# nanoporetech/dorado

Hardware: NVIDIA H100
Metric: basecalled samples/s (higher is better)
Workload: dtype f16 (fp32 accumulate; fp32 decode)

## Files before the change

### dorado_b200/csrc/capi.cu

```cuda
#include "b200call.h"

#include "common.cuh"
#include "decode.h"
#include "engine.h"

#include <cmath>
#include <cstddef>
#include <cstring>
#include <limits>
#include <string>

#undef b200_engine_create
#undef b200_pool_create

namespace {

thread_local std::string g_last_error;

constexpr size_t kDescSizeBeforeLstmPrecision = offsetof(b200_model_desc, lstm_precision);

b200_model_desc read_desc(const b200_model_desc* desc, size_t desc_size) {
    if (desc_size < kDescSizeBeforeLstmPrecision) throw std::invalid_argument("b200_model_desc: desc_size is smaller than any published descriptor");
    const unsigned char* bytes = reinterpret_cast<const unsigned char*>(desc);
    for (size_t i = sizeof(b200_model_desc); i < desc_size; ++i) {
// ... 90 lines not shown
        buf[buf_len - 1] = '\0';
    });
}

int b200_engine_terminate(b200_engine* e) {
    return guarded([&] {
        if (!e) throw std::invalid_argument("b200_engine_terminate: null argument");
        reinterpret_cast<b200::Engine*>(e)->terminate();
    });
}

int b200_engine_restart(b200_engine* e) {
    return guarded([&] {
        if (!e) throw std::invalid_argument("b200_engine_restart: null argument");
        reinterpret_cast<b200::Engine*>(e)->restart();
    });
}

int b200_engine_set_low_latency(b200_engine* e, int32_t on) {
    return guarded([&] {
        if (!e) throw std::invalid_argument("b200_engine_set_low_latency: null argument");
        reinterpret_cast<b200::Engine*>(e)->set_low_latency(on != 0);
    });
}

int b200_engine_set_num_runners(b200_engine* e, int32_t num_runners) {
    return guarded([&] {
        if (!e || num_runners < 1) throw std::invalid_argument("b200_engine_set_num_runners: null engine or num_runners < 1");
        reinterpret_cast<b200::Engine*>(e)->set_num_runners(num_runners);
    });
}

int32_t b200_engine_num_runners(const b200_engine* e) { return e ? reinterpret_cast<const b200::Engine*>(e)->num_runners() : 0; }

int32_t b200_engine_is_low_latency(const b200_engine* e) { return e && reinterpret_cast<const b200::Engine*>(e)->low_latency(); }

int b200_engine_batch_timeouts_ms(const b200_engine* e, int32_t* first_chunk_ms, int32_t* last_chunk_ms) {
    return guarded([&] {
        if (!e) throw std::invalid_argument("b200_engine_batch_timeouts_ms: null argument");
        int a = 0, b = 0;
        reinterpret_cast<const b200::Engine*>(e)->batch_timeouts_ms(&a, &b);
        if (first_chunk_ms) *first_chunk_ms = a;
        if (last_chunk_ms) *last_chunk_ms = b;
    });
}

int b200_pool_create_sized(const b200_model_desc* desc, size_t desc_size, const b200_tensor* tensors, int32_t num_tensors,
                           const int32_t* devices, int32_t num_devices, int32_t runners_per_device, int32_t batch_size,
                           int32_t chunk_size, b200_pool** out) {
    return guarded([&] {
        if (!desc || !tensors || !devices || !out) throw std::invalid_argument("b200_pool_create: null argument");
        *out = reinterpret_cast<b200_pool*>(new b200::Pool(read_desc(desc, desc_size), tensors, num_tensors, devices, num_devices,
                                                           runners_per_device, batch_size, chunk_size));
    });
}

int b200_pool_create(const b200_model_desc* desc, const b200_tensor* tensors, int32_t num_tensors, const int32_t* devices,
                     int32_t num_devices, int32_t runners_per_device, int32_t batch_size, int32_t chunk_size, b200_pool** out) {
    return b200_pool_create_sized(desc, kDescSizeBeforeLstmPrecision, tensors, num_tensors, devices, num_devices,
                                  runners_per_device, batch_size, chunk_size, out);
}

int b200_pool_destroy(b200_pool* p) {
    return guarded([&] { delete reinterpret_cast<b200::Pool*>(p); });
}

int32_t b200_pool_num_runners(const b200_pool* p) { return p ? reinterpret_cast<const b200::Pool*>(p)->num_runners() : 0; }
int32_t b200_pool_out_len(const b200_pool* p) { return p ? reinterpret_cast<const b200::Pool*>(p)->out_len() : 0; }

b200_runner* b200_pool_runner(b200_pool* p, int32_t index) {
    return p ? reinterpret_cast<b200_runner*>(reinterpret_cast<b200::Pool*>(p)->runner(index)) : nullptr;
}

int b200_pool_runner_info(const b200_pool* p, int32_t index, int32_t* numa_node, int64_t* batches) {
    return guarded([&] {
        if (!p) throw std::invalid_argument("b200_pool_runner_info: null argument");
        const auto* pool = reinterpret_cast<const b200::Pool*>(p);
        if (index < 0 || index >= pool->num_runners()) throw std::invalid_argument("b200_pool_runner_info: index out of range");
        if (numa_node) *numa_node = pool->runner_numa_node(index);
        if (batches) *batches = pool->runner_batches(index);
    });
}

int b200_pool_call_chunks(b200_pool* p, const uint16_t* chunks, int64_t num_chunks, uint8_t* moves, char* sequence,
                          char* qstring, int32_t* n_bases, double* seconds) {
    return guarded([&] {
        if (!p) throw std::invalid_argument("b200_pool_call_chunks: null argument");
        const double s = reinterpret_cast<b200::Pool*>(p)->call_chunks(chunks, num_chunks, moves, sequence, qstring, n_bases);
        if (seconds) *seconds = s;
    });
}

int b200_runner_create(b200_engine* e, int32_t batch_size, int32_t chunk_size, b200_runner** out) {
    return guarded([&] {
        if (!e || !out) throw std::invalid_argument("b200_runner_create: null argument");
        *out = reinterpret_cast<b200_runner*>(new b200::Runner(*reinterpret_cast<b200::Engine*>(e), batch_size, chunk_size));
    });
}

int b200_runner_destroy(b200_runner* r) {
    return guarded([&] { delete reinterpret_cast<b200::Runner*>(r); });
}

int b200_runner_set_decoder_options(b200_runner* r, const b200_decoder_options* o) {
    return guarded([&] {
        if (!r || !o) throw std::invalid_argument("b200_runner_set_decoder_options: null argument");
        reinterpret_cast<b200::Runner*>(r)->set_decoder_options(*o);
    });
}

int32_t b200_runner_batch_size(const b200_runner* r) { return r ? reinterpret_cast<const b200::Runner*>(r)->batch_size() : 0; }
int32_t b200_runner_chunk_size(const b200_runner* r) { return r ? reinterpret_cast<const b200::Runner*>(r)->chunk_size() : 0; }
int32_t b200_runner_out_len(const b200_runner* r) { return r ? reinterpret_cast<const b200::Runner*>(r)->out_len() : 0; }

int b200_runner_accept_chunk_f16(b200_runner* r, int32_t idx, const uint16_t* samples, int64_t len) {
    return guarded([&] {
        if (!r || !samples) throw std::invalid_argument("b200_runner_accept_chunk_f16: null argument");
        reinterpret_cast<b200::Runner*>(r)->accept_chunk_f16(idx, samples, len);
    });
}

int b200_runner_accept_chunk_f32(b200_runner* r, int32_t idx, const float* samples, int64_t len) {
    return guarded([&] {
        if (!r || !samples) throw std::invalid_argument("b200_runner_accept_chunk_f32: null argument");
        reinterpret_cast<b200::Runner*>(r)->accept_chunk_f32(idx, samples, len);
    });
}

int32_t b200_runner_variable_chunk_sizes(const b200_runner* r) {
    return r && reinterpret_cast<const b200::Runner*>(r)->variable_chunk_sizes();
}

int b200_runner_accept_chunk_var_f16(b200_runner* r, int32_t idx, const uint16_t* samples, int64_t len) {
    return guarded([&] {
        if (!r || !samples) throw std::invalid_argument("b200_runner_accept_chunk_var_f16: null argument");
        reinterpret_cast<b200::Runner*>(r)->accept_chunk_var_f16(idx, samples, len);
    });
}

uint16_t* b200_runner_input(b200_runner* r) { return r ? reinterpret_cast<b200::Runner*>(r)->input() : nullptr; }

int b200_runner_call_chunks(b200_runner* r, int32_t num_chunks, b200_result* out) {
    return guarded([&] {
        if (!r || !out) throw std::invalid_argument("b200_runner_call_chunks: null argument");
        *out = reinterpret_cast<b200::Runner*>(r)->call_chunks(num_chunks);
    });
}

int b200_generate_chunks(uint64_t num_samples, uint64_t chunk_size, uint64_t stride, uint64_t overlap, uint64_t* offsets,
                         uint64_t capacity, uint64_t* count) {
    return guarded([&] {
        if (!count || (!offsets && capacity)) throw std::invalid_argument("b200_generate_chunks: null argument");
        *count = b200::generate_chunks(num_samples, chunk_size, stride, overlap, offsets, capacity);
    });
}

int b200_generate_variable_chunks(uint64_t num_samples, uint64_t chunk_size, uint64_t stride, uint64_t overlap,
                                  uint64_t* intervals, uint64_t capacity, uint64_t* count) {
    return guarded([&] {
        if (!count || (!intervals && capacity)) throw std::invalid_argument("b200_generate_variable_chunks: null argument");
        *count = b200::generate_variable_chunks(num_samples, chunk_size, stride, overlap, intervals, capacity);
    });
}

int b200_stitch_chunks(const b200_called_chunk* chunks, uint64_t n_chunks, uint64_t raw_samples, int32_t stride,
                       uint8_t* moves_out, char* sequence_out, char* qstring_out, uint64_t* n_moves_out,
                       uint64_t* n_bases_out) {
    return guarded([&] {
        if (!moves_out || !sequence_out || !qstring_out || !n_moves_out || !n_bases_out) {
            throw std::invalid_argument("b200_stitch_chunks: null argument");
        }
        b200::stitch_chunks(chunks, n_chunks, raw_samples, stride, moves_out, sequence_out, qstring_out, n_moves_out,
                            n_bases_out);
    });
}

int b200_runner_accept_raw_chunk(b200_runner* r, int32_t chunk_idx, const b200_raw_chunk* chunk) {
    return guarded([&] {
        if (!r || !chunk) throw std::invalid_argument("b200_runner_accept_raw_chunk: null argument");
        reinterpret_cast<b200::Runner*>(r)->accept_raw_chunk(chunk_idx, *chunk);
    });
}

int b200_runner_debug_read_input(b200_runner* r, int32_t num_chunks, uint16_t* input_out) {
    return guarded([&] {
        if (!r) throw std::invalid_argument("b200_runner_debug_read_input: null argument");
        reinterpret_cast<b200::Runner*>(r)->debug_read_input(num_chunks, input_out);
    });
}

int b200_engine_runner_bytes(b200_engine* e, int32_t batch_size, int32_t chunk_size, uint64_t* bytes) {
    return guarded([&] {
        if (!e || !bytes) throw std::invalid_argument("b200_engine_runner_bytes: null argument");
        *bytes = b200::runner_device_bytes(*reinterpret_cast<b200::Engine*>(e), batch_size, chunk_size);
    });
}

int b200_engine_benchmark_batch_sizes(b200_engine* e, int32_t chunk_size, int32_t granularity, int32_t max_batch_size,
                                      int32_t* batch_sizes, float* ms_per_chunk, int32_t capacity, int32_t* count) {
    return guarded([&] {
        if (!e || !count || capacity < 0) throw std::invalid_argument("b200_engine_benchmark_batch_sizes: bad argument");
        *count = b200::benchmark_batch_sizes(*reinterpret_cast<b200::Engine*>(e), chunk_size, granularity, max_batch_size,
                                             batch_sizes, ms_per_chunk, capacity);
    });
}

int b200_select_batch_size(const int32_t* batch_sizes, const float* ms_per_chunk, int32_t count, int32_t max_batch_size,
                           int32_t granularity, float time_penalty, int32_t* selected) {
    return guarded([&] {
        if (!selected) throw std::invalid_argument("b200_select_batch_size: null argument");
        *selected = b200::select_batch_size(batch_sizes, ms_per_chunk, count, max_batch_size, granularity, time_penalty);
    });
}

int b200_runner_upload(b200_runner* r) {
    return guarded([&] {
        if (!r) throw std::invalid_argument("b200_runner_upload: null argument");
        reinterpret_cast<b200::Runner*>(r)->upload();
    });
}

int b200_runners_step_device(b200_runner** runners, int32_t n_runners, int32_t num_chunks, int32_t iters, float* total_ms) {
    return guarded([&] {
        if (!runners || !total_ms) throw std::invalid_argument("b200_runners_step_device: null argument");
        b200::pipelined_steps(reinterpret_cast<b200::Runner**>(runners), n_runners, num_chunks, iters, total_ms);
    });
}

int b200_runner_step_device(b200_runner* r, int32_t num_chunks, int32_t iters, float* total_ms, float* forward_ms,
                            float* decode_ms) {
    return guarded([&] {
        if (!r || !total_ms) throw std::invalid_argument("b200_runner_step_device: null argument");
        reinterpret_cast<b200::Runner*>(r)->step_device(num_chunks, iters, total_ms, forward_ms, decode_ms);
    });
}

int b200_runner_forward_scores(b200_runner* r, int32_t num_chunks, uint16_t* scores_out) {
    return guarded([&] {
        if (!r || !scores_out) throw std::invalid_argument("b200_runner_forward_scores: null argument");
        reinterpret_cast<b200::Runner*>(r)->forward_scores_to_host(num_chunks, scores_out);
    });
}

int b200_runner_profile(b200_runner* r, int32_t num_chunks, char* buf, uint64_t buf_len) {
    return guarded([&] {
        if (!r || !buf || buf_len == 0) throw std::invalid_argument("b200_runner_profile: null argument");
        const std::string s = reinterpret_cast<b200::Runner*>(r)->profile(num_chunks);
        std::strncpy(buf, s.c_str(), buf_len - 1);
        buf[buf_len - 1] = 0;
    });
}

int b200_runner_plan_info(const b200_runner* r, char* buf, uint64_t buf_len) {
    return guarded([&] {
        if (!r || !buf || buf_len == 0) throw std::invalid_argument("b200_runner_plan_info: null argument");
        const std::string s = reinterpret_cast<const b200::Runner*>(r)->plan_info();
        std::strncpy(buf, s.c_str(), buf_len - 1);
        buf[buf_len - 1] = 0;
    });
}

int b200_runner_debug_read_workspace(b200_runner* r, uint64_t offset, uint64_t bytes, void* dst) {
    return guarded([&] {
        if (!r || !dst) throw std::invalid_argument("debug_read_workspace: null argument");
        reinterpret_cast<b200::Runner*>(r)->debug_read_workspace(offset, bytes, dst);
    });
}

int b200_decode_scores(int32_t device, const uint16_t* scores, int32_t N, int32_t T, int32_t C, float clamp_val,
                       const b200_decoder_options* opts, uint8_t* moves, char* sequence, char* qstring,
                       int32_t* n_bases) {
    return guarded([&] {
        if (!scores || !opts || !moves || !sequence || !qstring || !n_bases) {
            throw std::invalid_argument("b200_decode_scores: null argument");
        }
        b200::decode_host_scores(device, scores, N, T, C, clamp_val, *opts, moves, sequence, qstring, n_bases);
    });
}

int b200_test_gemm(int32_t device, const uint16_t* a, const uint16_t* b, const float* bias, int32_t M, int32_t N,
                   int32_t K, int32_t activation, uint16_t* c) {
    return guarded([&] {
        if (!a || !b || !c) throw std::invalid_argument("b200_test_gemm: null argument");
        b200::test_gemm_host(device, a, b, bias, M, N, K, activation, c);
    });
}

int b200_test_gemm_fp8(int32_t device, const uint8_t* a, const uint8_t* b, int32_t M, int32_t N, int32_t K, int32_t activation,
                       const uint16_t* residual, float alpha, void* c) {
    return guarded([&] {
        if (!a || !b || !c) throw std::invalid_argument("b200_test_gemm_fp8: null argument");
        b200::test_gemm_fp8_host(device, a, b, M, N, K, activation, residual, alpha, c);
    });
}

int b200_test_gemm_s8(int32_t device, const int8_t* a, const int8_t* b, const float* col_scale, const float* bias, int32_t M,
                      int32_t N, int32_t K, int32_t activation, uint16_t* c) {
    return guarded([&] {
        if (!a || !b || !col_scale || !c) throw std::invalid_argument("b200_test_gemm_s8: null argument");
        b200::test_gemm_s8_host(device, a, b, col_scale, bias, M, N, K, activation, c);
    });
}

int b200_test_quantize_rows(const uint16_t* f16, int32_t rows, int32_t cols, int8_t* q, uint16_t* scale) {
    return guarded([&] {
        if (rows < 1 || cols < 1 || !f16 || !q || !scale) throw std::invalid_argument("b200_test_quantize_rows: bad argument");
        b200::quantize_rows_f16(f16, rows, cols, q, scale);
    });
}

int b200_test_to_e4m3(const uint16_t* f16, int64_t n, uint8_t* out) {
    return guarded([&] {
        if (n < 0 || (n && (!f16 || !out))) throw std::invalid_argument("b200_test_to_e4m3: bad argument");
        for (int64_t i = 0; i < n; ++i) out[i] = b200::e4m3_from_f16_bits(f16[i]);
    });
}

int b200_test_remove_bits(const uint16_t* f16, int64_t n, int32_t bits, uint16_t* out) {
    return guarded([&] {
        if (n < 0 || (n && (!f16 || !out)) || bits < 0 || bits > 10) throw std::invalid_argument("b200_test_remove_bits: bad argument");
        for (int64_t i = 0; i < n; ++i) out[i] = b200::remove_bits_f16(f16[i], bits);
    });
}

int b200_test_attention(int32_t device, const uint16_t* qkv, int32_t N, int32_t T, int32_t H, int32_t win_upper,
                        int32_t win_lower, uint16_t* out) {
    return guarded([&] {
        if (!qkv || !out) throw std::invalid_argument("b200_test_attention: null argument");
        b200::test_attention_host(device, qkv, N, T, H, win_upper, win_lower, out);
    });
}

}

extern "C" {

int b200_modbase_engine_create(const b200_modbase_desc* desc, const b200_tensor* tensors, int32_t num_tensors, int32_t device,
                               b200_modbase_engine** out) {
    return guarded([&] {
        if (!desc || !tensors || !out) throw std::invalid_argument("b200_modbase_engine_create: null argument");
        *out = reinterpret_cast<b200_modbase_engine*>(new b200::ModBaseEngine(*desc, tensors, num_tensors, device));
    });
}

int b200_modbase_engine_destroy(b200_modbase_engine* e) {
    return guarded([&] { delete reinterpret_cast<b200::ModBaseEngine*>(e); });
}

int b200_modbase_runner_create(b200_modbase_engine* e, int32_t batch_size, b200_modbase_runner** out) {
    return guarded([&] {
        if (!e || !out) throw std::invalid_argument("b200_modbase_runner_create: null argument");
        *out = reinterpret_cast<b200_modbase_runner*>(new b200::ModBaseRunner(*reinterpret_cast<b200::ModBaseEngine*>(e), batch_size));
    });
}

int b200_modbase_runner_destroy(b200_modbase_runner* r) {
    return guarded([&] { delete reinterpret_cast<b200::ModBaseRunner*>(r); });
}

static const b200::ModBaseRunner* mb_runner(const b200_modbase_runner* r) { return reinterpret_cast<const b200::ModBaseRunner*>(r); }
int32_t b200_modbase_runner_batch_size(const b200_modbase_runner* r) { return r ? mb_runner(r)->batch_size() : 0; }
int32_t b200_modbase_runner_sig_len(const b200_modbase_runner* r) { return r ? mb_runner(r)->engine().sig_len : 0; }
int32_t b200_modbase_runner_seq_len(const b200_modbase_runner* r) { return r ? mb_runner(r)->engine().seq_len : 0; }
int32_t b200_modbase_runner_out_len(const b200_modbase_runner* r) { return r ? mb_runner(r)->engine().out_len : 0; }
int32_t b200_modbase_runner_num_out(const b200_modbase_runner* r) { return r ? mb_runner(r)->engine().desc().num_out : 0; }

int b200_modbase_runner_accept_chunk(b200_modbase_runner* r, int32_t idx, const uint16_t* signal, int64_t sig_len,
                                     const int8_t* kmers, int64_t kmer_elems) {
    return guarded([&] {
        if (!r) throw std::invalid_argument("b200_modbase_runner_accept_chunk: null runner");
        reinterpret_cast<b200::ModBaseRunner*>(r)->accept_chunk(idx, signal, sig_len, kmers, kmer_elems);
    });
}

int b200_modbase_runner_call_chunks(b200_modbase_runner* r, int32_t num_chunks, const uint16_t** probs) {
    return guarded([&] {
        if (!r || !probs) throw std::invalid_argument("b200_modbase_runner_call_chunks: null argument");
        *probs = reinterpret_cast<b200::ModBaseRunner*>(r)->call_chunks(num_chunks);
    });
}

int b200_modbase_runner_profile(b200_modbase_runner* r, char* buf, uint64_t buf_len) {
    return guarded([&] {
        if (!r || !buf || buf_len == 0) throw std::invalid_argument("b200_modbase_runner_profile: null argument");
        const std::string s = reinterpret_cast<b200::ModBaseRunner*>(r)->profile();
        std::strncpy(buf, s.c_str(), buf_len - 1);
        buf[buf_len - 1] = '\0';
    });
}

int b200_modbase_runner_debug_read_workspace(b200_modbase_runner* r, uint64_t offset, uint64_t bytes, void* dst) {
    return guarded([&] {
        if (!r || !dst) throw std::invalid_argument("b200_modbase_runner_debug_read_workspace: null argument");
        reinterpret_cast<b200::ModBaseRunner*>(r)->debug_read_workspace(offset, bytes, dst);
    });
}

}
```

### dorado_b200/csrc/engine.h

```cpp
#pragma once

#include "b200call.h"
#include "b200_crf_math.h"
#include "frontend.h"
#include "common.cuh"
#include "lstm_kernels.h"

#include <atomic>
#include <condition_variable>
#include <memory>
#include <mutex>
#include <stdexcept>
#include <string>
#include <vector>

namespace b200 {

struct Unsupported : std::runtime_error {
    using std::runtime_error::runtime_error;
};

class Bump {
public:
    Bump() = default;
// ... 3 lines not shown
        const size_t off = m_used;
        m_used += (bytes + 255) & ~size_t(255);
        if (!m_base) return nullptr;
        if (m_used > m_cap) throw std::logic_error("device memory layout overflows its allocation");
        return static_cast<T*>(static_cast<void*>(m_base + off));
    }
    size_t used() const { return m_used; }

private:
    unsigned char* m_base = nullptr;
    size_t m_cap = 0, m_used = 0;
};

class Arena {
public:
    Arena() = default;
    ~Arena() {
        if (m_base) cudaFree(m_base);
    }
    Arena(const Arena&) = delete;
    Arena& operator=(const Arena&) = delete;
    template <typename F>
    void allocate(F&& layout) {
        if (m_base) throw std::logic_error("Arena::allocate called twice");
        Bump sizing;
        layout(sizing);
        B200_CUDA(cudaMalloc(&m_base, sizing.used()));
        m_cap = sizing.used();
        Bump carve(m_base, m_cap);
        layout(carve);
    }
    size_t capacity() const { return m_cap; }

private:
    unsigned char* m_base = nullptr;
    size_t m_cap = 0;
};

struct ProfileSink {
    std::vector<cudaEvent_t> events;
    std::vector<std::string> names;
    void begin(cudaStream_t s);
    void mark(const char* name, cudaStream_t s);
    std::vector<std::pair<std::string, float>> report();
    ~ProfileSink();
};

class ForwardPlan {
public:
    virtual ~ForwardPlan() = default;
    virtual void run(cudaStream_t stream, ProfileSink* prof = nullptr) = 0;
    virtual int launches() const = 0;
    virtual void set_chunk_lengths(const int32_t* ) {}
    virtual std::string info() const { return std::string(); }
    virtual void check_errors() {}
};

class Model {
public:
    virtual ~Model() = default;
    virtual size_t workspace_bytes(int N, int T_in) const = 0;
    virtual bool variable_chunk_sizes() const { return false; }
    int num_runners_hint = 2;
    virtual std::unique_ptr<ForwardPlan> make_plan(int N, int T_in, const __half* signal, __half* scores,
                                                   void* workspace, size_t workspace_bytes) = 0;
};

std::unique_ptr<Model> make_lstm_model(const b200_model_desc& desc, const b200_tensor* tensors, int n);
std::unique_ptr<Model> make_tx_model(const b200_model_desc& desc, const b200_tensor* tensors, int n);

const b200_tensor& find_tensor(const b200_tensor* tensors, int n, const std::string& name);
__half* upload_f16(const std::vector<float>& v);
float* upload_f32(const std::vector<float>& v);

class Engine {
public:
    Engine(const b200_model_desc& desc, const b200_tensor* tensors, int num_tensors, int device);
    ~Engine();
    const b200_model_desc& desc() const { return m_desc; }
    int device() const { return m_device; }
    cudaStream_t stream() const { return m_stream; }
    Model& model() { return *m_model; }
    std::mutex& stats_mutex() { return m_stats_mutex; }
    b200_stats stats() const;

    void terminate();
    void restart();
    bool terminated() const { return m_terminated.load(); }
    void set_low_latency(bool on) { m_low_latency.store(on); }
    void set_num_runners(int n) { m_model->num_runners_hint = n < 1 ? 1 : (n > 16 ? 16 : n); }
    int num_runners() const { return m_model->num_runners_hint; }
    bool low_latency() const { return m_low_latency.load(); }
    void batch_timeouts_ms(int* first_chunk_ms, int* last_chunk_ms) const;
    struct CallGuard {
        explicit CallGuard(Engine& e);
        ~CallGuard();
        Engine& eng;
    };

    std::atomic<int64_t> batches_called{0};
    std::atomic<int64_t> gpu_launches{0};
    std::atomic<int64_t> arena_bytes{0};
    double model_decode_ms = 0, h2d_ms = 0, d2h_ms = 0;

private:
    b200_model_desc m_desc;
    int m_device;
    cudaStream_t m_stream = nullptr;
    std::unique_ptr<Model> m_model;
    mutable std::mutex m_stats_mutex;
    std::atomic<bool> m_terminated{false};
    std::atomic<bool> m_low_latency{false};
    std::mutex m_life_mutex;
    std::condition_variable m_life_cv;
    int m_in_flight = 0;
};

class Runner;
void pipelined_steps(Runner** runners, int n_runners, int num_chunks, int iters, float* total_ms);

struct RunnerBuffers {
    b200_qtable* qtable = nullptr;
    int32_t* lens = nullptr;
    __half* input = nullptr;
    __half* scores = nullptr;
    void* ws = nullptr;
    size_t ws_bytes = 0;
    float* bwd = nullptr;
    uint2* beam = nullptr;
    unsigned char* out = nullptr;
    size_t out_bytes = 0;
};

class Runner {
public:
    friend void pipelined_steps(Runner** runners, int n_runners, int num_chunks, int iters, float* total_ms);
    Runner(Engine& engine, int batch_size, int chunk_size);
    ~Runner();
    int batch_size() const { return m_N; }
    int chunk_size() const { return m_T_in; }
    int out_len() const { return m_T_out; }
    uint16_t* input();
    void set_decoder_options(const b200_decoder_options& o);
    void accept_chunk_f16(int idx, const uint16_t* samples, int64_t len);
    void accept_chunk_f32(int idx, const float* samples, int64_t len);
    bool variable_chunk_sizes() const;
    void accept_chunk_var_f16(int idx, const uint16_t* samples, int64_t len);
    void accept_raw_chunk(int idx, const b200_raw_chunk& chunk);
    void debug_read_input(int num_chunks, uint16_t* input_out);
    b200_result call_chunks(int num_chunks);
    void upload();
    void fill_synthetic_input();
    void step_device(int num_chunks, int iters, float* total_ms, float* forward_ms, float* decode_ms);
    void forward_scores_to_host(int num_chunks, uint16_t* scores_out);
    void debug_read_workspace(uint64_t offset, uint64_t bytes, void* dst);
    std::string profile(int num_chunks);
    std::string plan_info() const { return m_plan ? m_plan->info() : std::string(); }

private:
    void init();
    void release();
    bool m_counted = false;
    void stage_input(int n);
    void clear_raw_slot(int idx);
    void run_forward(int n);
    void run_decode(int n, ProfileSink* prof = nullptr);

    Engine& m_engine;
    cudaStream_t m_stream = nullptr;
    std::mutex m_mutex;
    int m_N, m_T_in, m_T_out, m_C;
    b200_decoder_options m_opts;
    uint16_t* m_h_input = nullptr;
    unsigned char* m_h_out = nullptr;
    int16_t* m_h_raw = nullptr;
    RawSlot* m_h_slots = nullptr;
    int16_t* m_d_raw = nullptr;
    RawSlot* m_d_slots = nullptr;
    int m_num_raw = 0;
    Arena m_arena;
    RunnerBuffers m_dev;
    std::unique_ptr<ForwardPlan> m_plan;
    void upload_qtable();
    int32_t* m_h_lens = nullptr;
    int32_t* m_h_nmoves = nullptr;
    cudaEvent_t m_ev[4] = {nullptr, nullptr, nullptr, nullptr};
};

class ModBaseEngine {
public:
    ModBaseEngine(const b200_modbase_desc& desc, const b200_tensor* tensors, int num_tensors, int device);
    ~ModBaseEngine();
    ModBaseEngine(const ModBaseEngine&) = delete;
    ModBaseEngine& operator=(const ModBaseEngine&) = delete;
    const b200_modbase_desc& desc() const { return m_desc; }
    int device() const { return m_device; }

    int sig_len = 0;
    int seq_len = 0;
    int t_enc = 0;
    int T = 0;
    int out_len = 0;
    float* sig12_w = nullptr;
    __half* sig3_w = nullptr;
    float* sig3_b = nullptr;
    float* seq1_w = nullptr;
    __half* seq2_w = nullptr;
    float* seq2_b = nullptr;
    __half* merge_w = nullptr;
    float* merge_b = nullptr;
    LstmLayerWeights lstm[2];
    float* fc_w = nullptr;
    float* fc_b = nullptr;
    float* up_w = nullptr;
    float* up_b = nullptr;

private:
    b200_modbase_desc m_desc;
    int m_device;
};

struct ModBasePlan;
class ModBaseRunner {
public:
    ModBaseRunner(ModBaseEngine& engine, int batch_size);
    ~ModBaseRunner();
    int batch_size() const { return m_N; }
    const ModBaseEngine& engine() const { return m_engine; }
    void accept_chunk(int idx, const uint16_t* signal, int64_t sig_len, const int8_t* kmers, int64_t kmer_elems);
    const uint16_t* call_chunks(int num_chunks);
    std::string profile();
    void debug_read_workspace(uint64_t offset, uint64_t bytes, void* dst);

private:
    void init();
    void release();
    void run(ProfileSink* prof);

    ModBaseEngine& m_engine;
    int m_N;
    int64_t m_kmer_elems = 0, m_out_elems = 0;
    cudaStream_t m_stream = nullptr;
    std::mutex m_mutex;
    uint16_t* m_h_sig = nullptr;
    int8_t* m_h_kmers = nullptr;
    __half* m_h_out = nullptr;
    Arena m_arena;
    void* m_d_ws = nullptr;
    size_t m_ws_bytes = 0;
    __half* m_d_sig = nullptr;
    int8_t* m_d_kmers = nullptr;
    __half* m_d_out = nullptr;
    std::unique_ptr<ModBasePlan> m_plan;
};

class Pool {
public:
    Pool(const b200_model_desc& desc, const b200_tensor* tensors, int num_tensors, const int* devices, int num_devices,
         int runners_per_device, int batch_size, int chunk_size);
    ~Pool();
    int num_runners() const;
    Runner* runner(int i);
    int runner_numa_node(int i) const;
    int64_t runner_batches(int i) const;
    int out_len() const { return m_t_out; }
    double call_chunks(const uint16_t* chunks, int64_t num_chunks, uint8_t* moves, char* sequence, char* qstring,
                       int32_t* n_bases);

private:
    struct Worker;
    struct Job {
        const uint16_t* chunks = nullptr;
        int64_t num_chunks = 0;
        uint8_t* moves = nullptr;
        char* sequence = nullptr;
        char* qstring = nullptr;
        int32_t* n_bases = nullptr;
    };
    void worker_main(Worker& w);
    void shutdown();
    int m_batch, m_chunk, m_t_out = 0;
    std::vector<std::unique_ptr<Engine>> m_engines;
    std::vector<std::unique_ptr<Worker>> m_workers;
    std::mutex m_mutex, m_job_mutex;
    std::condition_variable m_cv_job, m_cv_done;
    long long m_job_id = 0;
    int m_ready = 0, m_done = 0;
    bool m_stop = false;
    Job m_job;
    std::atomic<int64_t> m_cursor{0};
};

void decode_host_scores(int device, const uint16_t* scores, int N, int T, int C, float clamp_val,
                        const b200_decoder_options& opts, uint8_t* moves, char* sequence, char* qstring,
                        int32_t* n_bases);
void test_gemm_host(int device, const uint16_t* a, const uint16_t* b, const float* bias, int M, int N, int K,
                    int activation, uint16_t* c);
void test_attention_host(int device, const uint16_t* qkv, int N, int T, int H, int win_upper, int win_lower, uint16_t* out);
void test_gemm_fp8_host(int device, const uint8_t* a, const uint8_t* b, int M, int N, int K, int activation,
                        const uint16_t* residual, float alpha, void* c);

void test_gemm_s8_host(int device, const int8_t* a, const int8_t* b, const float* col_scale, const float* bias, int M, int N,
                       int K, int activation, uint16_t* c);
void quantize_rows_f16(const uint16_t* w16, int rows, int cols, int8_t* q, uint16_t* scale16);
float int8_row_inv(uint16_t scale16);

uint16_t f16_bits(float v);
uint16_t remove_bits_f16(uint16_t b, int bits);
std::vector<float> fp16_remove_bits(const float* v, size_t n, int bits);
uint8_t e4m3_from_f16_bits(uint16_t b);

size_t runner_device_bytes(Engine& engine, int batch_size, int chunk_size);
int benchmark_batch_sizes(Engine& engine, int chunk_size, int granularity, int max_batch_size, int32_t* batch_sizes,
                          float* ms_per_chunk, int capacity);
int select_batch_size(const int32_t* batch_sizes, const float* ms_per_chunk, int count, int max_batch_size, int granularity,
                      float time_penalty);

int lookup_chunk_benchmarks(const char* gpu_name, const char* model_name, int32_t* batch_sizes, float* ms_per_chunk, int capacity);
std::string device_name(int device);

void ensure_dynamic_smem(const void* kernel, int bytes);
template <typename K>
inline void ensure_dynamic_smem(K* kernel, int bytes) {
    ensure_dynamic_smem(reinterpret_cast<const void*>(kernel), bytes);
}

float log_beam_cut_of(float beam_cut);
void require_sm90(int device);

}
```

### dorado_b200/csrc/gemm.cu

```cuda
#include "gemm.h"

#include "common.cuh"
#include "engine.h"

#include <cstdlib>
#include <cstring>
#include <type_traits>
#include <vector>

namespace b200 {

namespace {

constexpr int BM = 128;
constexpr int BK = 64;
constexpr int BK8 = 128;
constexpr int BN_MAX = 128;
constexpr int STAGES = 5;
constexpr int GEMM_PARTS = 4;
constexpr int GEMM_THREADS = 384;

struct GemmKernelParams {
    int rows_per_batch, tiles_per_batch, N, num_k_blocks, bn;
    int num_tiles, n_tiles, m_tiles;
    int mfast;
    const float* bias;
    __half* out;
    uint32_t out_m1;
    long long out_s0, out_s1;
    uint32_t out_col_m1;
    long long out_col_s0;
    int bias_per_row;
    const float* rope;
    int rope_T, rope_cols, rope_stride;
    const __half* residual;
    float alpha;
    float* out_ss;
    const float* a_ss;
    const float* res_ss;
    const float* res_gain;
    int a_ss_parts, res_ss_parts;
    float norm_inv_dim, norm_eps;
    const float* col_scale;
};

__device__ __forceinline__ bool gemm_tile_at(const GemmKernelParams& p, int i, int* mt, int* nt) {
    const int tile = (int)blockIdx.x + i * (int)gridDim.x;
    if (p.mfast) {
        *mt = tile % p.m_tiles;
        *nt = tile / p.m_tiles;
    } else {
        *mt = tile / p.n_tiles;
        *nt = tile % p.n_tiles;
    }
    return tile < p.num_tiles;
}

template <int ACT>
__device__ __forceinline__ float act_apply(float v) {
    if constexpr (ACT == GEMM_ACT_SWISH) return swish_fast(v);
    else if constexpr (ACT == GEMM_ACT_SWISH_CLAMP) return fminf(swish_fast(v), 3.5f);
    else if constexpr (ACT == GEMM_ACT_TANH) return tanh_fast(v);
    else if constexpr (ACT == GEMM_ACT_TANH_X5) return 5.0f * tanh_fast(v);
    else return v;
}

template <int NCH, bool FP8, typename Acc>
__device__ __forceinline__ void wgmma_k_block(Acc (&acc)[BN_MAX / 32][16], uint64_t adesc, uint64_t bdesc, bool accumulate) {
#pragma unroll
    for (int k = 0; k < 4; ++k) {
#pragma unroll
        for (int c = 0; c < NCH; ++c) {
            if constexpr (std::is_same_v<Acc, int32_t>) {
                tc::wgmma_m64n32k32_s8(acc[c], adesc + (uint64_t)(2 * k), bdesc + (uint64_t)(c * 256 + 2 * k), accumulate || k != 0);
            } else if constexpr (FP8) {
                tc::wgmma_m64n32k32_e4m3(acc[c], adesc + (uint64_t)(2 * k), bdesc + (uint64_t)(c * 256 + 2 * k), accumulate || k != 0);
            } else {
                tc::wgmma_m64n32k16(acc[c], adesc + (uint64_t)(2 * k), bdesc + (uint64_t)(c * 256 + 2 * k), accumulate || k != 0);
            }
        }
    }
}

template <int ACT, bool FP8, int Q8 = GEMM_Q8_NONE>
__global__ void __launch_bounds__(GEMM_THREADS, 1) gemm_wgmma_kernel(const __grid_constant__ CUtensorMap tma_a,
                                                                     const __grid_constant__ CUtensorMap tma_w,
                                                                     const GemmKernelParams p) {
    constexpr bool S8 = Q8 == GEMM_Q8_OPERANDS;
    constexpr int KB = FP8 || S8 ? BK8 : BK;
    using Acc = std::conditional_t<S8, int32_t, float>;
    extern __shared__ __align__(1024) uint8_t smem_raw[];
    uint8_t* smem = smem_raw + ((1024u - (tc::smem_u32(smem_raw) & 1023u)) & 1023u);
    const uint32_t a_bytes = BM * 128;
    const uint32_t w_bytes = (uint32_t)p.bn * 128;
    const uint32_t stage_bytes = a_bytes + w_bytes;
    uint64_t* full = reinterpret_cast<uint64_t*>(smem + STAGES * stage_bytes);
    uint64_t* empty = full + STAGES;
    const int nch = p.bn / 32;

    if (threadIdx.x == 0) {
        for (int s = 0; s < STAGES; ++s) {
            tc::mbar_init(&full[s], 1);
            tc::mbar_init(&empty[s], 2);
        }
        tc::fence_barrier_init();
        tc::prefetch_tmap(&tma_a);
        tc::prefetch_tmap(&tma_w);
    }
    __syncthreads();
    const int wg = threadIdx.x >> 7;

    if (wg == 0) {
        if (threadIdx.x == 0) {
            int s = 0;
            uint32_t ph = 0;
            int mt, nt;
            for (int i = 0; gemm_tile_at(p, i, &mt, &nt); ++i) {
                const int batch = mt / p.tiles_per_batch;
                const int r0 = (mt % p.tiles_per_batch) * BM;
                for (int kb = 0; kb < p.num_k_blocks; ++kb) {
                    tc::mbar_wait_silent(&empty[s], ph ^ 1);
                    tc::mbar_arrive_expect_tx(&full[s], stage_bytes);
                    uint8_t* st = smem + s * stage_bytes;
                    tc::tma_load_3d(st, &tma_a, &full[s], kb * KB, r0, batch);
                    tc::tma_load_2d(st + a_bytes, &tma_w, &full[s], kb * KB, nt * p.bn);
                    if (++s == STAGES) {
                        s = 0;
                        ph ^= 1;
                    }
                }
            }
        }
        return;
    }

    const int half = wg - 1;
    const int t = threadIdx.x - 128 * wg;
    const int lane = t & 31, quad = lane & 3;
    const int rloc = half * 64 + (t >> 5) * 16 + (lane >> 2);
    const int n_out_total = ACT == GEMM_ACT_SWIGLU ? p.N / 2 : p.N;
    int s = 0;
    uint32_t ph = 0;
    int mt, nt;
    for (int ti = 0; gemm_tile_at(p, ti, &mt, &nt); ++ti) {
        Acc acc[BN_MAX / 32][16];
        int prev = -1;
        for (int kb = 0; kb < p.num_k_blocks; ++kb) {
            tc::mbar_wait_silent(&full[s], ph);
            const uint32_t st = tc::smem_u32(smem + s * stage_bytes);
            const uint64_t adesc = tc::wgmma_desc_sw128(st + (uint32_t)(half * 64 * 128));
            const uint64_t bdesc = tc::wgmma_desc_sw128(st + a_bytes);
            tc::wgmma_fence();
            switch (nch) {
                case 1: wgmma_k_block<1, FP8>(acc, adesc, bdesc, kb != 0); break;
                case 2: wgmma_k_block<2, FP8>(acc, adesc, bdesc, kb != 0); break;
                case 3: wgmma_k_block<3, FP8>(acc, adesc, bdesc, kb != 0); break;
                default: wgmma_k_block<4, FP8>(acc, adesc, bdesc, kb != 0); break;
            }
            tc::wgmma_commit();
            tc::wgmma_wait<1>();
            if (prev >= 0 && t == 0) tc::mbar_arrive(&empty[prev]);
            prev = s;
            if (++s == STAGES) {
                s = 0;
                ph ^= 1;
            }
        }
        tc::wgmma_wait<0>();
        if (t == 0) tc::mbar_arrive(&empty[prev]);

        const int batch = mt / p.tiles_per_batch;
        const int r0 = (mt % p.tiles_per_batch) * BM;
        const int n0 = nt * p.bn;
        bool valid[2];
        long long g[2], off[2];
        float r_a[2], r_res[2], row_bias[2];
#pragma unroll
        for (int h = 0; h < 2; ++h) {
            const int row = r0 + rloc + 8 * h;
            valid[h] = row < p.rows_per_batch;
            const uint32_t g32 = (uint32_t)(batch * p.rows_per_batch + row);
            g[h] = g32;
            off[h] = valid[h] ? (long long)(g32 / p.out_m1) * p.out_s0 + (long long)(g32 % p.out_m1) * p.out_s1 : 0;
            r_a[h] = 1.0f;
            r_res[h] = 1.0f;
            if (p.a_ss && valid[h]) {
                float ss = 0.0f;
                for (int i = 0; i < p.a_ss_parts; ++i) ss += __ldg(p.a_ss + g[h] * p.a_ss_parts + i);
                r_a[h] = rsqrtf(ss * p.norm_inv_dim + p.norm_eps);
            }
            if (p.res_ss && valid[h]) {
                float ss = 0.0f;
                for (int i = 0; i < p.res_ss_parts; ++i) ss += __ldg(p.res_ss + g[h] * p.res_ss_parts + i);
                r_res[h] = rsqrtf(ss * p.norm_inv_dim + p.norm_eps);
            }
            row_bias[h] = (p.bias && p.bias_per_row && valid[h]) ? __ldg(p.bias + g[h]) : 0.0f;
        }
        if constexpr (S8) {
#pragma unroll
            for (int c = 0; c < BN_MAX / 32; ++c) {
                if (c >= nch) continue;
#pragma unroll
                for (int j = 0; j < 4; ++j) {
                    const int nc = n0 + c * 32 + 8 * j + 2 * quad;
                    const float2 sc = __ldg(reinterpret_cast<const float2*>(p.col_scale + nc));
                    float2 b2 = make_float2(0.0f, 0.0f);
                    if (p.bias) b2 = __ldg(reinterpret_cast<const float2*>(p.bias + nc));
#pragma unroll
                    for (int h = 0; h < 2; ++h) {
                        if (!valid[h]) continue;
                        const float v0 = fmaf((float)acc[c][4 * j + 2 * h], sc.x, b2.x);
                        const float v1 = fmaf((float)acc[c][4 * j + 2 * h + 1], sc.y, b2.y);
                        *reinterpret_cast<__half2*>(p.out + off[h] + nc) = __floats2half2_rn(act_apply<ACT>(v0), act_apply<ACT>(v1));
                    }
                }
            }
        } else if constexpr (ACT == GEMM_ACT_ROPE) {
#pragma unroll
            for (int c = 0; c < BN_MAX / 32; c += 2) {
                if (c < nch) {
                    const int nc0 = n0 + c * 32;
                    const bool rot = nc0 < p.rope_cols;
#pragma unroll
                    for (int h = 0; h < 2; ++h) {
                        if (!valid[h]) continue;
                        const float4* tab = reinterpret_cast<const float4*>(p.rope) + (int)((uint32_t)g[h] % (uint32_t)p.rope_T);
#pragma unroll
                        for (int j = 0; j < 4; ++j) {
                            const int col = 8 * j + 2 * quad;
                            float a0 = acc[c][4 * j + 2 * h] * r_a[h], a1 = acc[c][4 * j + 2 * h + 1] * r_a[h];
                            float b0 = acc[c + 1][4 * j + 2 * h] * r_a[h], b1 = acc[c + 1][4 * j + 2 * h + 1] * r_a[h];
                            if (rot) {
                                const float4 cs = __ldg(tab + (size_t)(col / 2) * p.rope_stride);
                                const float x0 = cs.x * a0 - cs.y * b0, y0 = cs.y * a0 + cs.x * b0;
                                const float x1 = cs.z * a1 - cs.w * b1, y1 = cs.w * a1 + cs.z * b1;
                                a0 = x0; b0 = y0; a1 = x1; b1 = y1;
                            }
                            *reinterpret_cast<__half2*>(p.out + off[h] + nc0 + col) = __floats2half2_rn(a0, a1);
                            *reinterpret_cast<__half2*>(p.out + off[h] + nc0 + 32 + col) = __floats2half2_rn(b0, b1);
                        }
                    }
                }
            }
        } else {
            float ss_out[2][BN_MAX / 32];
#pragma unroll
            for (int c = 0; c < BN_MAX / 32; ++c) {
                ss_out[0][c] = ss_out[1][c] = 0.0f;
                if (c >= nch) continue;
#pragma unroll
                for (int j = 0; j < 4; ++j) {
                    const int nc = n0 + c * 32 + 8 * j + 2 * quad;
                    float2 b2 = make_float2(0.0f, 0.0f);
                    if (p.bias && !p.bias_per_row) b2 = __ldg(reinterpret_cast<const float2*>(p.bias + nc));
                    float2 gain = make_float2(1.0f, 1.0f);
                    if (p.residual && p.res_gain) gain = __ldg(reinterpret_cast<const float2*>(p.res_gain + nc));
                    const long long coff = p.out_col_m1 > 0
                            ? (long long)((uint32_t)nc / p.out_col_m1) * p.out_col_s0 + (long long)((uint32_t)nc % p.out_col_m1)
                            : nc;
#pragma unroll
                    for (int h = 0; h < 2; ++h) {
                        if (!valid[h]) continue;
                        float v0 = acc[c][4 * j + 2 * h] * r_a[h] + b2.x + row_bias[h];
                        float v1 = acc[c][4 * j + 2 * h + 1] * r_a[h] + b2.y + row_bias[h];
                        if constexpr (ACT == GEMM_ACT_SWIGLU) {
                            if constexpr (FP8) {
                                reinterpret_cast<uint8_t*>(p.out)[off[h] + nc / 2] = (uint8_t)tc::cvt_e4m3x2(v0 * swish_fast(v1), 0.0f);
                            } else {
                                p.out[off[h] + nc / 2] = __float2half_rn(v0 * swish_fast(v1));
                            }
                        } else {
                            if (p.residual) {
                                const float2 f = __half22float2(
                                        *reinterpret_cast<const __half2*>(p.residual + g[h] * (long long)n_out_total + nc));
                                const float ar = p.alpha * r_res[h];
                                v0 += (ar * gain.x) * f.x;
                                v1 += (ar * gain.y) * f.y;
                            }
                            const __half2 o = __floats2half2_rn(act_apply<ACT>(v0), act_apply<ACT>(v1));
                            if (p.out_ss) {
                                const float2 f = __half22float2(o);
                                ss_out[h][c] = fmaf(f.x, f.x, ss_out[h][c]);
                                ss_out[h][c] = fmaf(f.y, f.y, ss_out[h][c]);
                            }
                            if constexpr (Q8 == GEMM_Q8_STORE) {
                                const int32_t q0 = tc::cvt_rni_sat_s8(kInt8ActScale * act_apply<ACT>(v0));
                                const int32_t q1 = tc::cvt_rni_sat_s8(kInt8ActScale * act_apply<ACT>(v1));
                                *reinterpret_cast<uint16_t*>(reinterpret_cast<int8_t*>(p.out) + off[h] + coff) =
                                        (uint16_t)((q0 & 0xff) | ((q1 & 0xff) << 8));
                            } else {
                                *reinterpret_cast<__half2*>(p.out + off[h] + coff) = o;
                            }
                        }
                    }
                }
            }
            if (p.out_ss) {
#pragma unroll
                for (int h = 0; h < 2; ++h) {
#pragma unroll
                    for (int c = 0; c < GEMM_PARTS; ++c) {
                        float v = ss_out[h][c];
                        v += __shfl_xor_sync(0xffffffffu, v, 1);
                        v += __shfl_xor_sync(0xffffffffu, v, 2);
                        if (quad == 0 && valid[h]) p.out_ss[g[h] * (long long)(p.n_tiles * GEMM_PARTS) + nt * GEMM_PARTS + c] = v;
                    }
                }
            }
        }
    }
}

using EncodeFn = CUresult (*)(CUtensorMap*, CUtensorMapDataType, cuuint32_t, void*, const cuuint64_t*, const cuuint64_t*,
                              const cuuint32_t*, const cuuint32_t*, CUtensorMapInterleave, CUtensorMapSwizzle,
                              CUtensorMapL2promotion, CUtensorMapFloatOOBfill);

EncodeFn get_encode_fn() {
    static const EncodeFn fn = [] {
        void* p = nullptr;
        cudaDriverEntryPointQueryResult q;
        B200_CUDA(cudaGetDriverEntryPoint("cuTensorMapEncodeTiled", &p, cudaEnableDefault, &q));
        if (q != cudaDriverEntryPointSuccess || !p) throw CudaError("cuTensorMapEncodeTiled entry point not available");
        return reinterpret_cast<EncodeFn>(p);
    }();
    return fn;
}

CUtensorMap encode(const void* base, int rank, const cuuint64_t* dims, const cuuint64_t* strides_bytes,
                   const cuuint32_t* box, CUtensorMapSwizzle swz, uint32_t elem_bytes) {
    CUtensorMap m;
    cuuint32_t estr[5] = {1, 1, 1, 1, 1};
    const CUtensorMapDataType dt = elem_bytes == 1 ? CU_TENSOR_MAP_DATA_TYPE_UINT8 : CU_TENSOR_MAP_DATA_TYPE_FLOAT16;
    const CUresult r = get_encode_fn()(&m, dt, (cuuint32_t)rank, const_cast<void*>(base), dims,
                                       strides_bytes, box, estr, CU_TENSOR_MAP_INTERLEAVE_NONE, swz,
                                       CU_TENSOR_MAP_L2_PROMOTION_L2_256B, CU_TENSOR_MAP_FLOAT_OOB_FILL_NONE);
    if (r != CUDA_SUCCESS) {
        throw CudaError("cuTensorMapEncodeTiled failed with CUresult " + std::to_string((int)r));
    }
    return m;
}

}

CUtensorMap make_tmap_2d(const void* base, uint64_t inner, uint64_t outer, uint64_t outer_stride_bytes, uint32_t box_inner,
                         uint32_t box_outer, uint32_t elem_bytes) {
    const cuuint64_t dims[2] = {inner, outer};
    const cuuint64_t strides[1] = {outer_stride_bytes};
    const cuuint32_t box[2] = {box_inner, box_outer};
    const CUtensorMapSwizzle swz = box_inner * elem_bytes == 128 ? CU_TENSOR_MAP_SWIZZLE_128B
                                   : box_inner * elem_bytes == 64 ? CU_TENSOR_MAP_SWIZZLE_64B
                                                                  : CU_TENSOR_MAP_SWIZZLE_NONE;
    return encode(base, 2, dims, strides, box, swz, elem_bytes);
}

CUtensorMap make_tmap_3d(const void* base, uint64_t d0, uint64_t d1, uint64_t d2, uint64_t s1_bytes, uint64_t s2_bytes,
                         uint32_t b0, uint32_t b1, uint32_t b2, uint32_t elem_bytes) {
    const cuuint64_t dims[3] = {d0, d1, d2};
    const cuuint64_t strides[2] = {s1_bytes, s2_bytes};
    const cuuint32_t box[3] = {b0, b1, b2};
    const CUtensorMapSwizzle swz = b0 * elem_bytes == 128 ? CU_TENSOR_MAP_SWIZZLE_128B
                                   : b0 * elem_bytes == 64 ? CU_TENSOR_MAP_SWIZZLE_64B
                                                           : CU_TENSOR_MAP_SWIZZLE_NONE;
    return encode(base, 3, dims, strides, box, swz, elem_bytes);
}

static int pick_bn(int N) {
    for (int bn = BN_MAX; bn >= 32; bn -= 32) {
        if (N % bn == 0) return bn;
    }
    return 0;
}

int gemm_out_ss_parts(int N) {
    const int bn = pick_bn(N);
    if (bn <= 0) throw std::invalid_argument("gemm: N must be a multiple of 32");
    return (N / bn) * GEMM_PARTS;
}

GemmPlan make_gemm_plan(const GemmDesc& d) {
    const bool s8 = d.q8 == GEMM_Q8_OPERANDS;
    const int kb = d.fp8 || s8 ? BK8 : BK;
    const int eb = d.fp8 || s8 ? 1 : 2;
    if (d.K % kb != 0 || d.K <= 0) {
        throw std::invalid_argument(eb == 1 ? "gemm: E4M3 / int8 K must be a positive multiple of 128" : "gemm: K must be a positive multiple of 64");
    }
    if (d.q8 != GEMM_Q8_NONE) {
        const bool plain = !d.fp8 && !d.residual && !d.out_ss && !d.a_ss && !d.res_ss && !d.bias_per_row && d.out_col_m1 == 0;
        if (s8 && !(plain && d.col_scale && (d.act == GEMM_ACT_NONE || d.act == GEMM_ACT_TANH_X5))) {
            throw std::invalid_argument("gemm: int8 operands take col_scale, a column bias and the plain or TANH_X5 epilogue only");
        }
        if (d.q8 == GEMM_Q8_STORE && !(plain && d.act == GEMM_ACT_TANH)) {
            throw std::invalid_argument("gemm: the int8 store goes with fp16 operands and the TANH epilogue only");
        }
        if (!s8 && d.q8 != GEMM_Q8_STORE) throw std::invalid_argument("gemm: unknown q8 form");
    }
    if (d.fp8 && (d.act != GEMM_ACT_NONE && d.act != GEMM_ACT_SWIGLU)) {
        throw std::invalid_argument("gemm: E4M3 operands take the plain and SwiGLU epilogues only");
    }
    if (d.N % 32 != 0) throw std::invalid_argument("gemm: N must be a multiple of 32");
    if (d.batches < 1 || d.rows_per_batch < 1) throw std::invalid_argument("gemm: empty A");
    if ((d.a_row_stride * eb) % 16 != 0 || (d.a_batch_stride * eb) % 16 != 0) {
        throw std::invalid_argument("gemm: A strides must be multiples of 16 bytes");
    }
    GemmPlan p{};
    p.d = d;
    p.bn = pick_bn(d.N);
    if (d.N / p.bn < 2 && d.N >= 128 && (long long)d.batches * ((d.rows_per_batch + BM - 1) / BM) < kNumSMs / 2) {
        p.bn = pick_bn(d.N / 2);
    }
    if (p.bn == 0) throw std::invalid_argument("gemm: no valid tile width");
    if (d.out_ss) {
        if (p.bn != pick_bn(d.N) || p.bn / 32 != GEMM_PARTS || d.act == GEMM_ACT_SWIGLU || d.act == GEMM_ACT_ROPE) {
            throw std::invalid_argument("gemm: out_ss needs a plain epilogue and tiles of 128 columns");
        }
    }
    if ((d.a_ss && (d.a_ss_parts < 1 || d.norm_dim < 1)) || (d.res_ss && (d.res_ss_parts < 1 || d.norm_dim < 1 || !d.residual))) {
        throw std::invalid_argument("gemm: folded RMSNorm needs the partial count, the norm dimension and a residual");
    }
    if (d.act == GEMM_ACT_SWIGLU && (p.bn % 64) != 0) throw std::invalid_argument("gemm: swiglu needs BN % 64 == 0");
    if (d.act == GEMM_ACT_ROPE && ((p.bn % 64) != 0 || !d.rope || d.rope_T <= 0)) {
        throw std::invalid_argument("gemm: rope epilogue needs BN % 64 == 0 and a table");
    }
    p.tiles_per_batch = (d.rows_per_batch + BM - 1) / BM;
    if ((long long)p.tiles_per_batch * BM * d.batches >= (1LL << 31) || d.out_m1 < 1 || d.out_m1 >= (1LL << 32) ||
        d.out_col_m1 < 0 || d.out_col_m1 >= (1LL << 32)) {
        throw std::invalid_argument("gemm: rows and output blocking must fit 32-bit index arithmetic");
    }
    p.grid = dim3((unsigned)(p.tiles_per_batch * d.batches), (unsigned)(d.N / p.bn), 1);
    p.smem = (size_t)STAGES * ((size_t)BM * 128 + (size_t)p.bn * 128) + 256 + 1024;
    if (p.smem > 227 * 1024) throw std::logic_error("gemm: shared-memory plan does not fit");
    const uint64_t batch_stride = d.batches > 1 ? (uint64_t)d.a_batch_stride * eb : (uint64_t)d.a_row_stride * eb * d.rows_per_batch;
    p.tma_a = make_tmap_3d(d.a, (uint64_t)(d.a_inner > 0 ? d.a_inner : d.K), (uint64_t)d.rows_per_batch, (uint64_t)d.batches, (uint64_t)d.a_row_stride * eb,
                           batch_stride, kb, BM, 1, eb);
    p.tma_w = make_tmap_2d(d.w, (uint64_t)d.K, (uint64_t)d.N, (uint64_t)d.K * eb, kb, (uint32_t)p.bn, eb);
    return p;
}

template <int ACT, bool FP8 = false, int Q8 = GEMM_Q8_NONE>
static void launch_gemm(int grid, size_t smem, cudaStream_t stream, const CUtensorMap& a, const CUtensorMap& w,
                        const GemmKernelParams& k) {
    ensure_dynamic_smem(gemm_wgmma_kernel<ACT, FP8, Q8>, 227 * 1024);
    gemm_wgmma_kernel<ACT, FP8, Q8><<<grid, GEMM_THREADS, smem, stream>>>(a, w, k);
}

void run_gemm(const GemmPlan& p, cudaStream_t stream) {
    GemmKernelParams k{};
    k.rows_per_batch = p.d.rows_per_batch;
    k.tiles_per_batch = p.tiles_per_batch;
    k.N = p.d.N;
    k.num_k_blocks = p.d.K / (p.d.fp8 || p.d.q8 == GEMM_Q8_OPERANDS ? BK8 : BK);
    k.bn = p.bn;
    k.bias = p.d.bias;
    k.out = static_cast<__half*>(p.d.out);
    k.out_m1 = (uint32_t)p.d.out_m1;
    k.out_s0 = p.d.out_s0;
    k.out_s1 = p.d.out_s1;
    k.out_col_m1 = (uint32_t)p.d.out_col_m1;
    k.out_col_s0 = p.d.out_col_s0;
    k.bias_per_row = p.d.bias_per_row;
    k.rope = p.d.rope;
    k.rope_T = p.d.rope_T;
    k.rope_cols = p.d.rope_cols;
    k.rope_stride = p.d.rope_stride;
    k.residual = p.d.residual;
    k.alpha = p.d.alpha;
    k.n_tiles = p.d.N / p.bn;
    k.m_tiles = p.tiles_per_batch * p.d.batches;
    k.num_tiles = k.m_tiles * k.n_tiles;
    k.mfast = k.m_tiles < k.n_tiles ? 1 : 0;
    k.out_ss = p.d.out_ss;
    k.a_ss = p.d.a_ss;
    k.res_ss = p.d.res_ss;
    k.res_gain = p.d.res_gain;
    k.a_ss_parts = p.d.a_ss_parts;
    k.res_ss_parts = p.d.res_ss_parts;
    k.norm_inv_dim = p.d.norm_dim > 0 ? 1.0f / (float)p.d.norm_dim : 0.0f;
    k.norm_eps = p.d.norm_eps;
    k.col_scale = p.d.col_scale;
    const int max_ctas = p.d.max_ctas > 0 && p.d.max_ctas < kNumSMs ? p.d.max_ctas : kNumSMs;
    const int grid = k.num_tiles < max_ctas ? k.num_tiles : max_ctas;
    if (p.d.fp8) {
        if (p.d.act == GEMM_ACT_SWIGLU) launch_gemm<GEMM_ACT_SWIGLU, true>(grid, p.smem, stream, p.tma_a, p.tma_w, k);
        else launch_gemm<GEMM_ACT_NONE, true>(grid, p.smem, stream, p.tma_a, p.tma_w, k);
        B200_CUDA(cudaGetLastError());
        return;
    }
    if (p.d.q8 != GEMM_Q8_NONE) {
        if (p.d.q8 == GEMM_Q8_STORE) launch_gemm<GEMM_ACT_TANH, false, GEMM_Q8_STORE>(grid, p.smem, stream, p.tma_a, p.tma_w, k);
        else if (p.d.act == GEMM_ACT_TANH_X5) launch_gemm<GEMM_ACT_TANH_X5, false, GEMM_Q8_OPERANDS>(grid, p.smem, stream, p.tma_a, p.tma_w, k);
        else launch_gemm<GEMM_ACT_NONE, false, GEMM_Q8_OPERANDS>(grid, p.smem, stream, p.tma_a, p.tma_w, k);
        B200_CUDA(cudaGetLastError());
        return;
    }
    switch (p.d.act) {
        case GEMM_ACT_NONE: launch_gemm<GEMM_ACT_NONE>(grid, p.smem, stream, p.tma_a, p.tma_w, k); break;
        case GEMM_ACT_SWISH: launch_gemm<GEMM_ACT_SWISH>(grid, p.smem, stream, p.tma_a, p.tma_w, k); break;
        case GEMM_ACT_SWISH_CLAMP: launch_gemm<GEMM_ACT_SWISH_CLAMP>(grid, p.smem, stream, p.tma_a, p.tma_w, k); break;
        case GEMM_ACT_TANH: launch_gemm<GEMM_ACT_TANH>(grid, p.smem, stream, p.tma_a, p.tma_w, k); break;
        case GEMM_ACT_TANH_X5: launch_gemm<GEMM_ACT_TANH_X5>(grid, p.smem, stream, p.tma_a, p.tma_w, k); break;
        case GEMM_ACT_SWIGLU: launch_gemm<GEMM_ACT_SWIGLU>(grid, p.smem, stream, p.tma_a, p.tma_w, k); break;
        case GEMM_ACT_ROPE: launch_gemm<GEMM_ACT_ROPE>(grid, p.smem, stream, p.tma_a, p.tma_w, k); break;
        default: throw std::invalid_argument("gemm: unknown activation");
    }
    B200_CUDA(cudaGetLastError());
}

void test_gemm_host(int device, const uint16_t* a, const uint16_t* b, const float* bias, int M, int N, int K, int activation,
                    uint16_t* c) {
    require_sm90(device);
    const int Kp = (K + BK - 1) / BK * BK;
    const int n_out = activation == GEMM_ACT_SWIGLU ? N / 2 : N;
    __half *d_a = nullptr, *d_w = nullptr, *d_c = nullptr;
    float* d_bias = nullptr;
    Arena arena;
    arena.allocate([&](Bump& b) {
        d_a = b.take<__half>((size_t)M * Kp * 2);
        d_w = b.take<__half>((size_t)N * Kp * 2);
        d_bias = b.take<float>((size_t)N * 4);
        d_c = b.take<__half>((size_t)M * n_out * 2);
    });
    B200_CUDA(cudaMemset(d_a, 0, (size_t)M * Kp * 2));
    B200_CUDA(cudaMemset(d_w, 0, (size_t)N * Kp * 2));
    B200_CUDA(cudaMemcpy2D(d_a, (size_t)Kp * 2, a, (size_t)K * 2, (size_t)K * 2, M, cudaMemcpyHostToDevice));
    B200_CUDA(cudaMemcpy2D(d_w, (size_t)Kp * 2, b, (size_t)K * 2, (size_t)K * 2, N, cudaMemcpyHostToDevice));
    if (bias) B200_CUDA(cudaMemcpy(d_bias, bias, (size_t)N * 4, cudaMemcpyHostToDevice));
    GemmDesc d{};
    d.a = d_a;
    d.batches = 1;
    d.rows_per_batch = M;
    d.a_row_stride = Kp;
    d.a_batch_stride = (int64_t)M * Kp;
    d.w = d_w;
    d.N = N;
    d.K = Kp;
    d.bias = bias ? d_bias : nullptr;
    d.act = activation;
    d.out = d_c;
    d.out_m1 = 1;
    d.out_s0 = n_out;
    d.out_s1 = 0;
    const GemmPlan plan = make_gemm_plan(d);
    run_gemm(plan, nullptr);
    B200_CUDA(cudaDeviceSynchronize());
    B200_CUDA(cudaMemcpy(c, d_c, (size_t)M * n_out * 2, cudaMemcpyDeviceToHost));
}

void test_gemm_fp8_host(int device, const uint8_t* a, const uint8_t* b, int M, int N, int K, int activation,
                        const uint16_t* residual, float alpha, void* c) {
    if (M < 1 || N < 1 || K < 1) throw std::invalid_argument("test_gemm_fp8: empty operand");
    if (activation != GEMM_ACT_NONE && activation != GEMM_ACT_SWIGLU) throw std::invalid_argument("test_gemm_fp8: plain or SwiGLU only");
    if (residual && activation != GEMM_ACT_NONE) throw std::invalid_argument("test_gemm_fp8: the residual goes with the plain epilogue");
    require_sm90(device);
    const int Kp = (K + BK8 - 1) / BK8 * BK8;
    const bool swiglu = activation == GEMM_ACT_SWIGLU;
    const int n_out = swiglu ? N / 2 : N;
    const size_t out_bytes = (size_t)M * n_out * (swiglu ? 1 : 2);
    uint8_t *d_a = nullptr, *d_w = nullptr;
    __half* d_res = nullptr;
    void* d_c = nullptr;
    Arena arena;
    arena.allocate([&](Bump& b) {
        d_a = b.take<uint8_t>((size_t)M * Kp);
        d_w = b.take<uint8_t>((size_t)N * Kp);
        d_res = b.take<__half>((size_t)M * N * 2);
        d_c = b.take(out_bytes);
    });
    B200_CUDA(cudaMemset(d_a, 0, (size_t)M * Kp));
    B200_CUDA(cudaMemset(d_w, 0, (size_t)N * Kp));
    B200_CUDA(cudaMemcpy2D(d_a, (size_t)Kp, a, (size_t)K, (size_t)K, M, cudaMemcpyHostToDevice));
    B200_CUDA(cudaMemcpy2D(d_w, (size_t)Kp, b, (size_t)K, (size_t)K, N, cudaMemcpyHostToDevice));
    if (residual) B200_CUDA(cudaMemcpy(d_res, residual, (size_t)M * N * 2, cudaMemcpyHostToDevice));
    GemmDesc d{};
    d.fp8 = 1;
    d.a = d_a;
    d.batches = 1;
    d.rows_per_batch = M;
    d.a_row_stride = Kp;
    d.a_batch_stride = (int64_t)M * Kp;
    d.w = d_w;
    d.N = N;
    d.K = Kp;
    d.act = activation;
    d.out = d_c;
    d.out_m1 = 1;
    d.out_s0 = n_out;
    d.out_s1 = 0;
    d.residual = residual ? d_res : nullptr;
    d.alpha = alpha;
    const GemmPlan plan = make_gemm_plan(d);
    run_gemm(plan, nullptr);
    B200_CUDA(cudaDeviceSynchronize());
    B200_CUDA(cudaMemcpy(c, d_c, out_bytes, cudaMemcpyDeviceToHost));
}

void test_gemm_s8_host(int device, const int8_t* a, const int8_t* b, const float* col_scale, const float* bias, int M, int N,
                       int K, int activation, uint16_t* c) {
    if (M < 1 || N < 1 || K < 1) throw std::invalid_argument("test_gemm_s8: empty operand");
    require_sm90(device);
    const int Kp = (K + BK8 - 1) / BK8 * BK8;
    int8_t *d_a = nullptr, *d_w = nullptr;
    float *d_scale = nullptr, *d_bias = nullptr;
    __half* d_c = nullptr;
    Arena arena;
    arena.allocate([&](Bump& bump) {
        d_a = bump.take<int8_t>((size_t)M * Kp);
        d_w = bump.take<int8_t>((size_t)N * Kp);
        d_scale = bump.take<float>((size_t)N * 4);
        d_bias = bump.take<float>((size_t)N * 4);
        d_c = bump.take<__half>((size_t)M * N * 2);
    });
    B200_CUDA(cudaMemset(d_a, 0, (size_t)M * Kp));
    B200_CUDA(cudaMemset(d_w, 0, (size_t)N * Kp));
    B200_CUDA(cudaMemcpy2D(d_a, (size_t)Kp, a, (size_t)K, (size_t)K, M, cudaMemcpyHostToDevice));
    B200_CUDA(cudaMemcpy2D(d_w, (size_t)Kp, b, (size_t)K, (size_t)K, N, cudaMemcpyHostToDevice));
    B200_CUDA(cudaMemcpy(d_scale, col_scale, (size_t)N * 4, cudaMemcpyHostToDevice));
    if (bias) B200_CUDA(cudaMemcpy(d_bias, bias, (size_t)N * 4, cudaMemcpyHostToDevice));
    GemmDesc d{};
    d.q8 = GEMM_Q8_OPERANDS;
    d.col_scale = d_scale;
    d.a = d_a;
    d.batches = 1;
    d.rows_per_batch = M;
    d.a_row_stride = Kp;
    d.a_batch_stride = (int64_t)M * Kp;
    d.w = d_w;
    d.N = N;
    d.K = Kp;
    d.bias = bias ? d_bias : nullptr;
    d.act = activation;
    d.out = d_c;
    d.out_m1 = 1;
    d.out_s0 = N;
    d.out_s1 = 0;
    const GemmPlan plan = make_gemm_plan(d);
    run_gemm(plan, nullptr);
    B200_CUDA(cudaDeviceSynchronize());
    B200_CUDA(cudaMemcpy(c, d_c, (size_t)M * N * 2, cudaMemcpyDeviceToHost));
}

}
```

### dorado_b200/csrc/gemm.h

```cpp
#pragma once

#include "tc.cuh"

namespace b200 {

enum GemmAct : int {
    GEMM_ACT_NONE = -1,
    GEMM_ACT_SWISH = 0,
    GEMM_ACT_SWISH_CLAMP = 1,
    GEMM_ACT_TANH = 2,
    GEMM_ACT_TANH_X5 = 3,
    GEMM_ACT_SWIGLU = 4,
    GEMM_ACT_ROPE = 5,
};

enum GemmQ8 : int {
    GEMM_Q8_NONE = 0,
    GEMM_Q8_OPERANDS = 1,
    GEMM_Q8_STORE = 2,
};
constexpr float kInt8ActScale = 127.0f;

struct GemmDesc {
    int fp8 = 0;
    int q8 = GEMM_Q8_NONE;
    const float* col_scale = nullptr;
    const void* a = nullptr;
    int batches = 1;
    int rows_per_batch = 0;
    int64_t a_row_stride = 0;
    int64_t a_batch_stride = 0;
    const void* w = nullptr;
    int N = 0;
    int K = 0;
    int a_inner = 0;
    const float* bias = nullptr;
    int act = GEMM_ACT_NONE;
    void* out = nullptr;
    int64_t out_m1 = 1;
    int64_t out_s0 = 0;
    int64_t out_s1 = 0;
    int64_t out_col_m1 = 0;
    int64_t out_col_s0 = 0;
    int bias_per_row = 0;
    const float* rope = nullptr;
    int rope_T = 0;
    int rope_cols = 0;
    int max_ctas = 0;
    int rope_stride = 0;
    const __half* residual = nullptr;
    float alpha = 0.0f;
    float* out_ss = nullptr;
    const float* a_ss = nullptr;
    int a_ss_parts = 0;
    const float* res_ss = nullptr;
    int res_ss_parts = 0;
    const float* res_gain = nullptr;
    int norm_dim = 0;
    float norm_eps = 1e-5f;
};

struct GemmPlan {
    CUtensorMap tma_a, tma_w;
    GemmDesc d;
    int bn = 128;
    int tiles_per_batch = 0;
    dim3 grid;
    size_t smem = 0;
};

GemmPlan make_gemm_plan(const GemmDesc& d);
int gemm_out_ss_parts(int N);
void run_gemm(const GemmPlan& p, cudaStream_t stream);

}
```

### dorado_b200/csrc/lstm_model.cu

```cuda
#include "engine.h"
#include "gemm.h"
#include "lstm_kernels.h"
#include "nvtx.h"
#include "tc.cuh"

#include <algorithm>
#include <cmath>
#include <cstdio>
#include <cstdlib>
#include <cstring>
#include <vector>

#include <cooperative_groups.h>

namespace cg = cooperative_groups;

namespace b200 {

namespace {

constexpr int CONV_TT = 256;
constexpr int MAXW = kConv12MaxWin;

constexpr int CONV_W_FLOATS = 16 * MAXW + 16 + MAXW * 16 * 16 + 16;
// ... 1119 lines not shown
}

bool LstmStack::run(cudaStream_t stream, ProfileSink* prof) {
    NvtxRange stack_range("lstm_stack");
    auto mark = [&](const char* name) {
        if (prof) prof->mark(name, stream);
    };
    const int C = m_d.C, Np = m_d.Np;
    if (m_ws.counters) B200_CUDA(cudaMemsetAsync(m_ws.counters, 0, m_ws.counter_bytes, stream));
    const int nl = m_debug_layers >= 0 && m_debug_layers < m_d.num_layers ? m_debug_layers : m_d.num_layers;
    for (int l = 0; l < nl; ++l) {
        NvtxRange r("lstm_layer");
        const LstmLayerWeights& w = m_d.layers[l];
        const int reverse = (l % 2 == 0) == m_d.reverse_first ? 1 : 0;
        if (m_kind == Kind::Layer) {
            lstm_layer_kernel<<<m_groups, FL_THREADS, 0, stream>>>(
                    LstmLayerParams{static_cast<__half*>(m_d.seq), w.w_ih, w.w_hh, w.bias, m_d.T, Np, reverse});
            mark("lstm_layer");
            continue;
        }
        run_gemm(m_gx_gemm[l], stream);
        if (m_d.int8) {
            mark("lstm_gx_gemm_i8");
            launch_lstm_rec_i8(C, m_nb, m_groups * m_group_ctas,
                               LstmRecI8Params{static_cast<int8_t*>(m_d.seq), m_ws.gx, w.w_hh8, w.inv, m_d.T, Np, reverse, m_lens,
                                               m_d.stride},
                               stream);
            mark("lstm_rec_i8");
            continue;
        }
        mark("lstm_gx_gemm");
        for (int i = 0; i < m_launches; ++i) {
            const int ctas = std::min(m_groups, Np / m_nb - i * m_groups) * m_group_ctas;
            unsigned int* counters = m_ws.counters ? m_ws.counters + (size_t)l * (Np / 32) + (size_t)i * m_groups : nullptr;
            const LstmRecParams p{static_cast<__half*>(m_d.seq), m_ws.gx, w.w_hh, m_d.T, Np, reverse, m_lens, m_d.stride, i * m_groups * m_nb,
                                  counters, m_ws.error};
            if (m_kind == Kind::Rec) {
                launch_lstm_rec(C, m_nb, ctas, p, stream);
                mark("lstm_rec");
            } else {
                launch_lstm_grid(C, m_nb, ctas, p, stream);
                mark("lstm_grid_rec");
            }
        }
    }
    if (m_error_host) B200_CUDA(cudaMemcpyAsync(m_error_host, m_ws.error, sizeof(int), cudaMemcpyDeviceToHost, stream));
    return nl == m_d.num_layers;
}

void LstmStack::check_errors() {
    if (!m_error_host || *m_error_host == 0) return;
    *m_error_host = 0;
    B200_CUDA(cudaMemset(m_ws.error, 0, sizeof(int)));
    throw std::runtime_error("lstm_grid_rec_kernel: a group of CTAs did not reach its step barrier within the time "
                             "budget; the outputs of this batch are invalid");
}

std::string LstmStack::info() const {
    const std::string ctas = std::to_string(m_groups * m_group_ctas);
    switch (m_kind) {
        case Kind::Layer: return "lstm_layer.ctas=" + ctas;
        case Kind::Rec:
            return "lstm_rec.ctas=" + ctas + ";lstm_rec.chunks_per_cluster=" + std::to_string(m_nb) + (m_d.int8 ? ";lstm.int8=1" : "");
        default:
            return "lstm_grid.ctas=" + ctas + ";lstm_grid.groups=" + std::to_string(m_groups) + ";lstm_grid.chunks_per_group=" +
                   std::to_string(m_nb) + ";lstm_grid.launches_per_layer=" + std::to_string(m_launches);
    }
}

int LstmStack::launches() const { return m_d.num_layers * (m_kind == Kind::Layer ? 1 : 1 + m_launches); }

namespace {

class LstmPlan final : public ForwardPlan {
public:
    void run(cudaStream_t stream, ProfileSink* prof) override;
    int launches() const override { return 1 + 1 + lstm->launches() + num_linear; }
    std::string info() const override { return lstm->info(); }
    void set_chunk_lengths(const int32_t* d_lens) override {
        if (!variable) return;
        conv12.lens = d_lens;
        lstm->set_chunk_lengths(d_lens);
    }
    void check_errors() override { lstm->check_errors(); }

    Conv12Params conv12{};
    dim3 conv12_grid;
    bool conv12_tc = false;
    int conv12_tiles_per_chunk = 0, conv12_tc_grid = 0;
    GemmPlan conv3;
    bool variable = false;
    std::unique_ptr<LstmStack> lstm;
    GemmPlan linear1, linear2;
    int num_linear = 1;
};

class LstmModel final : public Model {
public:
    LstmModel(const b200_model_desc& d, const b200_tensor* tensors, int n);
    ~LstmModel() override;
    size_t workspace_bytes(int N, int T_in) const override;
    std::unique_ptr<ForwardPlan> make_plan(int N, int T_in, const __half* signal, __half* scores, void* ws,
                                           size_t ws_bytes) override;
    bool variable_chunk_sizes() const override {
        return large() && desc.lstm_inner_dim == 0;
    }

    b200_model_desc desc;
    float* conv_w = nullptr;
    __half* w3 = nullptr;
    float* b3 = nullptr;
    int K3 = 0, K3p = 0;
    std::vector<LstmLayerWeights> layers;
    __half* wl1 = nullptr;
    float* bl1 = nullptr;
    __half* wl2 = nullptr;
    int Cp = 0, out1 = 0, out1p = 0;
    bool int8 = false;
    int8_t* wl1_8 = nullptr;
    float* wl1_inv = nullptr;

private:
    struct Buffers {
        __half* x2;
        void* seq;
        __half* mid;
        int* tile_counter;
        LstmStackBuffers lstm;
    };
    Buffers carve(Bump& b, int N, int T_in) const;
    int pad3() const { return desc.convs[2].winlen / 2; }
    int t_pad(int T_in) const { return T_in + 2 * pad3() + 8; }
    bool large() const { return desc.lstm_size > 96; }
    int n_pad(int N) const { return large() ? (N + 31) / 32 * 32 : (N + 15) / 16 * 16; }
};

LstmModel::LstmModel(const b200_model_desc& d, const b200_tensor* tensors, int n) : desc(d) {
    if (d.num_convs != 3) throw std::invalid_argument("Expected 3 convolution layers but found: " + std::to_string(d.num_convs));
    const auto &c1 = d.convs[0], &c2 = d.convs[1], &c3 = d.convs[2];
    if (c1.insize != 1 || c1.stride != 1 || c2.stride != 1 || c2.size != 16 || c1.size > 16 || c1.winlen > MAXW ||
        c2.winlen > MAXW || c2.insize != c1.size || c3.insize != 16) {
        throw Unsupported("conv stack shape outside what conv12_kernel implements");
    }
    const int C = d.lstm_size;
    if (C != c3.size) throw std::invalid_argument("last convolution size != lstm_size");
    if (C != 96 && C != 128 && C != 192 && C != 256 && C != 384 && C != 768 && C != 1024) {
        throw Unsupported("lstm_size " + std::to_string(C) + " is not supported (96, 128, 192, 256, 384, 768 and 1024 are)");
    }

    if (d.lstm_layers < 1 || d.lstm_layers > 8) throw std::invalid_argument("bad lstm_layers");
    int8 = d.lstm_precision == B200_LSTM_INT8;
    if (int8) {
        if (C != 256 && C != 384) {
            throw Unsupported("int8_lstm precision: lstm_size " + std::to_string(C) + " is not supported (256 and 384 are)");
        }
        if (c3.activation != B200_ACT_TANH) {
            throw Unsupported("int8_lstm precision needs a tanh last convolution: the int8 activations assume values in [-1, 1]");
        }
        if (d.lstm_inner_dim > 0) throw Unsupported("int8_lstm precision: FLSTM models (lstm_inner_dim > 0) are not supported");
    }

    conv_w = upload_conv12_weights(find_tensor(tensors, n, "0.conv.weight.tensor"), find_tensor(tensors, n, "0.conv.bias.tensor"),
                                   find_tensor(tensors, n, "1.conv.weight.tensor"), find_tensor(tensors, n, "1.conv.bias.tensor"),
                                   c1, c2);
    {
        const auto& tw = find_tensor(tensors, n, "2.conv.weight.tensor");
        const auto& tb = find_tensor(tensors, n, "2.conv.bias.tensor");
        K3 = c3.winlen * 16;
        K3p = (K3 + 63) / 64 * 64;
        std::vector<float> w((size_t)C * K3p, 0.0f);
        for (int co = 0; co < C; ++co)
            for (int ci = 0; ci < 16; ++ci)
                for (int k = 0; k < c3.winlen; ++k)
                    w[(size_t)co * K3p + k * 16 + ci] = tw.data[((size_t)co * 16 + ci) * c3.winlen + k];
        w3 = upload_f16(w);
        b3 = upload_f32(std::vector<float>(tb.data, tb.data + C));
    }
    for (int l = 0; l < d.lstm_layers; ++l) {
        const std::string pfx = std::to_string(d.num_convs + l + 1) + ".rnn.";
        std::vector<float> folded_ih, folded_hh;
        const float *wih, *whh, *bih, *bhh;
        if (d.lstm_inner_dim > 0) {
            const int K = d.lstm_inner_dim;
            auto fold = [&](const char* up_name, const char* dn_name, std::vector<float>& out) {
                const auto& up = find_tensor(tensors, n, pfx + up_name);
                const auto& dn = find_tensor(tensors, n, pfx + dn_name);
                if (up.ndim != 2 || dn.ndim != 2 || up.dims[0] != 4 * C || up.dims[1] != K || dn.dims[0] != K || dn.dims[1] != C) {
                    throw std::invalid_argument("FLSTM tensor " + pfx + up_name + " / " + dn_name + " has the wrong shape");
                }
                out.assign((size_t)4 * C * C, 0.0f);
                std::vector<double> acc((size_t)C);
                for (int r = 0; r < 4 * C; ++r) {
                    std::fill(acc.begin(), acc.end(), 0.0);
                    for (int k = 0; k < K; ++k) {
                        const double u = up.data[(size_t)r * K + k];
                        const float* drow = dn.data + (size_t)k * C;
                        for (int c2 = 0; c2 < C; ++c2) acc[c2] += u * (double)drow[c2];
                    }
                    for (int c2 = 0; c2 < C; ++c2) out[(size_t)r * C + c2] = (float)acc[c2];
                }
            };
            fold("up_weight_ih.tensor", "dn_weight_ih.tensor", folded_ih);
            fold("up_weight_hh.tensor", "dn_weight_hh.tensor", folded_hh);
            wih = folded_ih.data();
            whh = folded_hh.data();
            bih = find_tensor(tensors, n, pfx + "up_bias_ih.tensor").data;
            bhh = find_tensor(tensors, n, pfx + "up_bias_hh.tensor").data;
        } else {
            wih = find_tensor(tensors, n, pfx + "weight_ih_l0.tensor").data;
            whh = find_tensor(tensors, n, pfx + "weight_hh_l0.tensor").data;
            bih = find_tensor(tensors, n, pfx + "bias_ih_l0.tensor").data;
            bhh = find_tensor(tensors, n, pfx + "bias_hh_l0.tensor").data;
        }
        layers.push_back(int8 ? upload_lstm_layer_int8(C, wih, whh, bih, bhh) : upload_lstm_layer(C, wih, whh, bih, bhh));
    }
    {
        const int layer = d.num_convs + d.lstm_layers + 1;
        const auto& tw = find_tensor(tensors, n, std::to_string(layer) + ".linear.weight.tensor");
        out1 = d.out_features > 0 ? d.out_features : d.outsize;
        Cp = (C + 63) / 64 * 64;
        std::vector<float> w((size_t)out1 * Cp, 0.0f);
        for (int o = 0; o < out1; ++o) std::memcpy(&w[(size_t)o * Cp], &tw.data[(size_t)o * C], sizeof(float) * C);
        if (int8) {
            std::vector<uint16_t> w16((size_t)out1 * C), scale(out1);
            for (size_t i = 0; i < w16.size(); ++i) w16[i] = f16_bits(tw.data[i]);
            std::vector<int8_t> q(w16.size());
            quantize_rows_f16(w16.data(), out1, C, q.data(), scale.data());
            std::vector<float> inv(out1);
            for (int o = 0; o < out1; ++o) inv[o] = int8_row_inv(scale[o]);
            wl1_8 = upload_raw(q);
            wl1_inv = upload_f32(inv);
        } else {
            wl1 = upload_f16(w);
        }
        if (d.linear_bias) {
            const auto& tb = find_tensor(tensors, n, std::to_string(layer) + ".linear.bias.tensor");
            bl1 = upload_f32(std::vector<float>(tb.data, tb.data + out1));
        }
        if (d.out_features > 0) {
            if (out1 % 64 != 0) throw Unsupported("out_features must be a multiple of 64");
            const auto& tw2 = find_tensor(tensors, n, std::to_string(layer + 1) + ".linear.weight.tensor");
            wl2 = upload_f16(std::vector<float>(tw2.data, tw2.data + (size_t)d.outsize * out1));
        }
    }
}

LstmModel::~LstmModel() {
    cudaFree(conv_w);
    cudaFree(w3);
    cudaFree(b3);
    for (auto& l : layers) free_lstm_layer(l);
    cudaFree(wl1);
    cudaFree(wl1_8);
    cudaFree(wl1_inv);
    cudaFree(bl1);
    cudaFree(wl2);
}

LstmModel::Buffers LstmModel::carve(Bump& b, int N, int T_in) const {
    const int C = desc.lstm_size;
    const int T_out = T_in / desc.stride;
    const int Np = n_pad(N);
    if (Np != N) {
        throw std::invalid_argument(large() ? "batch_size must be a multiple of 32 for this LSTM size"
                                              : "batch_size must be a multiple of 16 for LSTM models");
    }
    Buffers w;
    w.x2 = b.take<__half>((size_t)N * t_pad(T_in) * 16 * 2);
    w.seq = b.take((size_t)(T_out + 1) * Np * C * (int8 ? 1 : 2));
    w.mid = desc.out_features > 0 ? b.take<__half>((size_t)T_out * Np * desc.out_features * 2) : nullptr;
    w.tile_counter = b.take<int>(sizeof(int));
    w.lstm = carve_lstm_stack(b, C, desc.lstm_layers, T_out, Np);
    return w;
}

size_t LstmModel::workspace_bytes(int N, int T_in) const {
    Bump sizing;
    carve(sizing, N, T_in);
    return sizing.used();
}

std::unique_ptr<ForwardPlan> LstmModel::make_plan(int N, int T_in, const __half* signal, __half* scores, void* ws,
                                                  size_t ws_bytes) {
    const int C = desc.lstm_size;
    const int T_out = T_in / desc.stride;
    const int Np = n_pad(N);
    Bump b(ws, ws_bytes);
    const auto [x2, seq, mid, tile_counter, lstm_ws] = carve(b, N, T_in);
    if (b.used() != ws_bytes) throw std::logic_error("LSTM workspace: the plan's layout differs from workspace_bytes()");
    auto plan = std::make_unique<LstmPlan>();
    const int Tp = t_pad(T_in);

    plan->conv12 = Conv12Params{signal, x2, conv_w, N, T_in, Tp, pad3(), desc.convs[0].size, desc.convs[0].winlen,
                                desc.convs[1].winlen, desc.convs[0].activation, desc.convs[1].activation, nullptr, tile_counter};
    plan->conv12_grid = dim3((T_in + CONV_TT - 1) / CONV_TT, N, 1);
    plan->conv12_tc = desc.convs[0].size == 16 && desc.convs[1].winlen == 5 && !std::getenv("B200_CONV12_FMA");
    plan->conv12_tiles_per_chunk = (T_in + C12_TILE - 1) / C12_TILE;
    {
        const long long tiles = (long long)plan->conv12_tiles_per_chunk * N;
        plan->conv12_tc_grid = (int)std::min<long long>(tiles, 5LL * kNumSMs);
        if (plan->conv12_tc) ensure_dynamic_smem(conv12_tc_kernel, C12_SMEM);
    }

    {
        GemmDesc g{};
        g.a = x2;
        g.batches = N;
        g.rows_per_batch = T_out;
        g.a_row_stride = (int64_t)desc.convs[2].stride * 16;
        g.a_batch_stride = (int64_t)Tp * 16;
        g.w = w3;
        g.N = C;
        g.K = K3p;
        g.bias = b3;
        g.act = desc.convs[2].activation;
        g.q8 = int8 ? GEMM_Q8_STORE : GEMM_Q8_NONE;
        g.out = seq;
        g.out_m1 = T_out;
        g.out_s0 = C;
        g.out_s1 = (int64_t)Np * C;
        plan->conv3 = make_gemm_plan(g);
    }
    plan->variable = variable_chunk_sizes();
    LstmStackDesc lstm{};
    lstm.C = C;
    lstm.T = T_out;
    lstm.Np = Np;
    lstm.stride = desc.stride;
    lstm.runners = num_runners_hint;
    lstm.reverse_first = true;
    lstm.int8 = int8;
    lstm.seq = seq;
    lstm.layers = layers.data();
    lstm.num_layers = desc.lstm_layers;
    plan->lstm = std::make_unique<LstmStack>(lstm, lstm_ws);
    {
        GemmDesc g{};
        g.a = seq;
        g.batches = 1;
        g.rows_per_batch = T_out * Np;
        g.a_row_stride = C;
        g.a_batch_stride = (int64_t)T_out * Np * C;
        g.w = wl1;
        g.N = out1;
        g.K = Cp;
        g.a_inner = C;
        g.bias = bl1;
        if (int8) {
            g.q8 = GEMM_Q8_OPERANDS;
            g.w = wl1_8;
            g.col_scale = wl1_inv;
            g.K = C;
        }
        if (desc.out_features > 0) {
            g.act = GEMM_ACT_NONE;
            g.out = mid;
            g.out_m1 = 1;
            g.out_s0 = out1;
            g.out_s1 = 0;
            plan->linear1 = make_gemm_plan(g);
            GemmDesc g2{};
            g2.a = mid;
            g2.batches = 1;
            g2.rows_per_batch = T_out * Np;
            g2.a_row_stride = out1;
            g2.a_batch_stride = (int64_t)T_out * Np * out1;
            g2.w = wl2;
            g2.N = desc.outsize;
            g2.K = out1;
            g2.act = desc.crf_scale == 5.0f ? GEMM_ACT_TANH_X5 : GEMM_ACT_NONE;
            g2.out = scores;
            g2.out_m1 = Np;
            g2.out_s0 = desc.outsize;
            g2.out_s1 = (int64_t)T_out * desc.outsize;
            plan->linear2 = make_gemm_plan(g2);
            plan->num_linear = 2;
        } else {
            g.act = desc.crf_scale == 5.0f ? GEMM_ACT_TANH_X5 : GEMM_ACT_NONE;
            g.out = scores;
            g.out_m1 = Np;
            g.out_s0 = desc.outsize;
            g.out_s1 = (int64_t)T_out * desc.outsize;
            plan->linear1 = make_gemm_plan(g);
            plan->num_linear = 1;
        }
    }
    return plan;
}

void LstmPlan::run(cudaStream_t stream, ProfileSink* prof) {
    {
        NvtxRange r("conv");
        if (conv12_tc) {
            B200_CUDA(cudaMemsetAsync(conv12.tile_counter, 0, sizeof(int), stream));
            conv12_tc_kernel<<<conv12_tc_grid, C12_THREADS, C12_SMEM, stream>>>(conv12, conv12_tiles_per_chunk,
                                                                                 conv12_tiles_per_chunk * conv12.N);
        } else {
            conv12_kernel<<<conv12_grid, CONV_TT, 0, stream>>>(conv12);
        }
        if (prof) prof->mark("conv12", stream);
        run_gemm(conv3, stream);
        if (prof) prof->mark("conv3_gemm", stream);
    }
    if (!lstm->run(stream, prof)) {
        B200_CUDA(cudaGetLastError());
        return;
    }
    NvtxRange r("linear");
    run_gemm(linear1, stream);
    if (prof) prof->mark("linear_gemm", stream);
    if (num_linear == 2) {
        run_gemm(linear2, stream);
        if (prof) prof->mark("linear2_gemm", stream);
    }
    B200_CUDA(cudaGetLastError());
}

}

std::unique_ptr<Model> make_lstm_model(const b200_model_desc& desc, const b200_tensor* tensors, int n) {
    return std::make_unique<LstmModel>(desc, tensors, n);
}

}
```

### dorado_b200/csrc/tc.cuh

```cuda
#pragma once

#include <cuda.h>
#include <cuda_fp16.h>
#include <cuda_runtime.h>
#include <stdint.h>
#include <stdio.h>

namespace b200 {
namespace tc {

__device__ __forceinline__ uint32_t smem_u32(const void* p) { return (uint32_t)__cvta_generic_to_shared(p); }

__device__ __forceinline__ void mbar_init(uint64_t* bar, uint32_t count) {
    asm volatile("mbarrier.init.shared::cta.b64 [%0], %1;" ::"r"(smem_u32(bar)), "r"(count));
}
__device__ __forceinline__ void fence_barrier_init() {
    asm volatile("fence.mbarrier_init.release.cluster;" ::: "memory");
}
__device__ __forceinline__ void mbar_arrive_expect_tx(uint64_t* bar, uint32_t bytes) {
    asm volatile("mbarrier.arrive.expect_tx.shared::cta.b64 _, [%0], %1;" ::"r"(smem_u32(bar)), "r"(bytes) : "memory");
}
__device__ __forceinline__ void mbar_arrive(uint64_t* bar) {
    asm volatile("mbarrier.arrive.shared::cta.b64 _, [%0];" ::"r"(smem_u32(bar)) : "memory");
}
__device__ __forceinline__ bool mbar_try_wait(uint64_t* bar, uint32_t parity) {
    uint32_t ok;
    asm volatile(
            "{\n\t.reg .pred p;\n\t"
            "mbarrier.try_wait.parity.shared::cta.b64 p, [%1], %2;\n\t"
            "selp.u32 %0, 1, 0, p;\n\t}"
            : "=r"(ok)
            : "r"(smem_u32(bar)), "r"(parity)
            : "memory");
    return ok != 0;
}
__device__ __forceinline__ void mbar_wait(uint64_t* bar, uint32_t parity) {
    uint32_t spins = 0;
    while (!mbar_try_wait(bar, parity)) {
        if (++spins > (1u << 26)) {
            printf("b200: mbarrier wait timeout (block %d thread %d)\n", (int)blockIdx.x, (int)threadIdx.x);
            __trap();
        }
    }
}

__device__ __forceinline__ void mbar_wait_silent(uint64_t* bar, uint32_t parity) {
    uint32_t spins = 0;
    while (!mbar_try_wait(bar, parity)) {
        if (++spins > (1u << 26)) __trap();
    }
}

__device__ __forceinline__ void prefetch_tmap(const CUtensorMap* m) {
    asm volatile("prefetch.tensormap [%0];" ::"l"(m) : "memory");
}
__device__ __forceinline__ void tma_load_2d(void* smem_dst, const CUtensorMap* m, uint64_t* bar, int c0, int c1) {
    asm volatile(
            "cp.async.bulk.tensor.2d.shared::cluster.global.mbarrier::complete_tx::bytes [%0], [%1, {%3, %4}], [%2];"
            ::"r"(smem_u32(smem_dst)), "l"(m), "r"(smem_u32(bar)), "r"(c0), "r"(c1)
            : "memory");
}
__device__ __forceinline__ void tma_load_3d(void* smem_dst, const CUtensorMap* m, uint64_t* bar, int c0, int c1, int c2) {
    asm volatile(
            "cp.async.bulk.tensor.3d.shared::cluster.global.mbarrier::complete_tx::bytes [%0], [%1, {%3, %4, %5}], [%2];"
            ::"r"(smem_u32(smem_dst)), "l"(m), "r"(smem_u32(bar)), "r"(c0), "r"(c1), "r"(c2)
            : "memory");
}
__device__ __forceinline__ void tma_store_2d(const CUtensorMap* m, const void* smem_src, int c0, int c1) {
    asm volatile("cp.async.bulk.tensor.2d.global.shared::cta.bulk_group [%0, {%2, %3}], [%1];"
                 ::"l"(m), "r"(smem_u32(smem_src)), "r"(c0), "r"(c1)
                 : "memory");
}
__device__ __forceinline__ void tma_store_3d(const CUtensorMap* m, const void* smem_src, int c0, int c1, int c2) {
    asm volatile("cp.async.bulk.tensor.3d.global.shared::cta.bulk_group [%0, {%2, %3, %4}], [%1];"
                 ::"l"(m), "r"(smem_u32(smem_src)), "r"(c0), "r"(c1), "r"(c2)
                 : "memory");
}
__device__ __forceinline__ void bulk_commit_group() { asm volatile("cp.async.bulk.commit_group;" ::: "memory"); }
template <int N>
__device__ __forceinline__ void bulk_wait_group_read() { asm volatile("cp.async.bulk.wait_group.read %0;" ::"n"(N) : "memory"); }
template <int N>
__device__ __forceinline__ void bulk_wait_group() { asm volatile("cp.async.bulk.wait_group %0;" ::"n"(N) : "memory"); }
__device__ __forceinline__ void bulk_copy_smem_to_cluster(uint32_t dst_cluster_addr, uint32_t src_cta_addr, uint32_t bytes,
                                                          uint32_t dst_mbar_cluster_addr) {
    asm volatile("cp.async.bulk.shared::cluster.shared::cta.mbarrier::complete_tx::bytes [%0], [%1], %2, [%3];"
                 ::"r"(dst_cluster_addr), "r"(src_cta_addr), "r"(bytes), "r"(dst_mbar_cluster_addr)
                 : "memory");
}
__device__ __forceinline__ void tma_load_2d_multicast(void* smem_dst, const CUtensorMap* m, uint64_t* bar, int c0, int c1,
                                                      uint16_t cta_mask) {
    asm volatile(
            "cp.async.bulk.tensor.2d.shared::cluster.global.mbarrier::complete_tx::bytes.multicast::cluster [%0], [%1, {%3, %4}], [%2], %5;"
            ::"r"(smem_u32(smem_dst)), "l"(m), "r"(smem_u32(bar)), "r"(c0), "r"(c1), "h"(cta_mask)
            : "memory");
}
__device__ __forceinline__ void cp_async_16(uint32_t smem_dst, const void* gmem_src) {
    asm volatile("cp.async.cg.shared.global [%0], [%1], 16;" ::"r"(smem_dst), "l"(gmem_src) : "memory");
}
__device__ __forceinline__ void cp_async_commit() { asm volatile("cp.async.commit_group;" ::: "memory"); }
template <int N>
__device__ __forceinline__ void cp_async_wait() { asm volatile("cp.async.wait_group %0;" ::"n"(N) : "memory"); }

__device__ __forceinline__ void red_release_gpu_add(unsigned int* p, unsigned int v) {
    asm volatile("red.release.gpu.global.add.u32 [%0], %1;" ::"l"(p), "r"(v) : "memory");
}
__device__ __forceinline__ unsigned int ld_acquire_gpu(const unsigned int* p) {
    unsigned int v;
    asm volatile("ld.acquire.gpu.global.u32 %0, [%1];" : "=r"(v) : "l"(p) : "memory");
    return v;
}
__device__ __forceinline__ int ld_relaxed_gpu(const int* p) {
    int v;
    asm volatile("ld.relaxed.gpu.global.s32 %0, [%1];" : "=r"(v) : "l"(p) : "memory");
    return v;
}

__device__ __forceinline__ void fence_proxy_async_smem() { asm volatile("fence.proxy.async.shared::cta;" ::: "memory"); }

__device__ __forceinline__ uint64_t wgmma_desc_sw128(uint32_t smem_addr) {
    uint64_t d = 0;
    d |= (uint64_t)((smem_addr & 0x3ffffu) >> 4);
    d |= (uint64_t)1 << 16;
    d |= (uint64_t)(1024 >> 4) << 32;
    d |= (uint64_t)1 << 62;
    return d;
}
__device__ __forceinline__ void wgmma_fence() { asm volatile("wgmma.fence.sync.aligned;" ::: "memory"); }
__device__ __forceinline__ void wgmma_commit() { asm volatile("wgmma.commit_group.sync.aligned;" ::: "memory"); }
template <int N>
__device__ __forceinline__ void wgmma_wait() { asm volatile("wgmma.wait_group.sync.aligned %0;" ::"n"(N) : "memory"); }
__device__ __forceinline__ void wgmma_m64n32k16(float* d, uint64_t adesc, uint64_t bdesc, bool accumulate) {
    asm volatile(
            "{\n\t.reg .pred p;\n\t"
            "setp.ne.b32 p, %18, 0;\n\t"
            "wgmma.mma_async.sync.aligned.m64n32k16.f32.f16.f16 "
            "{%0,%1,%2,%3,%4,%5,%6,%7,%8,%9,%10,%11,%12,%13,%14,%15}, %16, %17, p, 1, 1, 0, 0;\n\t}"
            : "+f"(d[0]), "+f"(d[1]), "+f"(d[2]), "+f"(d[3]), "+f"(d[4]), "+f"(d[5]), "+f"(d[6]), "+f"(d[7]), "+f"(d[8]),
              "+f"(d[9]), "+f"(d[10]), "+f"(d[11]), "+f"(d[12]), "+f"(d[13]), "+f"(d[14]), "+f"(d[15])
            : "l"(adesc), "l"(bdesc), "r"((uint32_t)accumulate)
            : "memory");
}
__device__ __forceinline__ void wgmma_m64n32k32_e4m3(float* d, uint64_t adesc, uint64_t bdesc, bool accumulate) {
    asm volatile(
            "{\n\t.reg .pred p;\n\t"
            "setp.ne.b32 p, %18, 0;\n\t"
            "wgmma.mma_async.sync.aligned.m64n32k32.f32.e4m3.e4m3 "
            "{%0,%1,%2,%3,%4,%5,%6,%7,%8,%9,%10,%11,%12,%13,%14,%15}, %16, %17, p, 1, 1;\n\t}"
            : "+f"(d[0]), "+f"(d[1]), "+f"(d[2]), "+f"(d[3]), "+f"(d[4]), "+f"(d[5]), "+f"(d[6]), "+f"(d[7]), "+f"(d[8]),
              "+f"(d[9]), "+f"(d[10]), "+f"(d[11]), "+f"(d[12]), "+f"(d[13]), "+f"(d[14]), "+f"(d[15])
            : "l"(adesc), "l"(bdesc), "r"((uint32_t)accumulate)
            : "memory");
}
__device__ __forceinline__ void wgmma_m64n32k32_s8(int32_t* d, uint64_t adesc, uint64_t bdesc, bool accumulate) {
    asm volatile(
            "{\n\t.reg .pred p;\n\t"
            "setp.ne.b32 p, %18, 0;\n\t"
            "wgmma.mma_async.sync.aligned.m64n32k32.s32.s8.s8 "
            "{%0,%1,%2,%3,%4,%5,%6,%7,%8,%9,%10,%11,%12,%13,%14,%15}, %16, %17, p;\n\t}"
            : "+r"(d[0]), "+r"(d[1]), "+r"(d[2]), "+r"(d[3]), "+r"(d[4]), "+r"(d[5]), "+r"(d[6]), "+r"(d[7]), "+r"(d[8]),
              "+r"(d[9]), "+r"(d[10]), "+r"(d[11]), "+r"(d[12]), "+r"(d[13]), "+r"(d[14]), "+r"(d[15])
            : "l"(adesc), "l"(bdesc), "r"((uint32_t)accumulate)
            : "memory");
}
__device__ __forceinline__ uint16_t cvt_e4m3x2(float lo, float hi) {
    uint16_t r;
    asm("cvt.rn.satfinite.e4m3x2.f32 %0, %1, %2;" : "=h"(r) : "f"(hi), "f"(lo));
    return r;
}

__device__ __forceinline__ void mma_f16_16816(float* c, const uint32_t* a, uint32_t b0, uint32_t b1) {
    asm volatile("mma.sync.aligned.m16n8k16.row.col.f32.f16.f16.f32 {%0,%1,%2,%3}, {%4,%5,%6,%7}, {%8,%9}, {%0,%1,%2,%3};"
                 : "+f"(c[0]), "+f"(c[1]), "+f"(c[2]), "+f"(c[3])
                 : "r"(a[0]), "r"(a[1]), "r"(a[2]), "r"(a[3]), "r"(b0), "r"(b1));
}
__device__ __forceinline__ void mma_s8_16832(int32_t* c, const uint32_t* a, uint32_t b0, uint32_t b1) {
    asm volatile("mma.sync.aligned.m16n8k32.row.col.s32.s8.s8.s32 {%0,%1,%2,%3}, {%4,%5,%6,%7}, {%8,%9}, {%0,%1,%2,%3};"
                 : "+r"(c[0]), "+r"(c[1]), "+r"(c[2]), "+r"(c[3])
                 : "r"(a[0]), "r"(a[1]), "r"(a[2]), "r"(a[3]), "r"(b0), "r"(b1));
}
__device__ __forceinline__ int32_t cvt_rni_sat_s8(float v) {
    int32_t r;
    asm("cvt.rni.sat.s8.f32 %0, %1;" : "=r"(r) : "f"(v));
    return r;
}
__device__ __forceinline__ void ldmatrix_x4(uint32_t* r, uint32_t smem_addr) {
    asm volatile("ldmatrix.sync.aligned.m8n8.x4.shared.b16 {%0,%1,%2,%3}, [%4];"
                 : "=r"(r[0]), "=r"(r[1]), "=r"(r[2]), "=r"(r[3])
                 : "r"(smem_addr));
}
__device__ __forceinline__ void ldmatrix_x4_trans(uint32_t* r, uint32_t smem_addr) {
    asm volatile("ldmatrix.sync.aligned.m8n8.x4.trans.shared.b16 {%0,%1,%2,%3}, [%4];"
                 : "=r"(r[0]), "=r"(r[1]), "=r"(r[2]), "=r"(r[3])
                 : "r"(smem_addr));
}
__device__ __forceinline__ uint32_t pack_half2(float lo, float hi) {
    const __half2 h = __floats2half2_rn(lo, hi);
    return *reinterpret_cast<const uint32_t*>(&h);
}

__device__ __forceinline__ bool elect_one() {
    uint32_t pred;
    asm volatile(
            "{\n\t.reg .pred p;\n\t"
            "elect.sync _|p, 0xffffffff;\n\t"
            "selp.u32 %0, 1, 0, p;\n\t}"
            : "=r"(pred));
    return pred != 0;
}

__device__ __forceinline__ uint32_t sw128_offset(int row, int chunk16) {
    return (uint32_t)(row * 128 + ((chunk16 ^ (row & 7)) << 4));
}

}

CUtensorMap make_tmap_2d(const void* base, uint64_t inner, uint64_t outer, uint64_t outer_stride_bytes, uint32_t box_inner,
                         uint32_t box_outer, uint32_t elem_bytes = 2);
CUtensorMap make_tmap_3d(const void* base, uint64_t d0, uint64_t d1, uint64_t d2, uint64_t s1_bytes, uint64_t s2_bytes,
                         uint32_t b0, uint32_t b1, uint32_t b2, uint32_t elem_bytes = 2);

}
```

### dorado_b200/lib.py

```python
from __future__ import annotations

import ctypes as C
import pathlib
import subprocess

import numpy as np

from .config import BasecallModelConfig

HERE = pathlib.Path(__file__).resolve().parent
import os as _os
LIB_PATH = pathlib.Path(_os.environ["B200CALL_LIB"]) if _os.environ.get("B200CALL_LIB") else HERE / "libb200call.so"

B200_OK, B200_ERR_INVALID, B200_ERR_CUDA, B200_ERR_UNSUPPORTED, B200_ERR_INTERNAL = 0, -1, -2, -3, -4


class B200Error(RuntimeError):
    def __init__(self, status, msg):
        super().__init__(f"b200call error {status}: {msg}")
        self.status = status


class ConvDesc(C.Structure):
    _fields_ = [(n, C.c_int32) for n in ("insize", "size", "winlen", "stride", "activation")]


class ModelDesc(C.Structure):
    _fields_ = [
        ("model_type", C.c_int32), ("num_convs", C.c_int32), ("convs", ConvDesc * 8),
        ("state_len", C.c_int32), ("outsize", C.c_int32), ("stride", C.c_int32), ("clamp", C.c_int32),
        ("qscale", C.c_float), ("qbias", C.c_float),
        ("lstm_size", C.c_int32), ("lstm_layers", C.c_int32), ("linear_bias", C.c_int32),
        ("out_features", C.c_int32), ("crf_scale", C.c_float),
        ("d_model", C.c_int32), ("nhead", C.c_int32), ("dim_feedforward", C.c_int32), ("depth", C.c_int32),
        ("attn_window_upper", C.c_int32), ("attn_window_lower", C.c_int32),
        ("upsample_scale", C.c_int32), ("max_seq_len", C.c_int32),
        ("deepnorm_alpha", C.c_float), ("theta", C.c_float), ("tx_crf_scale", C.c_float),
        ("lstm_inner_dim", C.c_int32), ("tx_precision", C.c_int32), ("lstm_precision", C.c_int32),
    ]


PRECISIONS = {"fp16": (0, 0), "fp8_ffn": (1, 0), "int8_lstm": (0, 1)}


class Tensor(C.Structure):
    _fields_ = [("name", C.c_char_p), ("data", C.POINTER(C.c_float)), ("ndim", C.c_int32), ("dims", C.c_int64 * 4)]


class DecoderOptions(C.Structure):
    _fields_ = [("beam_width", C.c_int32), ("beam_cut", C.c_float), ("blank_score", C.c_float),
                ("q_shift", C.c_float), ("q_scale", C.c_float), ("temperature", C.c_float), ("move_pad", C.c_int32)]


class Result(C.Structure):
    _fields_ = [("moves", C.POINTER(C.c_uint8)), ("sequence", C.POINTER(C.c_char)), ("qstring", C.POINTER(C.c_char)),
                ("n_bases", C.POINTER(C.c_int32)), ("t_out", C.c_int32), ("num_chunks", C.c_int32),
                ("n_moves", C.POINTER(C.c_int32))]


class RawChunk(C.Structure):
    _fields_ = [("raw", C.c_void_p), ("num_samples", C.c_uint64), ("input_offset", C.c_uint64), ("shift", C.c_float),
                ("scale", C.c_float)]


class CalledChunk(C.Structure):
    _fields_ = [("input_offset", C.c_uint64), ("raw_chunk_size", C.c_uint64), ("moves", C.c_void_p),
                ("n_moves", C.c_uint64), ("sequence", C.c_void_p), ("qstring", C.c_void_p), ("n_bases", C.c_uint64)]


class ModBaseDesc(C.Structure):
    _fields_ = [("sig_convs", ConvDesc * 3), ("seq_convs", ConvDesc * 2), ("merge_conv", ConvDesc),
                ("lstm_size", C.c_int32), ("num_out", C.c_int32), ("upsample_scale", C.c_int32),
                ("kmer_len", C.c_int32), ("chunk_size", C.c_int32)]


class Stats(C.Structure):
    _fields_ = [("batches_called", C.c_int64), ("model_decode_ms", C.c_double), ("h2d_ms", C.c_double),
                ("d2h_ms", C.c_double), ("gpu_launches", C.c_int64), ("arena_bytes", C.c_int64)]


EXPORTS = [
    "b200_last_error", "b200_version", "b200_device_count", "b200_default_decoder_options", "b200_engine_create", "b200_engine_create_sized",
    "b200_engine_destroy", "b200_engine_get_stats", "b200_runner_create", "b200_runner_destroy",
    "b200_runner_set_decoder_options", "b200_runner_batch_size", "b200_runner_chunk_size", "b200_runner_out_len",
    "b200_runner_accept_chunk_f16", "b200_runner_accept_chunk_f32", "b200_runner_input", "b200_runner_call_chunks",
    "b200_runner_upload", "b200_runner_step_device", "b200_runners_step_device", "b200_runner_forward_scores", "b200_runner_profile", "b200_runner_plan_info", "b200_runner_debug_read_workspace", "b200_decode_scores",
    "b200_test_gemm", "b200_test_gemm_fp8", "b200_test_gemm_s8", "b200_test_quantize_rows", "b200_test_to_e4m3", "b200_test_remove_bits", "b200_test_attention", "b200_generate_chunks", "b200_stitch_chunks", "b200_runner_accept_raw_chunk",
    "b200_runner_debug_read_input", "b200_engine_runner_bytes", "b200_engine_benchmark_batch_sizes",
    "b200_select_batch_size", "b200_generate_variable_chunks", "b200_engine_terminate", "b200_engine_restart",
    "b200_engine_set_low_latency", "b200_engine_is_low_latency", "b200_engine_batch_timeouts_ms",
    "b200_engine_set_num_runners", "b200_engine_num_runners",
    "b200_pool_create", "b200_pool_create_sized", "b200_pool_destroy", "b200_pool_num_runners", "b200_pool_runner", "b200_pool_out_len",
    "b200_pool_runner_info", "b200_pool_call_chunks", "b200_runner_variable_chunk_sizes",
    "b200_runner_accept_chunk_var_f16", "b200_chunk_benchmarks_lookup", "b200_engine_gpu_name",
    "b200_modbase_engine_create", "b200_modbase_engine_destroy", "b200_modbase_runner_create", "b200_modbase_runner_destroy",
    "b200_modbase_runner_batch_size", "b200_modbase_runner_sig_len", "b200_modbase_runner_seq_len",
    "b200_modbase_runner_out_len", "b200_modbase_runner_num_out", "b200_modbase_runner_accept_chunk",
    "b200_modbase_runner_call_chunks", "b200_modbase_runner_profile", "b200_modbase_runner_debug_read_workspace",
]

_lib = None


def build_library(verbose: bool = False) -> None:
    subprocess.run(["make", "-j8", "-C", str(HERE / "csrc")], check=True,
                   stdout=None if verbose else subprocess.DEVNULL)


def load_library() -> C.CDLL:
    global _lib
    if _lib is not None:
        return _lib
    if not LIB_PATH.exists():
        raise FileNotFoundError(f"{LIB_PATH} is missing: run `python -c 'import __graft_entry__ as g; g.build()'`; "
                                "there is no CPU fallback")
    lib = C.CDLL(str(LIB_PATH))
    vp, i32, f32 = C.c_void_p, C.c_int32, C.c_float
    lib.b200_last_error.restype = C.c_char_p
    lib.b200_version.restype = C.c_char_p
    lib.b200_default_decoder_options.argtypes = [C.POINTER(DecoderOptions)]
    lib.b200_pool_create.argtypes = [C.POINTER(ModelDesc), C.POINTER(Tensor), i32, C.POINTER(i32), i32, i32, i32, i32,
                                     C.POINTER(vp)]
    lib.b200_pool_create_sized.argtypes = [C.POINTER(ModelDesc), C.c_size_t, C.POINTER(Tensor), i32, C.POINTER(i32), i32, i32, i32,
                                           i32, C.POINTER(vp)]
    lib.b200_pool_destroy.argtypes = [vp]
    lib.b200_pool_num_runners.argtypes = [vp]
    lib.b200_pool_out_len.argtypes = [vp]
    lib.b200_pool_runner.argtypes = [vp, i32]
    lib.b200_pool_runner.restype = vp
    lib.b200_pool_runner_info.argtypes = [vp, i32, C.POINTER(i32), C.POINTER(C.c_int64)]
    lib.b200_pool_call_chunks.argtypes = [vp, vp, C.c_int64, vp, vp, vp, vp, C.POINTER(C.c_double)]
    lib.b200_chunk_benchmarks_lookup.argtypes = [C.c_char_p, C.c_char_p, C.POINTER(i32), C.POINTER(f32), i32, C.POINTER(i32)]
    lib.b200_engine_gpu_name.argtypes = [vp, C.c_char_p, C.c_uint64]
    lib.b200_runner_variable_chunk_sizes.argtypes = [vp]
    lib.b200_runner_variable_chunk_sizes.restype = i32
    lib.b200_runner_accept_chunk_var_f16.argtypes = [vp, i32, vp, C.c_int64]
    lib.b200_engine_terminate.argtypes = [vp]
    lib.b200_engine_restart.argtypes = [vp]
    lib.b200_engine_set_low_latency.argtypes = [vp, i32]
    lib.b200_engine_set_num_runners.argtypes = [vp, i32]
    lib.b200_engine_num_runners.argtypes = [vp]
    lib.b200_engine_num_runners.restype = i32
    lib.b200_engine_is_low_latency.argtypes = [vp]
    lib.b200_engine_is_low_latency.restype = i32
    lib.b200_engine_batch_timeouts_ms.argtypes = [vp, C.POINTER(i32), C.POINTER(i32)]
    lib.b200_engine_create.argtypes = [C.POINTER(ModelDesc), C.POINTER(Tensor), i32, i32, C.POINTER(vp)]
    lib.b200_engine_create_sized.argtypes = [C.POINTER(ModelDesc), C.c_size_t, C.POINTER(Tensor), i32, i32, C.POINTER(vp)]
    lib.b200_engine_destroy.argtypes = [vp]
    lib.b200_engine_get_stats.argtypes = [vp, C.POINTER(Stats)]
    lib.b200_runner_create.argtypes = [vp, i32, i32, C.POINTER(vp)]
    lib.b200_runner_destroy.argtypes = [vp]
    lib.b200_runner_set_decoder_options.argtypes = [vp, C.POINTER(DecoderOptions)]
    for fn in ("b200_runner_batch_size", "b200_runner_chunk_size", "b200_runner_out_len"):
        getattr(lib, fn).argtypes = [vp]
        getattr(lib, fn).restype = i32
    lib.b200_runner_accept_chunk_f16.argtypes = [vp, i32, vp, C.c_int64]
    lib.b200_runner_accept_chunk_f32.argtypes = [vp, i32, vp, C.c_int64]
    lib.b200_runner_input.argtypes = [vp]
    lib.b200_runner_input.restype = C.POINTER(C.c_uint16)
    lib.b200_runner_call_chunks.argtypes = [vp, i32, C.POINTER(Result)]
    lib.b200_runner_upload.argtypes = [vp]
    lib.b200_runner_step_device.argtypes = [vp, i32, i32, C.POINTER(f32), C.POINTER(f32), C.POINTER(f32)]
    lib.b200_runners_step_device.argtypes = [C.POINTER(vp), i32, i32, i32, C.POINTER(f32)]
    lib.b200_runner_forward_scores.argtypes = [vp, i32, vp]
    lib.b200_decode_scores.argtypes = [i32, vp, i32, i32, i32, f32, C.POINTER(DecoderOptions), vp, vp, vp, vp]
    lib.b200_runner_profile.argtypes = [vp, i32, C.c_char_p, C.c_uint64]
    lib.b200_runner_plan_info.argtypes = [vp, C.c_char_p, C.c_uint64]
    lib.b200_runner_debug_read_workspace.argtypes = [vp, C.c_uint64, C.c_uint64, vp]
    lib.b200_test_gemm.argtypes = [i32, vp, vp, vp, i32, i32, i32, i32, vp]
    lib.b200_test_attention.argtypes = [i32, vp, i32, i32, i32, i32, i32, vp]
    lib.b200_test_gemm_fp8.argtypes = [i32, vp, vp, i32, i32, i32, i32, vp, f32, vp]
    lib.b200_test_gemm_s8.argtypes = [i32, vp, vp, vp, vp, i32, i32, i32, i32, vp]
    lib.b200_test_quantize_rows.argtypes = [vp, i32, i32, vp, vp]
    lib.b200_test_to_e4m3.argtypes = [vp, C.c_int64, vp]
    lib.b200_test_remove_bits.argtypes = [vp, C.c_int64, i32, vp]
    u64 = C.c_uint64
    lib.b200_generate_chunks.argtypes = [u64, u64, u64, u64, C.POINTER(u64), u64, C.POINTER(u64)]
    lib.b200_generate_variable_chunks.argtypes = [u64, u64, u64, u64, C.POINTER(u64), u64, C.POINTER(u64)]
    lib.b200_stitch_chunks.argtypes = [C.POINTER(CalledChunk), u64, u64, i32, vp, vp, vp, C.POINTER(u64), C.POINTER(u64)]
    lib.b200_runner_accept_raw_chunk.argtypes = [vp, i32, C.POINTER(RawChunk)]
    lib.b200_runner_debug_read_input.argtypes = [vp, i32, vp]
    lib.b200_engine_runner_bytes.argtypes = [vp, i32, i32, C.POINTER(u64)]
    lib.b200_engine_benchmark_batch_sizes.argtypes = [vp, i32, i32, i32, C.POINTER(i32), C.POINTER(f32), i32, C.POINTER(i32)]
    lib.b200_select_batch_size.argtypes = [C.POINTER(i32), C.POINTER(f32), i32, i32, i32, f32, C.POINTER(i32)]
    lib.b200_modbase_engine_create.argtypes = [C.POINTER(ModBaseDesc), C.POINTER(Tensor), i32, i32, C.POINTER(vp)]
    lib.b200_modbase_engine_destroy.argtypes = [vp]
    lib.b200_modbase_runner_create.argtypes = [vp, i32, C.POINTER(vp)]
    lib.b200_modbase_runner_destroy.argtypes = [vp]
    for fn in ("batch_size", "sig_len", "seq_len", "out_len", "num_out"):
        getattr(lib, "b200_modbase_runner_" + fn).argtypes = [vp]
        getattr(lib, "b200_modbase_runner_" + fn).restype = i32
    lib.b200_modbase_runner_accept_chunk.argtypes = [vp, i32, vp, C.c_int64, vp, C.c_int64]
    lib.b200_modbase_runner_call_chunks.argtypes = [vp, i32, C.POINTER(C.POINTER(C.c_uint16))]
    lib.b200_modbase_runner_profile.argtypes = [vp, C.c_char_p, C.c_uint64]
    lib.b200_modbase_runner_debug_read_workspace.argtypes = [vp, C.c_uint64, C.c_uint64, vp]
    _lib = lib
    return lib


def check(status: int) -> None:
    if status != B200_OK:
        raise B200Error(status, load_library().b200_last_error().decode())


def model_desc_from_config(cfg: BasecallModelConfig, precision: str = "fp16") -> ModelDesc:
    if precision not in PRECISIONS:
        raise ValueError(f"precision must be one of {sorted(PRECISIONS)}, got {precision!r}")
    d = ModelDesc()
    d.tx_precision, d.lstm_precision = PRECISIONS[precision]
    d.model_type = 1 if cfg.is_tx_model else 0
    d.num_convs = len(cfg.convs)
    for i, c in enumerate(cfg.convs):
        d.convs[i] = ConvDesc(c.insize, c.size, c.winlen, c.stride, c.activation)
    d.state_len, d.outsize, d.stride, d.clamp = cfg.state_len, cfg.outsize, cfg.stride, int(cfg.clamp)
    d.qscale, d.qbias = cfg.qscale, cfg.qbias
    d.lstm_size, d.lstm_layers = cfg.lstm_size, cfg.lstm_layers
    d.lstm_inner_dim = cfg.lstm_inner_dim or 0
    d.linear_bias, d.out_features, d.crf_scale = int(cfg.bias), cfg.out_features or 0, cfg.scale
    if cfg.tx:
        t = cfg.tx
        d.d_model, d.nhead, d.dim_feedforward, d.depth = t.d_model, t.nhead, t.dim_feedforward, t.depth
        d.attn_window_upper, d.attn_window_lower = t.attn_window
        d.upsample_scale, d.max_seq_len = t.upsample_scale, t.max_seq_len
        d.deepnorm_alpha, d.theta, d.tx_crf_scale = t.deepnorm_alpha, t.theta, t.crf_scale
    return d


def modbase_desc_from_config(cfg) -> ModBaseDesc:
    if len(cfg.modules.signal_convs) != 3 or len(cfg.modules.sequence_convs) != 2 or len(cfg.modules.lstms) != 2:
        raise ValueError("ModBaseConvLSTMV3Model expects 3 signal convolutions, 2 sequence convolutions and 2 lstms")
    d = ModBaseDesc()
    conv = lambda c: ConvDesc(c.insize, c.size, c.winlen, c.stride, c.activation)
    for i, c in enumerate(cfg.modules.signal_convs):
        d.sig_convs[i] = conv(c)
    for i, c in enumerate(cfg.modules.sequence_convs):
        d.seq_convs[i] = conv(c)
    d.merge_conv = conv(cfg.modules.merge_conv)
    d.lstm_size, d.num_out, d.upsample_scale = cfg.lstm_size, cfg.num_out, cfg.upsample_scale
    d.kmer_len, d.chunk_size = cfg.kmer_len, cfg.chunk_size
    return d


def default_decoder_options() -> DecoderOptions:
    o = DecoderOptions()
    load_library().b200_default_decoder_options(C.byref(o))
    return o


def decode_scores(scores: np.ndarray, clamp_val: float = 0.0, opts: DecoderOptions | None = None, device: int = 0):
    lib = load_library()
    assert scores.dtype == np.float16 and scores.ndim == 3
    s = np.ascontiguousarray(scores)
    N, T, Cc = s.shape
    opts = opts or default_decoder_options()
    moves = np.zeros((N, T), np.uint8)
    seq = np.zeros((N, T), np.uint8)
    qstr = np.zeros((N, T), np.uint8)
    nb = np.zeros(N, np.int32)
    check(lib.b200_decode_scores(device, s.ctypes.data, N, T, Cc, clamp_val, C.byref(opts), moves.ctypes.data,
                                 seq.ctypes.data, qstr.ctypes.data, nb.ctypes.data))
    return moves, seq, qstr, nb


def test_gemm(a: np.ndarray, b: np.ndarray, bias: np.ndarray | None, activation: int = -1, device: int = 0):
    lib = load_library()
    a = np.ascontiguousarray(a, np.float16)
    b = np.ascontiguousarray(b, np.float16)
    M, K = a.shape
    N = b.shape[0]
    c = np.empty((M, N // 2 if activation == 4 else N), np.float16)
    bias_p = None
    if bias is not None:
        bias = np.ascontiguousarray(bias, np.float32)
        bias_p = bias.ctypes.data
    check(lib.b200_test_gemm(device, a.ctypes.data, b.ctypes.data, bias_p, M, N, K, activation, c.ctypes.data))
    return c


def test_gemm_fp8(a: np.ndarray, b: np.ndarray, activation: int = -1, residual: np.ndarray | None = None,
                  alpha: float = 0.0, device: int = 0):
    lib = load_library()
    a = np.ascontiguousarray(a, np.uint8)
    b = np.ascontiguousarray(b, np.uint8)
    M, K = a.shape
    N = b.shape[0]
    c = np.empty((M, N // 2), np.uint8) if activation == 4 else np.empty((M, N), np.float16)
    res_p = None
    if residual is not None:
        residual = np.ascontiguousarray(residual, np.float16)
        assert residual.shape == (M, N)
        res_p = residual.ctypes.data
    check(lib.b200_test_gemm_fp8(device, a.ctypes.data, b.ctypes.data, M, N, K, activation, res_p, alpha, c.ctypes.data))
    return c


def test_gemm_s8(a: np.ndarray, b: np.ndarray, col_scale: np.ndarray, bias: np.ndarray | None = None, activation: int = -1,
                 device: int = 0):
    lib = load_library()
    a = np.ascontiguousarray(a, np.int8)
    b = np.ascontiguousarray(b, np.int8)
    M, K = a.shape
    N = b.shape[0]
    col_scale = np.ascontiguousarray(col_scale, np.float32)
    assert col_scale.shape == (N,)
    bias_p = None
    if bias is not None:
        bias = np.ascontiguousarray(bias, np.float32)
        bias_p = bias.ctypes.data
    c = np.empty((M, N), np.float16)
    check(lib.b200_test_gemm_s8(device, a.ctypes.data, b.ctypes.data, col_scale.ctypes.data, bias_p, M, N, K, activation,
                                c.ctypes.data))
    return c


def quantize_rows(w: np.ndarray):
    h = np.ascontiguousarray(w, np.float16)
    q = np.empty(h.shape, np.int8)
    scale = np.empty(h.shape[0], np.float16)
    check(load_library().b200_test_quantize_rows(h.ctypes.data, h.shape[0], h.shape[1], q.ctypes.data, scale.ctypes.data))
    return q, scale


def to_e4m3(x: np.ndarray) -> np.ndarray:
    h = np.ascontiguousarray(x, np.float16)
    out = np.empty(h.shape, np.uint8)
    check(load_library().b200_test_to_e4m3(h.ctypes.data, h.size, out.ctypes.data))
    return out


def remove_bits(x: np.ndarray, bits: int = 4) -> np.ndarray:
    h = np.ascontiguousarray(x, np.float16)
    out = np.empty(h.shape, np.float16)
    check(load_library().b200_test_remove_bits(h.ctypes.data, h.size, bits, out.ctypes.data))
    return out


def test_attention(qkv: np.ndarray, win_upper: int, win_lower: int, device: int = 0):
    lib = load_library()
    qkv = np.ascontiguousarray(qkv, np.float16)
    N, T, three, H, D = qkv.shape
    assert three == 3 and D == 64
    out = np.empty((N, T, H * 64), np.float16)
    check(lib.b200_test_attention(device, qkv.ctypes.data, N, T, H, win_upper, win_lower, out.ctypes.data))
    return out
```

### include/b200call.h

```cpp
#ifndef B200CALL_H
#define B200CALL_H

#include <stddef.h>
#include <stdint.h>

#ifdef __cplusplus
extern "C" {
#endif

#define B200_API __attribute__((visibility("default")))

typedef enum b200_status {
    B200_OK = 0,
    B200_ERR_INVALID = -1,
    B200_ERR_CUDA = -2,
    B200_ERR_UNSUPPORTED = -3,
    B200_ERR_INTERNAL = -4
} b200_status;

enum { B200_ACT_SWISH = 0, B200_ACT_SWISH_CLAMP = 1, B200_ACT_TANH = 2 };
enum { B200_MODEL_LSTM = 0, B200_MODEL_TX = 1 };
enum { B200_TX_FP16 = 0, B200_TX_FP8_FFN = 1 };
enum { B200_LSTM_FP16 = 0, B200_LSTM_INT8 = 1 };

typedef struct b200_conv_desc {
    int32_t insize, size, winlen, stride, activation;
} b200_conv_desc;

typedef struct b200_model_desc {
    int32_t model_type;
    int32_t num_convs;
    b200_conv_desc convs[8];
    int32_t state_len;
    int32_t outsize;
    int32_t stride;
    int32_t clamp;
    float qscale, qbias;
    int32_t lstm_size, lstm_layers;
    int32_t linear_bias;
    int32_t out_features;
    float crf_scale;
    int32_t d_model, nhead, dim_feedforward, depth;
    int32_t attn_window_upper, attn_window_lower;
    int32_t upsample_scale, max_seq_len;
    float deepnorm_alpha, theta, tx_crf_scale;
    int32_t lstm_inner_dim;
    int32_t tx_precision;
    int32_t lstm_precision;
} b200_model_desc;

typedef struct b200_tensor {
    const char* name;
    const float* data;
    int32_t ndim;
    int64_t dims[4];
} b200_tensor;

typedef struct b200_decoder_options {
    int32_t beam_width;
    float beam_cut;
    float blank_score;
    float q_shift;
    float q_scale;
    float temperature;
    int32_t move_pad;
} b200_decoder_options;

typedef struct b200_result {
    const uint8_t* moves;
    const char* sequence;
    const char* qstring;
    const int32_t* n_bases;
    int32_t t_out;
    int32_t num_chunks;
    const int32_t* n_moves;
} b200_result;

typedef struct b200_stats {
    int64_t batches_called;
    double model_decode_ms;
    double h2d_ms, d2h_ms;
    int64_t gpu_launches;
    int64_t arena_bytes;
} b200_stats;

typedef struct b200_engine b200_engine;
typedef struct b200_runner b200_runner;

B200_API const char* b200_last_error(void);
B200_API const char* b200_version(void);
B200_API int b200_device_count(void);

B200_API void b200_default_decoder_options(b200_decoder_options* opts);

B200_API int b200_engine_create_sized(const b200_model_desc* desc,
                                      size_t desc_size,
                                      const b200_tensor* tensors,
                                      int32_t num_tensors,
                                      int32_t device,
                                      b200_engine** out);
B200_API int b200_engine_create(const b200_model_desc* desc,
                                const b200_tensor* tensors,
                                int32_t num_tensors,
                                int32_t device,
                                b200_engine** out);
#define b200_engine_create(desc, tensors, num_tensors, device, out) \
    b200_engine_create_sized((desc), sizeof(b200_model_desc), (tensors), (num_tensors), (device), (out))
B200_API int b200_engine_destroy(b200_engine* engine);
B200_API int b200_engine_get_stats(const b200_engine* engine, b200_stats* out);

B200_API int b200_engine_terminate(b200_engine* engine);
B200_API int b200_engine_restart(b200_engine* engine);
B200_API int b200_engine_set_low_latency(b200_engine* engine, int32_t on);
B200_API int32_t b200_engine_is_low_latency(const b200_engine* engine);
B200_API int b200_engine_batch_timeouts_ms(const b200_engine* engine, int32_t* first_chunk_ms, int32_t* last_chunk_ms);
B200_API int b200_engine_set_num_runners(b200_engine* engine, int32_t num_runners);
B200_API int32_t b200_engine_num_runners(const b200_engine* engine);

B200_API int b200_runner_create(b200_engine* engine, int32_t batch_size, int32_t chunk_size, b200_runner** out);
B200_API int b200_runner_destroy(b200_runner* runner);
B200_API int b200_runner_set_decoder_options(b200_runner* runner, const b200_decoder_options* opts);
B200_API int32_t b200_runner_batch_size(const b200_runner* runner);
B200_API int32_t b200_runner_chunk_size(const b200_runner* runner);
B200_API int32_t b200_runner_out_len(const b200_runner* runner);

B200_API int b200_runner_accept_chunk_f16(b200_runner* runner, int32_t chunk_idx, const uint16_t* samples, int64_t len);
B200_API int b200_runner_accept_chunk_f32(b200_runner* runner, int32_t chunk_idx, const float* samples, int64_t len);
B200_API int32_t b200_runner_variable_chunk_sizes(const b200_runner* runner);
B200_API int b200_runner_accept_chunk_var_f16(b200_runner* runner, int32_t chunk_idx, const uint16_t* samples, int64_t len);

B200_API uint16_t* b200_runner_input(b200_runner* runner);

B200_API int b200_runner_call_chunks(b200_runner* runner, int32_t num_chunks, b200_result* out);

B200_API int b200_runner_upload(b200_runner* runner);
B200_API int b200_runner_step_device(b200_runner* runner, int32_t num_chunks, int32_t iters, float* total_ms,
                                     float* forward_ms, float* decode_ms);
B200_API int b200_runners_step_device(b200_runner** runners, int32_t n_runners, int32_t num_chunks, int32_t iters,
                                      float* total_ms);

B200_API int b200_generate_chunks(uint64_t num_samples,
                                  uint64_t chunk_size,
                                  uint64_t stride,
                                  uint64_t overlap,
                                  uint64_t* offsets,
                                  uint64_t capacity,
                                  uint64_t* count);

B200_API int b200_generate_variable_chunks(uint64_t num_samples,
                                           uint64_t chunk_size,
                                           uint64_t stride,
                                           uint64_t overlap,
                                           uint64_t* intervals,
                                           uint64_t capacity,
                                           uint64_t* count);

typedef struct b200_raw_chunk {
    const int16_t* raw;
    uint64_t num_samples;
    uint64_t input_offset;
    float shift, scale;
} b200_raw_chunk;
B200_API int b200_runner_accept_raw_chunk(b200_runner* runner, int32_t chunk_idx, const b200_raw_chunk* chunk);
B200_API int b200_runner_debug_read_input(b200_runner* runner, int32_t num_chunks, uint16_t* input_out);

typedef struct b200_called_chunk {
    uint64_t input_offset;
    uint64_t raw_chunk_size;
    const uint8_t* moves;
    uint64_t n_moves;
    const char* sequence;
    const char* qstring;
    uint64_t n_bases;
} b200_called_chunk;
B200_API int b200_stitch_chunks(const b200_called_chunk* chunks,
                                uint64_t n_chunks,
                                uint64_t raw_samples,
                                int32_t stride,
                                uint8_t* moves_out,
                                char* sequence_out,
                                char* qstring_out,
                                uint64_t* n_moves_out,
                                uint64_t* n_bases_out);

B200_API int b200_engine_runner_bytes(b200_engine* engine, int32_t batch_size, int32_t chunk_size, uint64_t* bytes);
B200_API int b200_engine_benchmark_batch_sizes(b200_engine* engine,
                                               int32_t chunk_size,
                                               int32_t granularity,
                                               int32_t max_batch_size,
                                               int32_t* batch_sizes,
                                               float* ms_per_chunk,
                                               int32_t capacity,
                                               int32_t* count);
B200_API int b200_chunk_benchmarks_lookup(const char* gpu_name,
                                          const char* model_name,
                                          int32_t* batch_sizes,
                                          float* ms_per_chunk,
                                          int32_t capacity,
                                          int32_t* count);
B200_API int b200_engine_gpu_name(const b200_engine* engine, char* buf, uint64_t buf_len);

B200_API int b200_select_batch_size(const int32_t* batch_sizes,
                                    const float* ms_per_chunk,
                                    int32_t count,
                                    int32_t max_batch_size,
                                    int32_t granularity,
                                    float time_penalty,
                                    int32_t* selected);

typedef struct b200_pool b200_pool;
B200_API int b200_pool_create_sized(const b200_model_desc* desc,
                                    size_t desc_size,
                                    const b200_tensor* tensors,
                                    int32_t num_tensors,
                                    const int32_t* devices,
                                    int32_t num_devices,
                                    int32_t runners_per_device,
                                    int32_t batch_size,
                                    int32_t chunk_size,
                                    b200_pool** out);
B200_API int b200_pool_create(const b200_model_desc* desc,
                              const b200_tensor* tensors,
                              int32_t num_tensors,
                              const int32_t* devices,
                              int32_t num_devices,
                              int32_t runners_per_device,
                              int32_t batch_size,
                              int32_t chunk_size,
                              b200_pool** out);
#define b200_pool_create(desc, tensors, num_tensors, devices, num_devices, runners_per_device, batch_size, chunk_size, out) \
    b200_pool_create_sized((desc), sizeof(b200_model_desc), (tensors), (num_tensors), (devices), (num_devices),          \
                           (runners_per_device), (batch_size), (chunk_size), (out))
B200_API int b200_pool_destroy(b200_pool* pool);
B200_API int32_t b200_pool_num_runners(const b200_pool* pool);
B200_API b200_runner* b200_pool_runner(b200_pool* pool, int32_t index);
B200_API int32_t b200_pool_out_len(const b200_pool* pool);
B200_API int b200_pool_runner_info(const b200_pool* pool, int32_t index, int32_t* numa_node, int64_t* batches);
B200_API int b200_pool_call_chunks(b200_pool* pool,
                                   const uint16_t* chunks,
                                   int64_t num_chunks,
                                   uint8_t* moves,
                                   char* sequence,
                                   char* qstring,
                                   int32_t* n_bases,
                                   double* seconds);

B200_API int b200_runner_forward_scores(b200_runner* runner, int32_t num_chunks, uint16_t* scores_out );
B200_API int b200_decode_scores(int32_t device,
                                const uint16_t* scores ,
                                int32_t N,
                                int32_t T,
                                int32_t C,
                                float clamp_val,
                                const b200_decoder_options* opts,
                                uint8_t* moves,
                                char* sequence,
                                char* qstring,
                                int32_t* n_bases);

B200_API int b200_runner_profile(b200_runner* runner, int32_t num_chunks, char* buf, uint64_t buf_len);

B200_API int b200_runner_plan_info(const b200_runner* runner, char* buf, uint64_t buf_len);

B200_API int b200_runner_debug_read_workspace(b200_runner* runner, uint64_t offset, uint64_t bytes, void* dst);

typedef struct b200_modbase_desc {
    b200_conv_desc sig_convs[3];
    b200_conv_desc seq_convs[2];
    b200_conv_desc merge_conv;
    int32_t lstm_size;
    int32_t num_out;
    int32_t upsample_scale;
    int32_t kmer_len;
    int32_t chunk_size;
} b200_modbase_desc;

typedef struct b200_modbase_engine b200_modbase_engine;
typedef struct b200_modbase_runner b200_modbase_runner;

B200_API int b200_modbase_engine_create(const b200_modbase_desc* desc,
                                        const b200_tensor* tensors,
                                        int32_t num_tensors,
                                        int32_t device,
                                        b200_modbase_engine** out);
B200_API int b200_modbase_engine_destroy(b200_modbase_engine* engine);

B200_API int b200_modbase_runner_create(b200_modbase_engine* engine, int32_t batch_size, b200_modbase_runner** out);
B200_API int b200_modbase_runner_destroy(b200_modbase_runner* runner);
B200_API int32_t b200_modbase_runner_batch_size(const b200_modbase_runner* runner);
B200_API int32_t b200_modbase_runner_sig_len(const b200_modbase_runner* runner);
B200_API int32_t b200_modbase_runner_seq_len(const b200_modbase_runner* runner);
B200_API int32_t b200_modbase_runner_out_len(const b200_modbase_runner* runner);
B200_API int32_t b200_modbase_runner_num_out(const b200_modbase_runner* runner);

B200_API int b200_modbase_runner_accept_chunk(b200_modbase_runner* runner,
                                              int32_t idx,
                                              const uint16_t* signal,
                                              int64_t sig_len,
                                              const int8_t* kmers,
                                              int64_t kmer_elems);
B200_API int b200_modbase_runner_call_chunks(b200_modbase_runner* runner, int32_t num_chunks, const uint16_t** probs);
B200_API int b200_modbase_runner_profile(b200_modbase_runner* runner, char* buf, uint64_t buf_len);
B200_API int b200_modbase_runner_debug_read_workspace(b200_modbase_runner* runner, uint64_t offset, uint64_t bytes, void* dst);

B200_API int b200_test_gemm_fp8(int32_t device, const uint8_t* a, const uint8_t* b, int32_t M, int32_t N, int32_t K,
                                int32_t activation, const uint16_t* residual, float alpha, void* c);
B200_API int b200_test_gemm_s8(int32_t device, const int8_t* a, const int8_t* b, const float* col_scale, const float* bias,
                               int32_t M, int32_t N, int32_t K, int32_t activation, uint16_t* c);
B200_API int b200_test_quantize_rows(const uint16_t* f16, int32_t rows, int32_t cols, int8_t* q, uint16_t* scale);
B200_API int b200_test_to_e4m3(const uint16_t* f16, int64_t n, uint8_t* out);
B200_API int b200_test_remove_bits(const uint16_t* f16, int64_t n, int32_t bits, uint16_t* out);
B200_API int b200_test_gemm(int32_t device, const uint16_t* a , const uint16_t* b ,
                            const float* bias , int32_t M, int32_t N, int32_t K, int32_t activation,
                            uint16_t* c );
B200_API int b200_test_attention(int32_t device, const uint16_t* qkv , int32_t N, int32_t T,
                                 int32_t H, int32_t win_upper, int32_t win_lower, uint16_t* out );

#ifdef __cplusplus
}
#endif
#endif
```

Baseline: 1.099 billion.

## Stage GEMM epilogue through swizzled shared memory and store tiles via TMA

The GEMM epilogue can now write results into a swizzled shared-memory staging buffer, double-buffered per tile, and issue TMA bulk tensor stores instead of scattered per-thread global writes, whenever the output layout allows it. The wgmma calls are also merged into a single wide m64nN instruction per k-step instead of several n32 instructions. These aim to cut uncoalesced store traffic and instruction overhead. In exchange the kernel uses more shared memory and adds named-barrier synchronisation and bulk-group waits, and test entry points are added.

Result: no change. 1.103 billion (median of 6 runs) (+0.4%).

```diff
diff --git a/dorado_b200/csrc/capi.cu b/dorado_b200/csrc/capi.cu
--- a/dorado_b200/csrc/capi.cu
+++ b/dorado_b200/csrc/capi.cu
@@ -416,6 +416,25 @@
     });
 }
 
+int b200_test_gemm_store_map(int32_t batches, int32_t rows_per_batch, int32_t N, int32_t q8_store, int64_t out_m1,
+                              int64_t out_s0, int64_t out_s1, int64_t* info, uint32_t* slices) {
+    return guarded([&] {
+        if (batches < 1 || rows_per_batch < 1 || N < 32 || !info || !slices) throw std::invalid_argument("b200_test_gemm_store_map: bad argument");
+        b200::test_gemm_store_map_host(batches, rows_per_batch, N, q8_store, out_m1, out_s0, out_s1, info, slices);
+    });
+}
+
+int b200_test_gemm_strided(int32_t device, const uint16_t* a, int64_t a_elems, int32_t batches, int32_t rows_per_batch,
+                           int64_t a_row_stride, int64_t a_batch_stride, const uint16_t* w, const float* bias, int32_t N, int32_t K,
+                           int32_t activation, int32_t q8_store, int64_t out_m1, int64_t out_s0, int64_t out_s1, int64_t out_bytes,
+                           int32_t max_ctas, void* out, int32_t* staged) {
+    return guarded([&] {
+        if (!a || !w || !out || !staged || a_elems < 1 || out_bytes < 1) throw std::invalid_argument("b200_test_gemm_strided: bad argument");
+        b200::test_gemm_strided_host(device, a, a_elems, batches, rows_per_batch, a_row_stride, a_batch_stride, w, bias, N, K,
+                                     activation, q8_store, out_m1, out_s0, out_s1, out_bytes, max_ctas, out, staged);
+    });
+}
+
 int b200_test_quantize_rows(const uint16_t* f16, int32_t rows, int32_t cols, int8_t* q, uint16_t* scale) {
     return guarded([&] {
         if (rows < 1 || cols < 1 || !f16 || !q || !scale) throw std::invalid_argument("b200_test_quantize_rows: bad argument");
diff --git a/dorado_b200/csrc/engine.h b/dorado_b200/csrc/engine.h
--- a/dorado_b200/csrc/engine.h
+++ b/dorado_b200/csrc/engine.h
@@ -329,6 +329,12 @@
 
 void test_gemm_s8_host(int device, const int8_t* a, const int8_t* b, const float* col_scale, const float* bias, int M, int N,
                        int K, int activation, uint16_t* c);
+void test_gemm_store_map_host(int batches, int rows_per_batch, int N, int q8_store, int64_t out_m1, int64_t out_s0, int64_t out_s1,
+                              int64_t* info, uint32_t* slices);
+void test_gemm_strided_host(int device, const uint16_t* a, int64_t a_elems, int batches, int rows_per_batch, int64_t a_row_stride,
+                            int64_t a_batch_stride, const uint16_t* w, const float* bias, int N, int K, int activation, int q8_store,
+                            int64_t out_m1, int64_t out_s0, int64_t out_s1, int64_t out_bytes, int max_ctas, void* out,
+                            int32_t* staged);
 void quantize_rows_f16(const uint16_t* w16, int rows, int cols, int8_t* q, uint16_t* scale16);
 float int8_row_inv(uint16_t scale16);
 
diff --git a/dorado_b200/csrc/gemm.cu b/dorado_b200/csrc/gemm.cu
--- a/dorado_b200/csrc/gemm.cu
+++ b/dorado_b200/csrc/gemm.cu
@@ -42,6 +42,8 @@
     int a_ss_parts, res_ss_parts;
     float norm_inv_dim, norm_eps;
     const float* col_scale;
+    int staged;
+    uint32_t store_m1;
 };
 
 __device__ __forceinline__ bool gemm_tile_at(const GemmKernelParams& p, int i, int* mt, int* nt) {
@@ -65,38 +67,45 @@
     else return v;
 }
 
-template <int NCH, bool FP8, typename Acc>
-__device__ __forceinline__ void wgmma_k_block(Acc (&acc)[BN_MAX / 32][16], uint64_t adesc, uint64_t bdesc, bool accumulate) {
+template <int BN, bool FP8, typename Acc>
+__device__ __forceinline__ void wgmma_k_block(Acc (&acc)[BN_MAX / 2], uint64_t adesc, uint64_t bdesc, bool accumulate) {
 #pragma unroll
     for (int k = 0; k < 4; ++k) {
-#pragma unroll
-        for (int c = 0; c < NCH; ++c) {
-            if constexpr (std::is_same_v<Acc, int32_t>) {
-                tc::wgmma_m64n32k32_s8(acc[c], adesc + (uint64_t)(2 * k), bdesc + (uint64_t)(c * 256 + 2 * k), accumulate || k != 0);
-            } else if constexpr (FP8) {
-                tc::wgmma_m64n32k32_e4m3(acc[c], adesc + (uint64_t)(2 * k), bdesc + (uint64_t)(c * 256 + 2 * k), accumulate || k != 0);
-            } else {
-                tc::wgmma_m64n32k16(acc[c], adesc + (uint64_t)(2 * k), bdesc + (uint64_t)(c * 256 + 2 * k), accumulate || k != 0);
-            }
-        }
-    }
+        if constexpr (std::is_same_v<Acc, int32_t>) {
+            tc::wgmma_m64nNk32_s8<BN>(acc, adesc + (uint64_t)(2 * k), bdesc + (uint64_t)(2 * k), accumulate || k != 0);
+        } else if constexpr (FP8) {
+            tc::wgmma_m64nNk32_e4m3<BN>(acc, adesc + (uint64_t)(2 * k), bdesc + (uint64_t)(2 * k), accumulate || k != 0);
+        } else {
+            tc::wgmma_m64nNk16<BN>(acc, adesc + (uint64_t)(2 * k), bdesc + (uint64_t)(2 * k), accumulate || k != 0);
+        }
+    }
+}
+
+template <int ROW>
+__device__ __forceinline__ uint32_t staging_offset(int row, int b) {
+    const uint32_t o = (uint32_t)(row * ROW + b);
+    return o ^ (((o >> 7) & (ROW / 16 - 1)) << 4);
 }
 
 template <int ACT, bool FP8, int Q8 = GEMM_Q8_NONE>
 __global__ void __launch_bounds__(GEMM_THREADS, 1) gemm_wgmma_kernel(const __grid_constant__ CUtensorMap tma_a,
                                                                      const __grid_constant__ CUtensorMap tma_w,
+                                                                     const __grid_constant__ CUtensorMap tma_out,
                                                                      const GemmKernelParams p) {
     constexpr bool S8 = Q8 == GEMM_Q8_OPERANDS;
     constexpr int KB = FP8 || S8 ? BK8 : BK;
+    constexpr int SROW = Q8 == GEMM_Q8_STORE ? 32 : 64;
     using Acc = std::conditional_t<S8, int32_t, float>;
     extern __shared__ __align__(1024) uint8_t smem_raw[];
     uint8_t* smem = smem_raw + ((1024u - (tc::smem_u32(smem_raw) & 1023u)) & 1023u);
     const uint32_t a_bytes = BM * 128;
     const uint32_t w_bytes = (uint32_t)p.bn * 128;
     const uint32_t stage_bytes = a_bytes + w_bytes;
-    uint64_t* full = reinterpret_cast<uint64_t*>(smem + STAGES * stage_bytes);
+    const int nch = p.bn / 32;
+    const uint32_t box_bytes = 64 * SROW;
+    uint8_t* staging = smem + STAGES * stage_bytes;
+    uint64_t* full = reinterpret_cast<uint64_t*>(staging + (p.staged ? 4 * nch * box_bytes : 0));
     uint64_t* empty = full + STAGES;
-    const int nch = p.bn / 32;
 
     if (threadIdx.x == 0) {
         for (int s = 0; s < STAGES; ++s) {
@@ -106,6 +115,7 @@
         tc::fence_barrier_init();
         tc::prefetch_tmap(&tma_a);
         tc::prefetch_tmap(&tma_w);
+        if (p.staged) tc::prefetch_tmap(&tma_out);
     }
     __syncthreads();
     const int wg = threadIdx.x >> 7;
@@ -143,7 +153,7 @@
     uint32_t ph = 0;
     int mt, nt;
     for (int ti = 0; gemm_tile_at(p, ti, &mt, &nt); ++ti) {
-        Acc acc[BN_MAX / 32][16];
+        Acc acc[BN_MAX / 2];
         int prev = -1;
         for (int kb = 0; kb < p.num_k_blocks; ++kb) {
             tc::mbar_wait_silent(&full[s], ph);
@@ -152,10 +162,10 @@
             const uint64_t bdesc = tc::wgmma_desc_sw128(st + a_bytes);
             tc::wgmma_fence();
             switch (nch) {
-                case 1: wgmma_k_block<1, FP8>(acc, adesc, bdesc, kb != 0); break;
-                case 2: wgmma_k_block<2, FP8>(acc, adesc, bdesc, kb != 0); break;
-                case 3: wgmma_k_block<3, FP8>(acc, adesc, bdesc, kb != 0); break;
-                default: wgmma_k_block<4, FP8>(acc, adesc, bdesc, kb != 0); break;
+                case 1: wgmma_k_block<32, FP8>(acc, adesc, bdesc, kb != 0); break;
+                case 2: wgmma_k_block<64, FP8>(acc, adesc, bdesc, kb != 0); break;
+                case 3: wgmma_k_block<96, FP8>(acc, adesc, bdesc, kb != 0); break;
+                default: wgmma_k_block<128, FP8>(acc, adesc, bdesc, kb != 0); break;
             }
             tc::wgmma_commit();
             tc::wgmma_wait<1>();
@@ -196,6 +206,12 @@
             }
             row_bias[h] = (p.bias && p.bias_per_row && valid[h]) ? __ldg(p.bias + g[h]) : 0.0f;
         }
+        uint8_t* stg = staging + (uint32_t)(2 * half + (ti & 1)) * (uint32_t)nch * box_bytes;
+        const int srow = rloc - 64 * half;
+        if (p.staged) {
+            if (t == 0) tc::bulk_wait_group_read<1>();
+            named_bar_sync(1 + half, 128);
+        }
         if constexpr (S8) {
 #pragma unroll
             for (int c = 0; c < BN_MAX / 32; ++c) {
@@ -209,9 +225,14 @@
 #pragma unroll
                     for (int h = 0; h < 2; ++h) {
                         if (!valid[h]) continue;
-                        const float v0 = fmaf((float)acc[c][4 * j + 2 * h], sc.x, b2.x);
-                        const float v1 = fmaf((float)acc[c][4 * j + 2 * h + 1], sc.y, b2.y);
-                        *reinterpret_cast<__half2*>(p.out + off[h] + nc) = __floats2half2_rn(act_apply<ACT>(v0), act_apply<ACT>(v1));
+                        const float v0 = fmaf((float)acc[16 * c + 4 * j + 2 * h], sc.x, b2.x);
+                        const float v1 = fmaf((float)acc[16 * c + 4 * j + 2 * h + 1], sc.y, b2.y);
+                        const __half2 o = __floats2half2_rn(act_apply<ACT>(v0), act_apply<ACT>(v1));
+                        if (p.staged) {
+                            *reinterpret_cast<__half2*>(stg + c * box_bytes + staging_offset<SROW>(srow + 8 * h, 2 * (8 * j + 2 * quad))) = o;
+                        } else {
+                            *reinterpret_cast<__half2*>(p.out + off[h] + nc) = o;
+                        }
                     }
                 }
             }
@@ -228,8 +249,8 @@
 #pragma unroll
                         for (int j = 0; j < 4; ++j) {
                             const int col = 8 * j + 2 * quad;
-                            float a0 = acc[c][4 * j + 2 * h] * r_a[h], a1 = acc[c][4 * j + 2 * h + 1] * r_a[h];
-                            float b0 = acc[c + 1][4 * j + 2 * h] * r_a[h], b1 = acc[c + 1][4 * j + 2 * h + 1] * r_a[h];
+                            float a0 = acc[16 * c + 4 * j + 2 * h] * r_a[h], a1 = acc[16 * c + 4 * j + 2 * h + 1] * r_a[h];
+                            float b0 = acc[16 * c + 16 + 4 * j + 2 * h] * r_a[h], b1 = acc[16 * c + 16 + 4 * j + 2 * h + 1] * r_a[h];
                             if (rot) {
                                 const float4 cs = __ldg(tab + (size_t)(col / 2) * p.rope_stride);
                                 const float x0 = cs.x * a0 - cs.y * b0, y0 = cs.y * a0 + cs.x * b0;
@@ -261,8 +282,8 @@
 #pragma unroll
                     for (int h = 0; h < 2; ++h) {
                         if (!valid[h]) continue;
-                        float v0 = acc[c][4 * j + 2 * h] * r_a[h] + b2.x + row_bias[h];
-                        float v1 = acc[c][4 * j + 2 * h + 1] * r_a[h] + b2.y + row_bias[h];
+                        float v0 = acc[16 * c + 4 * j + 2 * h] * r_a[h] + b2.x + row_bias[h];
+                        float v1 = acc[16 * c + 4 * j + 2 * h + 1] * r_a[h] + b2.y + row_bias[h];
                         if constexpr (ACT == GEMM_ACT_SWIGLU) {
                             if constexpr (FP8) {
                                 reinterpret_cast<uint8_t*>(p.out)[off[h] + nc / 2] = (uint8_t)tc::cvt_e4m3x2(v0 * swish_fast(v1), 0.0f);
@@ -286,8 +307,14 @@
                             if constexpr (Q8 == GEMM_Q8_STORE) {
                                 const int32_t q0 = tc::cvt_rni_sat_s8(kInt8ActScale * act_apply<ACT>(v0));
                                 const int32_t q1 = tc::cvt_rni_sat_s8(kInt8ActScale * act_apply<ACT>(v1));
-                                *reinterpret_cast<uint16_t*>(reinterpret_cast<int8_t*>(p.out) + off[h] + coff) =
-                                        (uint16_t)((q0 & 0xff) | ((q1 & 0xff) << 8));
+                                const uint16_t q = (uint16_t)((q0 & 0xff) | ((q1 & 0xff) << 8));
+                                if (p.staged) {
+                                    *reinterpret_cast<uint16_t*>(stg + c * box_bytes + staging_offset<SROW>(srow + 8 * h, 8 * j + 2 * quad)) = q;
+                                } else {
+                                    *reinterpret_cast<uint16_t*>(reinterpret_cast<int8_t*>(p.out) + off[h] + coff) = q;
+                                }
+                            } else if (p.staged) {
+                                *reinterpret_cast<__half2*>(stg + c * box_bytes + staging_offset<SROW>(srow + 8 * h, 2 * (8 * j + 2 * quad))) = o;
                             } else {
                                 *reinterpret_cast<__half2*>(p.out + off[h] + coff) = o;
                             }
@@ -308,7 +335,21 @@
                 }
             }
         }
-    }
+        if (p.staged) {
+            tc::fence_proxy_async_smem();
+            named_bar_sync(1 + half, 128);
+            if (t == 0) {
+                const int row0 = r0 + 64 * half;
+                if (row0 < p.rows_per_batch) {
+                    uint32_t brow, bslice;
+                    gemm_store_box((uint32_t)(batch * p.rows_per_batch + row0), p.store_m1, &brow, &bslice);
+                    for (int c = 0; c < nch; ++c) tc::tma_store_3d(&tma_out, stg + c * box_bytes, n0 + 32 * c, (int)brow, (int)bslice);
+                }
+                tc::bulk_commit_group();
+            }
+        }
+    }
+    if (p.staged && t == 0) tc::bulk_wait_group<0>();
 }
 
 using EncodeFn = CUresult (*)(CUtensorMap*, CUtensorMapDataType, cuuint32_t, void*, const cuuint64_t*, const cuuint64_t*,
@@ -371,6 +412,40 @@
     return 0;
 }
 
+GemmStoreMap gemm_store_map(const GemmDesc& d) {
+    GemmStoreMap m;
+    m.elem_bytes = d.q8 == GEMM_Q8_STORE ? 1 : 2;
+    if (d.act == GEMM_ACT_SWIGLU || d.act == GEMM_ACT_ROPE || d.out_col_m1 != 0) return m;
+    const int64_t eb = m.elem_bytes;
+    const int64_t rows = (int64_t)d.batches * d.rows_per_batch;
+    const int64_t m1 = d.out_m1 == 1 ? d.rows_per_batch : d.out_m1;
+    const int64_t s_row = d.out_m1 == 1 ? d.out_s0 : d.out_s1;
+    const int64_t s_slice = d.out_m1 == 1 ? d.rows_per_batch * d.out_s0 : d.out_s0;
+    const auto aligned = [](int64_t bytes) { return bytes > 0 && bytes % 16 == 0 && bytes < (1LL << 40); };
+    if (m1 < 1 || d.rows_per_batch % m1 != 0 || (m1 != d.rows_per_batch && m1 % 64 != 0) || !aligned(s_row * eb) || !aligned(s_slice * eb) ||
+        reinterpret_cast<uintptr_t>(d.out) % 16 != 0) {
+        return m;
+    }
+    m.staged = 1;
+    m.dims[0] = (uint64_t)d.N;
+    m.dims[1] = (uint64_t)m1;
+    m.dims[2] = (uint64_t)(rows / m1);
+    m.strides[0] = (uint64_t)(s_row * eb);
+    m.strides[1] = (uint64_t)(s_slice * eb);
+    m.box[0] = 32;
+    m.box[1] = 64;
+    m.box[2] = 1;
+    return m;
+}
+
+static int plan_bn(const GemmDesc& d) {
+    int bn = pick_bn(d.N);
+    if (bn > 0 && d.N / bn < 2 && d.N >= 128 && (long long)d.batches * ((d.rows_per_batch + BM - 1) / BM) < kNumSMs / 2) {
+        bn = pick_bn(d.N / 2);
+    }
+    return bn;
+}
+
 int gemm_out_ss_parts(int N) {
     const int bn = pick_bn(N);
     if (bn <= 0) throw std::invalid_argument("gemm: N must be a multiple of 32");
@@ -404,10 +479,7 @@
     }
     GemmPlan p{};
     p.d = d;
-    p.bn = pick_bn(d.N);
-    if (d.N / p.bn < 2 && d.N >= 128 && (long long)d.batches * ((d.rows_per_batch + BM - 1) / BM) < kNumSMs / 2) {
-        p.bn = pick_bn(d.N / 2);
-    }
+    p.bn = plan_bn(d);
     if (p.bn == 0) throw std::invalid_argument("gemm: no valid tile width");
     if (d.out_ss) {
         if (p.bn != pick_bn(d.N) || p.bn / 32 != GEMM_PARTS || d.act == GEMM_ACT_SWIGLU || d.act == GEMM_ACT_ROPE) {
@@ -427,20 +499,30 @@
         throw std::invalid_argument("gemm: rows and output blocking must fit 32-bit index arithmetic");
     }
     p.grid = dim3((unsigned)(p.tiles_per_batch * d.batches), (unsigned)(d.N / p.bn), 1);
-    p.smem = (size_t)STAGES * ((size_t)BM * 128 + (size_t)p.bn * 128) + 256 + 1024;
+    p.store = gemm_store_map(d);
+    p.smem = (size_t)STAGES * ((size_t)BM * 128 + (size_t)p.bn * 128) + (p.store.staged ? (size_t)4 * 64 * p.bn * p.store.elem_bytes : 0) +
+             256 + 1024;
     if (p.smem > 227 * 1024) throw std::logic_error("gemm: shared-memory plan does not fit");
     const uint64_t batch_stride = d.batches > 1 ? (uint64_t)d.a_batch_stride * eb : (uint64_t)d.a_row_stride * eb * d.rows_per_batch;
     p.tma_a = make_tmap_3d(d.a, (uint64_t)(d.a_inner > 0 ? d.a_inner : d.K), (uint64_t)d.rows_per_batch, (uint64_t)d.batches, (uint64_t)d.a_row_stride * eb,
                            batch_stride, kb, BM, 1, eb);
     p.tma_w = make_tmap_2d(d.w, (uint64_t)d.K, (uint64_t)d.N, (uint64_t)d.K * eb, kb, (uint32_t)p.bn, eb);
+    if (p.store.staged) {
+        const cuuint64_t sdims[3] = {p.store.dims[0], p.store.dims[1], p.store.dims[2]};
+        const cuuint64_t sstrides[2] = {p.store.strides[0], p.store.strides[1]};
+        const cuuint32_t sbox[3] = {p.store.box[0], p.store.box[1], p.store.box[2]};
+        p.tma_out = encode(d.out, 3, sdims, sstrides, sbox,
+                           p.store.elem_bytes == 2 ? CU_TENSOR_MAP_SWIZZLE_64B : CU_TENSOR_MAP_SWIZZLE_32B, (uint32_t)p.store.elem_bytes);
+    } else {
+        std::memset(&p.tma_out, 0, sizeof(p.tma_out));
+    }
     return p;
 }
 
 template <int ACT, bool FP8 = false, int Q8 = GEMM_Q8_NONE>
-static void launch_gemm(int grid, size_t smem, cudaStream_t stream, const CUtensorMap& a, const CUtensorMap& w,
-                        const GemmKernelParams& k) {
+static void launch_gemm(int grid, size_t smem, cudaStream_t stream, const GemmPlan& p, const GemmKernelParams& k) {
     ensure_dynamic_smem(gemm_wgmma_kernel<ACT, FP8, Q8>, 227 * 1024);
-    gemm_wgmma_kernel<ACT, FP8, Q8><<<grid, GEMM_THREADS, smem, stream>>>(a, w, k);
+    gemm_wgmma_kernel<ACT, FP8, Q8><<<grid, GEMM_THREADS, smem, stream>>>(p.tma_a, p.tma_w, p.tma_out, k);
 }
 
 void run_gemm(const GemmPlan& p, cudaStream_t stream) {
@@ -477,29 +559,31 @@
     k.norm_inv_dim = p.d.norm_dim > 0 ? 1.0f / (float)p.d.norm_dim : 0.0f;
     k.norm_eps = p.d.norm_eps;
     k.col_scale = p.d.col_scale;
+    k.staged = p.store.staged;
+    k.store_m1 = (uint32_t)p.store.dims[1];
     const int max_ctas = p.d.max_ctas > 0 && p.d.max_ctas < kNumSMs ? p.d.max_ctas : kNumSMs;
     const int grid = k.num_tiles < max_ctas ? k.num_tiles : max_ctas;
     if (p.d.fp8) {
-        if (p.d.act == GEMM_ACT_SWIGLU) launch_gemm<GEMM_ACT_SWIGLU, true>(grid, p.smem, stream, p.tma_a, p.tma_w, k);
-        else launch_gemm<GEMM_ACT_NONE, true>(grid, p.smem, stream, p.tma_a, p.tma_w, k);
+        if (p.d.act == GEMM_ACT_SWIGLU) launch_gemm<GEMM_ACT_SWIGLU, true>(grid, p.smem, stream, p, k);
+        else launch_gemm<GEMM_ACT_NONE, true>(grid, p.smem, stream, p, k);
         B200_CUDA(cudaGetLastError());
         return;
     }
     if (p.d.q8 != GEMM_Q8_NONE) {
-        if (p.d.q8 == GEMM_Q8_STORE) launch_gemm<GEMM_ACT_TANH, false, GEMM_Q8_STORE>(grid, p.smem, stream, p.tma_a, p.tma_w, k);
-        else if (p.d.act == GEMM_ACT_TANH_X5) launch_gemm<GEMM_ACT_TANH_X5, false, GEMM_Q8_OPERANDS>(grid, p.smem, stream, p.tma_a, p.tma_w, k);
-        else launch_gemm<GEMM_ACT_NONE, false, GEMM_Q8_OPERANDS>(grid, p.smem, stream, p.tma_a, p.tma_w, k);
+        if (p.d.q8 == GEMM_Q8_STORE) launch_gemm<GEMM_ACT_TANH, false, GEMM_Q8_STORE>(grid, p.smem, stream, p, k);
+        else if (p.d.act == GEMM_ACT_TANH_X5) launch_gemm<GEMM_ACT_TANH_X5, false, GEMM_Q8_OPERANDS>(grid, p.smem, stream, p, k);
+        else launch_gemm<GEMM_ACT_NONE, false, GEMM_Q8_OPERANDS>(grid, p.smem, stream, p, k);
         B200_CUDA(cudaGetLastError());
         return;
     }
     switch (p.d.act) {
-        case GEMM_ACT_NONE: launch_gemm<GEMM_ACT_NONE>(grid, p.smem, stream, p.tma_a, p.tma_w, k); break;
-        case GEMM_ACT_SWISH: launch_gemm<GEMM_ACT_SWISH>(grid, p.smem, stream, p.tma_a, p.tma_w, k); break;
-        case GEMM_ACT_SWISH_CLAMP: launch_gemm<GEMM_ACT_SWISH_CLAMP>(grid, p.smem, stream, p.tma_a, p.tma_w, k); break;
-        case GEMM_ACT_TANH: launch_gemm<GEMM_ACT_TANH>(grid, p.smem, stream, p.tma_a, p.tma_w, k); break;
-        case GEMM_ACT_TANH_X5: launch_gemm<GEMM_ACT_TANH_X5>(grid, p.smem, stream, p.tma_a, p.tma_w, k); break;
-        case GEMM_ACT_SWIGLU: launch_gemm<GEMM_ACT_SWIGLU>(grid, p.smem, stream, p.tma_a, p.tma_w, k); break;
-        case GEMM_ACT_ROPE: launch_gemm<GEMM_ACT_ROPE>(grid, p.smem, stream, p.tma_a, p.tma_w, k); break;
+        case GEMM_ACT_NONE: launch_gemm<GEMM_ACT_NONE>(grid, p.smem, stream, p, k); break;
+        case GEMM_ACT_SWISH: launch_gemm<GEMM_ACT_SWISH>(grid, p.smem, stream, p, k); break;
+        case GEMM_ACT_SWISH_CLAMP: launch_gemm<GEMM_ACT_SWISH_CLAMP>(grid, p.smem, stream, p, k); break;
+        case GEMM_ACT_TANH: launch_gemm<GEMM_ACT_TANH>(grid, p.smem, stream, p, k); break;
+        case GEMM_ACT_TANH_X5: launch_gemm<GEMM_ACT_TANH_X5>(grid, p.smem, stream, p, k); break;
+        case GEMM_ACT_SWIGLU: launch_gemm<GEMM_ACT_SWIGLU>(grid, p.smem, stream, p, k); break;
+        case GEMM_ACT_ROPE: launch_gemm<GEMM_ACT_ROPE>(grid, p.smem, stream, p, k); break;
         default: throw std::invalid_argument("gemm: unknown activation");
     }
     B200_CUDA(cudaGetLastError());
@@ -638,4 +722,80 @@
     B200_CUDA(cudaMemcpy(c, d_c, (size_t)M * N * 2, cudaMemcpyDeviceToHost));
 }
 
-}
+void test_gemm_store_map_host(int batches, int rows_per_batch, int N, int q8_store, int64_t out_m1, int64_t out_s0, int64_t out_s1,
+                              int64_t* info, uint32_t* slices) {
+    GemmDesc d{};
+    d.batches = batches;
+    d.rows_per_batch = rows_per_batch;
+    d.N = N;
+    d.K = BK;
+    d.act = q8_store ? GEMM_ACT_TANH : GEMM_ACT_NONE;
+    d.q8 = q8_store ? GEMM_Q8_STORE : GEMM_Q8_NONE;
+    d.out = reinterpret_cast<void*>(uintptr_t{1} << 20);
+    d.out_m1 = out_m1;
+    d.out_s0 = out_s0;
+    d.out_s1 = out_s1;
+    const GemmStoreMap m = gemm_store_map(d);
+    info[0] = m.staged;
+    info[1] = m.elem_bytes;
+    for (int i = 0; i < 3; ++i) info[2 + i] = (int64_t)m.dims[i];
+    for (int i = 0; i < 2; ++i) info[5 + i] = (int64_t)m.strides[i];
+    for (int i = 0; i < 3; ++i) info[7 + i] = m.box[i];
+    info[10] = plan_bn(d);
+    const int tiles_per_batch = (rows_per_batch + BM - 1) / BM;
+    for (int mt = 0; mt < batches * tiles_per_batch; ++mt) {
+        const int batch = mt / tiles_per_batch, r0 = (mt % tiles_per_batch) * BM;
+        for (int half = 0; half < 2; ++half) {
+            uint32_t* box = slices + (mt * 2 + half) * 2;
+            const int row0 = r0 + 64 * half;
+            box[0] = box[1] = UINT32_MAX;
+            if (!m.staged || row0 >= rows_per_batch) continue;
+            gemm_store_box((uint32_t)(batch * rows_per_batch + row0), (uint32_t)m.dims[1], &box[0], &box[1]);
+        }
+    }
+}
+
+void test_gemm_strided_host(int device, const uint16_t* a, int64_t a_elems, int batches, int rows_per_batch, int64_t a_row_stride,
+                            int64_t a_batch_stride, const uint16_t* w, const float* bias, int N, int K, int activation, int q8_store,
+                            int64_t out_m1, int64_t out_s0, int64_t out_s1, int64_t out_bytes, int max_ctas, void* out,
+                            int32_t* staged) {
+    require_sm90(device);
+    __half *d_a = nullptr, *d_w = nullptr;
+    float* d_bias = nullptr;
+    void* d_out = nullptr;
+    Arena arena;
+    arena.allocate([&](Bump& b) {
+        d_a = b.take<__half>((size_t)a_elems * 2);
+        d_w = b.take<__half>((size_t)N * K * 2);
+        d_bias = b.take<float>((size_t)N * 4);
+        d_out = b.take((size_t)out_bytes);
+    });
+    B200_CUDA(cudaMemcpy(d_a, a, (size_t)a_elems * 2, cudaMemcpyHostToDevice));
+    B200_CUDA(cudaMemcpy(d_w, w, (size_t)N * K * 2, cudaMemcpyHostToDevice));
+    if (bias) B200_CUDA(cudaMemcpy(d_bias, bias, (size_t)N * 4, cudaMemcpyHostToDevice));
+    B200_CUDA(cudaMemcpy(d_out, out, (size_t)out_bytes, cudaMemcpyHostToDevice));
+    GemmDesc d{};
+    d.a = d_a;
+    d.batches = batches;
+    d.rows_per_batch = rows_per_batch;
+    d.a_row_stride = a_row_stride;
+    d.a_batch_stride = a_batch_stride;
+    d.w = d_w;
+    d.N = N;
+    d.K = K;
+    d.bias = bias ? d_bias : nullptr;
+    d.act = activation;
+    d.q8 = q8_store ? GEMM_Q8_STORE : GEMM_Q8_NONE;
+    d.out = d_out;
+    d.out_m1 = out_m1;
+    d.out_s0 = out_s0;
+    d.out_s1 = out_s1;
+    d.max_ctas = max_ctas;
+    const GemmPlan plan = make_gemm_plan(d);
+    run_gemm(plan, nullptr);
+    B200_CUDA(cudaDeviceSynchronize());
+    B200_CUDA(cudaMemcpy(out, d_out, (size_t)out_bytes, cudaMemcpyDeviceToHost));
+    *staged = plan.store.staged;
+}
+
+}
diff --git a/dorado_b200/csrc/gemm.h b/dorado_b200/csrc/gemm.h
--- a/dorado_b200/csrc/gemm.h
+++ b/dorado_b200/csrc/gemm.h
@@ -60,9 +60,24 @@
     float norm_eps = 1e-5f;
 };
 
+struct GemmStoreMap {
+    int staged = 0;
+    int elem_bytes = 2;
+    uint64_t dims[3] = {};
+    uint64_t strides[2] = {};
+    uint32_t box[3] = {};
+};
+GemmStoreMap gemm_store_map(const GemmDesc& d);
+
+__host__ __device__ inline void gemm_store_box(uint32_t g0, uint32_t m1, uint32_t* row, uint32_t* slice) {
+    *row = g0 % m1;
+    *slice = g0 / m1;
+}
+
 struct GemmPlan {
-    CUtensorMap tma_a, tma_w;
+    CUtensorMap tma_a, tma_w, tma_out;
     GemmDesc d;
+    GemmStoreMap store;
     int bn = 128;
     int tiles_per_batch = 0;
     dim3 grid;
diff --git a/dorado_b200/csrc/lstm_model.cu b/dorado_b200/csrc/lstm_model.cu
--- a/dorado_b200/csrc/lstm_model.cu
+++ b/dorado_b200/csrc/lstm_model.cu
@@ -1445,6 +1445,7 @@
         if (plan->conv12_tc) ensure_dynamic_smem(conv12_tc_kernel, C12_SMEM);
     }
 
+    const int share_cap = num_runners_hint >= 3 ? 2 * kNumSMs / num_runners_hint : 0;
     {
         GemmDesc g{};
         g.a = x2;
@@ -1462,6 +1463,7 @@
         g.out_m1 = T_out;
         g.out_s0 = C;
         g.out_s1 = (int64_t)Np * C;
+        g.max_ctas = share_cap;
         plan->conv3 = make_gemm_plan(g);
     }
     plan->variable = variable_chunk_sizes();
@@ -1489,6 +1491,7 @@
         g.K = Cp;
         g.a_inner = C;
         g.bias = bl1;
+        g.max_ctas = share_cap;
         if (int8) {
             g.q8 = GEMM_Q8_OPERANDS;
             g.w = wl1_8;
@@ -1516,6 +1519,7 @@
             g2.out_m1 = Np;
             g2.out_s0 = desc.outsize;
             g2.out_s1 = (int64_t)T_out * desc.outsize;
+            g2.max_ctas = share_cap;
             plan->linear2 = make_gemm_plan(g2);
             plan->num_linear = 2;
         } else {
diff --git a/dorado_b200/csrc/tc.cuh b/dorado_b200/csrc/tc.cuh
--- a/dorado_b200/csrc/tc.cuh
+++ b/dorado_b200/csrc/tc.cuh
@@ -129,36 +129,189 @@
 __device__ __forceinline__ void wgmma_commit() { asm volatile("wgmma.commit_group.sync.aligned;" ::: "memory"); }
 template <int N>
 __device__ __forceinline__ void wgmma_wait() { asm volatile("wgmma.wait_group.sync.aligned %0;" ::"n"(N) : "memory"); }
-__device__ __forceinline__ void wgmma_m64n32k16(float* d, uint64_t adesc, uint64_t bdesc, bool accumulate) {
+template <int N>
+__device__ __forceinline__ void wgmma_m64nNk16(float* d, uint64_t adesc, uint64_t bdesc, bool accumulate);
+template <>
+__device__ __forceinline__ void wgmma_m64nNk16<32>(float* d, uint64_t adesc, uint64_t bdesc, bool accumulate) {
     asm volatile(
             "{\n\t.reg .pred p;\n\t"
             "setp.ne.b32 p, %18, 0;\n\t"
             "wgmma.mma_async.sync.aligned.m64n32k16.f32.f16.f16 "
             "{%0,%1,%2,%3,%4,%5,%6,%7,%8,%9,%10,%11,%12,%13,%14,%15}, %16, %17, p, 1, 1, 0, 0;\n\t}"
-            : "+f"(d[0]), "+f"(d[1]), "+f"(d[2]), "+f"(d[3]), "+f"(d[4]), "+f"(d[5]), "+f"(d[6]), "+f"(d[7]), "+f"(d[8]),
-              "+f"(d[9]), "+f"(d[10]), "+f"(d[11]), "+f"(d[12]), "+f"(d[13]), "+f"(d[14]), "+f"(d[15])
-            : "l"(adesc), "l"(bdesc), "r"((uint32_t)accumulate)
-            : "memory");
-}
-__device__ __forceinline__ void wgmma_m64n32k32_e4m3(float* d, uint64_t adesc, uint64_t bdesc, bool accumulate) {
+            : "+f"(d[0]), "+f"(d[1]), "+f"(d[2]), "+f"(d[3]), "+f"(d[4]), "+f"(d[5]), "+f"(d[6]), "+f"(d[7]),
+              "+f"(d[8]), "+f"(d[9]), "+f"(d[10]), "+f"(d[11]), "+f"(d[12]), "+f"(d[13]), "+f"(d[14]), "+f"(d[15])
+            : "l"(adesc), "l"(bdesc), "r"((uint32_t)accumulate)
+            : "memory");
+}
+template <>
+__device__ __forceinline__ void wgmma_m64nNk16<64>(float* d, uint64_t adesc, uint64_t bdesc, bool accumulate) {
+    asm volatile(
+            "{\n\t.reg .pred p;\n\t"
+            "setp.ne.b32 p, %34, 0;\n\t"
+            "wgmma.mma_async.sync.aligned.m64n64k16.f32.f16.f16 "
+            "{%0,%1,%2,%3,%4,%5,%6,%7,%8,%9,%10,%11,%12,%13,%14,%15,%16,%17,%18,%19,%20,%21,%22,%23,%24,%25,%26,%27,%28,%29,%30,%31}, %32, %33, p, 1, 1, 0, 0;\n\t}"
+            : "+f"(d[0]), "+f"(d[1]), "+f"(d[2]), "+f"(d[3]), "+f"(d[4]), "+f"(d[5]), "+f"(d[6]), "+f"(d[7]),
+              "+f"(d[8]), "+f"(d[9]), "+f"(d[10]), "+f"(d[11]), "+f"(d[12]), "+f"(d[13]), "+f"(d[14]), "+f"(d[15]),
+              "+f"(d[16]), "+f"(d[17]), "+f"(d[18]), "+f"(d[19]), "+f"(d[20]), "+f"(d[21]), "+f"(d[22]), "+f"(d[23]),
+              "+f"(d[24]), "+f"(d[25]), "+f"(d[26]), "+f"(d[27]), "+f"(d[28]), "+f"(d[29]), "+f"(d[30]), "+f"(d[31])
+            : "l"(adesc), "l"(bdesc), "r"((uint32_t)accumulate)
+            : "memory");
+}
+template <>
+__device__ __forceinline__ void wgmma_m64nNk16<96>(float* d, uint64_t adesc, uint64_t bdesc, bool accumulate) {
+    asm volatile(
+            "{\n\t.reg .pred p;\n\t"
+            "setp.ne.b32 p, %50, 0;\n\t"
+            "wgmma.mma_async.sync.aligned.m64n96k16.f32.f16.f16 "
+            "{%0,%1,%2,%3,%4,%5,%6,%7,%8,%9,%10,%11,%12,%13,%14,%15,%16,%17,%18,%19,%20,%21,%22,%23,%24,%25,%26,%27,%28,%29,%30,%31,%32,%33,%34,%35,%36,%37,%38,%39,%40,%41,%42,%43,%44,%45,%46,%47}, %48, %49, p, 1, 1, 0, 0;\n\t}"
+            : "+f"(d[0]), "+f"(d[1]), "+f"(d[2]), "+f"(d[3]), "+f"(d[4]), "+f"(d[5]), "+f"(d[6]), "+f"(d[7]),
+              "+f"(d[8]), "+f"(d[9]), "+f"(d[10]), "+f"(d[11]), "+f"(d[12]), "+f"(d[13]), "+f"(d[14]), "+f"(d[15]),
+              "+f"(d[16]), "+f"(d[17]), "+f"(d[18]), "+f"(d[19]), "+f"(d[20]), "+f"(d[21]), "+f"(d[22]), "+f"(d[23]),
+              "+f"(d[24]), "+f"(d[25]), "+f"(d[26]), "+f"(d[27]), "+f"(d[28]), "+f"(d[29]), "+f"(d[30]), "+f"(d[31]),
+              "+f"(d[32]), "+f"(d[33]), "+f"(d[34]), "+f"(d[35]), "+f"(d[36]), "+f"(d[37]), "+f"(d[38]), "+f"(d[39]),
+              "+f"(d[40]), "+f"(d[41]), "+f"(d[42]), "+f"(d[43]), "+f"(d[44]), "+f"(d[45]), "+f"(d[46]), "+f"(d[47])
+            : "l"(adesc), "l"(bdesc), "r"((uint32_t)accumulate)
+            : "memory");
+}
+template <>
+__device__ __forceinline__ void wgmma_m64nNk16<128>(float* d, uint64_t adesc, uint64_t bdesc, bool accumulate) {
+    asm volatile(
+            "{\n\t.reg .pred p;\n\t"
+            "setp.ne.b32 p, %66, 0;\n\t"
+            "wgmma.mma_async.sync.aligned.m64n128k16.f32.f16.f16 "
+            "{%0,%1,%2,%3,%4,%5,%6,%7,%8,%9,%10,%11,%12,%13,%14,%15,%16,%17,%18,%19,%20,%21,%22,%23,%24,%25,%26,%27,%28,%29,%30,%31,%32,%33,%34,%35,%36,%37,%38,%39,%40,%41,%42,%43,%44,%45,%46,%47,%48,%49,%50,%51,%52,%53,%54,%55,%56,%57,%58,%59,%60,%61,%62,%63}, %64, %65, p, 1, 1, 0, 0;\n\t}"
+            : "+f"(d[0]), "+f"(d[1]), "+f"(d[2]), "+f"(d[3]), "+f"(d[4]), "+f"(d[5]), "+f"(d[6]), "+f"(d[7]),
+              "+f"(d[8]), "+f"(d[9]), "+f"(d[10]), "+f"(d[11]), "+f"(d[12]), "+f"(d[13]), "+f"(d[14]), "+f"(d[15]),
+              "+f"(d[16]), "+f"(d[17]), "+f"(d[18]), "+f"(d[19]), "+f"(d[20]), "+f"(d[21]), "+f"(d[22]), "+f"(d[23]),
+              "+f"(d[24]), "+f"(d[25]), "+f"(d[26]), "+f"(d[27]), "+f"(d[28]), "+f"(d[29]), "+f"(d[30]), "+f"(d[31]),
+              "+f"(d[32]), "+f"(d[33]), "+f"(d[34]), "+f"(d[35]), "+f"(d[36]), "+f"(d[37]), "+f"(d[38]), "+f"(d[39]),
+              "+f"(d[40]), "+f"(d[41]), "+f"(d[42]), "+f"(d[43]), "+f"(d[44]), "+f"(d[45]), "+f"(d[46]), "+f"(d[47]),
+              "+f"(d[48]), "+f"(d[49]), "+f"(d[50]), "+f"(d[51]), "+f"(d[52]), "+f"(d[53]), "+f"(d[54]), "+f"(d[55]),
+              "+f"(d[56]), "+f"(d[57]), "+f"(d[58]), "+f"(d[59]), "+f"(d[60]), "+f"(d[61]), "+f"(d[62]), "+f"(d[63])
+            : "l"(adesc), "l"(bdesc), "r"((uint32_t)accumulate)
+            : "memory");
+}
+template <int N>
+__device__ __forceinline__ void wgmma_m64nNk32_e4m3(float* d, uint64_t adesc, uint64_t bdesc, bool accumulate);
+template <>
+__device__ __forceinline__ void wgmma_m64nNk32_e4m3<32>(float* d, uint64_t adesc, uint64_t bdesc, bool accumulate) {
     asm volatile(
             "{\n\t.reg .pred p;\n\t"
             "setp.ne.b32 p, %18, 0;\n\t"
             "wgmma.mma_async.sync.aligned.m64n32k32.f32.e4m3.e4m3 "
             "{%0,%1,%2,%3,%4,%5,%6,%7,%8,%9,%10,%11,%12,%13,%14,%15}, %16, %17, p, 1, 1;\n\t}"
-            : "+f"(d[0]), "+f"(d[1]), "+f"(d[2]), "+f"(d[3]), "+f"(d[4]), "+f"(d[5]), "+f"(d[6]), "+f"(d[7]), "+f"(d[8]),
-              "+f"(d[9]), "+f"(d[10]), "+f"(d[11]), "+f"(d[12]), "+f"(d[13]), "+f"(d[14]), "+f"(d[15])
-            : "l"(adesc), "l"(bdesc), "r"((uint32_t)accumulate)
-            : "memory");
-}
-__device__ __forceinline__ void wgmma_m64n32k32_s8(int32_t* d, uint64_t adesc, uint64_t bdesc, bool accumulate) {
+            : "+f"(d[0]), "+f"(d[1]), "+f"(d[2]), "+f"(d[3]), "+f"(d[4]), "+f"(d[5]), "+f"(d[6]), "+f"(d[7]),
+              "+f"(d[8]), "+f"(d[9]), "+f"(d[10]), "+f"(d[11]), "+f"(d[12]), "+f"(d[13]), "+f"(d[14]), "+f"(d[15])
+            : "l"(adesc), "l"(bdesc), "r"((uint32_t)accumulate)
+            : "memory");
+}
+template <>
+__device__ __forceinline__ void wgmma_m64nNk32_e4m3<64>(float* d, uint64_t adesc, uint64_t bdesc, bool accumulate) {
+    asm volatile(
+            "{\n\t.reg .pred p;\n\t"
+            "setp.ne.b32 p, %34, 0;\n\t"
+            "wgmma.mma_async.sync.aligned.m64n64k32.f32.e4m3.e4m3 "
+            "{%0,%1,%2,%3,%4,%5,%6,%7,%8,%9,%10,%11,%12,%13,%14,%15,%16,%17,%18,%19,%20,%21,%22,%23,%24,%25,%26,%27,%28,%29,%30,%31}, %32, %33, p, 1, 1;\n\t}"
+            : "+f"(d[0]), "+f"(d[1]), "+f"(d[2]), "+f"(d[3]), "+f"(d[4]), "+f"(d[5]), "+f"(d[6]), "+f"(d[7]),
+              "+f"(d[8]), "+f"(d[9]), "+f"(d[10]), "+f"(d[11]), "+f"(d[12]), "+f"(d[13]), "+f"(d[14]), "+f"(d[15]),
+              "+f"(d[16]), "+f"(d[17]), "+f"(d[18]), "+f"(d[19]), "+f"(d[20]), "+f"(d[21]), "+f"(d[22]), "+f"(d[23]),
+              "+f"(d[24]), "+f"(d[25]), "+f"(d[26]), "+f"(d[27]), "+f"(d[28]), "+f"(d[29]), "+f"(d[30]), "+f"(d[31])
+            : "l"(adesc), "l"(bdesc), "r"((uint32_t)accumulate)
+            : "memory");
+}
+template <>
+__device__ __forceinline__ void wgmma_m64nNk32_e4m3<96>(float* d, uint64_t adesc, uint64_t bdesc, bool accumulate) {
+    asm volatile(
+            "{\n\t.reg .pred p;\n\t"
+            "setp.ne.b32 p, %50, 0;\n\t"
+            "wgmma.mma_async.sync.aligned.m64n96k32.f32.e4m3.e4m3 "
+            "{%0,%1,%2,%3,%4,%5,%6,%7,%8,%9,%10,%11,%12,%13,%14,%15,%16,%17,%18,%19,%20,%21,%22,%23,%24,%25,%26,%27,%28,%29,%30,%31,%32,%33,%34,%35,%36,%37,%38,%39,%40,%41,%42,%43,%44,%45,%46,%47}, %48, %49, p, 1, 1;\n\t}"
+            : "+f"(d[0]), "+f"(d[1]), "+f"(d[2]), "+f"(d[3]), "+f"(d[4]), "+f"(d[5]), "+f"(d[6]), "+f"(d[7]),
+              "+f"(d[8]), "+f"(d[9]), "+f"(d[10]), "+f"(d[11]), "+f"(d[12]), "+f"(d[13]), "+f"(d[14]), "+f"(d[15]),
+              "+f"(d[16]), "+f"(d[17]), "+f"(d[18]), "+f"(d[19]), "+f"(d[20]), "+f"(d[21]), "+f"(d[22]), "+f"(d[23]),
+              "+f"(d[24]), "+f"(d[25]), "+f"(d[26]), "+f"(d[27]), "+f"(d[28]), "+f"(d[29]), "+f"(d[30]), "+f"(d[31]),
+              "+f"(d[32]), "+f"(d[33]), "+f"(d[34]), "+f"(d[35]), "+f"(d[36]), "+f"(d[37]), "+f"(d[38]), "+f"(d[39]),
+              "+f"(d[40]), "+f"(d[41]), "+f"(d[42]), "+f"(d[43]), "+f"(d[44]), "+f"(d[45]), "+f"(d[46]), "+f"(d[47])
+            : "l"(adesc), "l"(bdesc), "r"((uint32_t)accumulate)
+            : "memory");
+}
+template <>
+__device__ __forceinline__ void wgmma_m64nNk32_e4m3<128>(float* d, uint64_t adesc, uint64_t bdesc, bool accumulate) {
+    asm volatile(
+            "{\n\t.reg .pred p;\n\t"
+            "setp.ne.b32 p, %66, 0;\n\t"
+            "wgmma.mma_async.sync.aligned.m64n128k32.f32.e4m3.e4m3 "
+            "{%0,%1,%2,%3,%4,%5,%6,%7,%8,%9,%10,%11,%12,%13,%14,%15,%16,%17,%18,%19,%20,%21,%22,%23,%24,%25,%26,%27,%28,%29,%30,%31,%32,%33,%34,%35,%36,%37,%38,%39,%40,%41,%42,%43,%44,%45,%46,%47,%48,%49,%50,%51,%52,%53,%54,%55,%56,%57,%58,%59,%60,%61,%62,%63}, %64, %65, p, 1, 1;\n\t}"
+            : "+f"(d[0]), "+f"(d[1]), "+f"(d[2]), "+f"(d[3]), "+f"(d[4]), "+f"(d[5]), "+f"(d[6]), "+f"(d[7]),
+              "+f"(d[8]), "+f"(d[9]), "+f"(d[10]), "+f"(d[11]), "+f"(d[12]), "+f"(d[13]), "+f"(d[14]), "+f"(d[15]),
+              "+f"(d[16]), "+f"(d[17]), "+f"(d[18]), "+f"(d[19]), "+f"(d[20]), "+f"(d[21]), "+f"(d[22]), "+f"(d[23]),
+              "+f"(d[24]), "+f"(d[25]), "+f"(d[26]), "+f"(d[27]), "+f"(d[28]), "+f"(d[29]), "+f"(d[30]), "+f"(d[31]),
+              "+f"(d[32]), "+f"(d[33]), "+f"(d[34]), "+f"(d[35]), "+f"(d[36]), "+f"(d[37]), "+f"(d[38]), "+f"(d[39]),
+              "+f"(d[40]), "+f"(d[41]), "+f"(d[42]), "+f"(d[43]), "+f"(d[44]), "+f"(d[45]), "+f"(d[46]), "+f"(d[47]),
+              "+f"(d[48]), "+f"(d[49]), "+f"(d[50]), "+f"(d[51]), "+f"(d[52]), "+f"(d[53]), "+f"(d[54]), "+f"(d[55]),
+              "+f"(d[56]), "+f"(d[57]), "+f"(d[58]), "+f"(d[59]), "+f"(d[60]), "+f"(d[61]), "+f"(d[62]), "+f"(d[63])
+            : "l"(adesc), "l"(bdesc), "r"((uint32_t)accumulate)
+            : "memory");
+}
+template <int N>
+__device__ __forceinline__ void wgmma_m64nNk32_s8(int32_t* d, uint64_t adesc, uint64_t bdesc, bool accumulate);
+template <>
+__device__ __forceinline__ void wgmma_m64nNk32_s8<32>(int32_t* d, uint64_t adesc, uint64_t bdesc, bool accumulate) {
     asm volatile(
             "{\n\t.reg .pred p;\n\t"
             "setp.ne.b32 p, %18, 0;\n\t"
             "wgmma.mma_async.sync.aligned.m64n32k32.s32.s8.s8 "
             "{%0,%1,%2,%3,%4,%5,%6,%7,%8,%9,%10,%11,%12,%13,%14,%15}, %16, %17, p;\n\t}"
-            : "+r"(d[0]), "+r"(d[1]), "+r"(d[2]), "+r"(d[3]), "+r"(d[4]), "+r"(d[5]), "+r"(d[6]), "+r"(d[7]), "+r"(d[8]),
-              "+r"(d[9]), "+r"(d[10]), "+r"(d[11]), "+r"(d[12]), "+r"(d[13]), "+r"(d[14]), "+r"(d[15])
+            : "+r"(d[0]), "+r"(d[1]), "+r"(d[2]), "+r"(d[3]), "+r"(d[4]), "+r"(d[5]), "+r"(d[6]), "+r"(d[7]),
+              "+r"(d[8]), "+r"(d[9]), "+r"(d[10]), "+r"(d[11]), "+r"(d[12]), "+r"(d[13]), "+r"(d[14]), "+r"(d[15])
+            : "l"(adesc), "l"(bdesc), "r"((uint32_t)accumulate)
+            : "memory");
+}
+template <>
+__device__ __forceinline__ void wgmma_m64nNk32_s8<64>(int32_t* d, uint64_t adesc, uint64_t bdesc, bool accumulate) {
+    asm volatile(
+            "{\n\t.reg .pred p;\n\t"
+            "setp.ne.b32 p, %34, 0;\n\t"
+            "wgmma.mma_async.sync.aligned.m64n64k32.s32.s8.s8 "
+            "{%0,%1,%2,%3,%4,%5,%6,%7,%8,%9,%10,%11,%12,%13,%14,%15,%16,%17,%18,%19,%20,%21,%22,%23,%24,%25,%26,%27,%28,%29,%30,%31}, %32, %33, p;\n\t}"
+            : "+r"(d[0]), "+r"(d[1]), "+r"(d[2]), "+r"(d[3]), "+r"(d[4]), "+r"(d[5]), "+r"(d[6]), "+r"(d[7]),
+              "+r"(d[8]), "+r"(d[9]), "+r"(d[10]), "+r"(d[11]), "+r"(d[12]), "+r"(d[13]), "+r"(d[14]), "+r"(d[15]),
+              "+r"(d[16]), "+r"(d[17]), "+r"(d[18]), "+r"(d[19]), "+r"(d[20]), "+r"(d[21]), "+r"(d[22]), "+r"(d[23]),
+              "+r"(d[24]), "+r"(d[25]), "+r"(d[26]), "+r"(d[27]), "+r"(d[28]), "+r"(d[29]), "+r"(d[30]), "+r"(d[31])
+            : "l"(adesc), "l"(bdesc), "r"((uint32_t)accumulate)
+            : "memory");
+}
+template <>
+__device__ __forceinline__ void wgmma_m64nNk32_s8<96>(int32_t* d, uint64_t adesc, uint64_t bdesc, bool accumulate) {
+    asm volatile(
+            "{\n\t.reg .pred p;\n\t"
+            "setp.ne.b32 p, %50, 0;\n\t"
+            "wgmma.mma_async.sync.aligned.m64n96k32.s32.s8.s8 "
+            "{%0,%1,%2,%3,%4,%5,%6,%7,%8,%9,%10,%11,%12,%13,%14,%15,%16,%17,%18,%19,%20,%21,%22,%23,%24,%25,%26,%27,%28,%29,%30,%31,%32,%33,%34,%35,%36,%37,%38,%39,%40,%41,%42,%43,%44,%45,%46,%47}, %48, %49, p;\n\t}"
+            : "+r"(d[0]), "+r"(d[1]), "+r"(d[2]), "+r"(d[3]), "+r"(d[4]), "+r"(d[5]), "+r"(d[6]), "+r"(d[7]),
+              "+r"(d[8]), "+r"(d[9]), "+r"(d[10]), "+r"(d[11]), "+r"(d[12]), "+r"(d[13]), "+r"(d[14]), "+r"(d[15]),
+              "+r"(d[16]), "+r"(d[17]), "+r"(d[18]), "+r"(d[19]), "+r"(d[20]), "+r"(d[21]), "+r"(d[22]), "+r"(d[23]),
+              "+r"(d[24]), "+r"(d[25]), "+r"(d[26]), "+r"(d[27]), "+r"(d[28]), "+r"(d[29]), "+r"(d[30]), "+r"(d[31]),
+              "+r"(d[32]), "+r"(d[33]), "+r"(d[34]), "+r"(d[35]), "+r"(d[36]), "+r"(d[37]), "+r"(d[38]), "+r"(d[39]),
+              "+r"(d[40]), "+r"(d[41]), "+r"(d[42]), "+r"(d[43]), "+r"(d[44]), "+r"(d[45]), "+r"(d[46]), "+r"(d[47])
+            : "l"(adesc), "l"(bdesc), "r"((uint32_t)accumulate)
+            : "memory");
+}
+template <>
+__device__ __forceinline__ void wgmma_m64nNk32_s8<128>(int32_t* d, uint64_t adesc, uint64_t bdesc, bool accumulate) {
+    asm volatile(
+            "{\n\t.reg .pred p;\n\t"
+            "setp.ne.b32 p, %66, 0;\n\t"
+            "wgmma.mma_async.sync.aligned.m64n128k32.s32.s8.s8 "
+            "{%0,%1,%2,%3,%4,%5,%6,%7,%8,%9,%10,%11,%12,%13,%14,%15,%16,%17,%18,%19,%20,%21,%22,%23,%24,%25,%26,%27,%28,%29,%30,%31,%32,%33,%34,%35,%36,%37,%38,%39,%40,%41,%42,%43,%44,%45,%46,%47,%48,%49,%50,%51,%52,%53,%54,%55,%56,%57,%58,%59,%60,%61,%62,%63}, %64, %65, p;\n\t}"
+            : "+r"(d[0]), "+r"(d[1]), "+r"(d[2]), "+r"(d[3]), "+r"(d[4]), "+r"(d[5]), "+r"(d[6]), "+r"(d[7]),
+              "+r"(d[8]), "+r"(d[9]), "+r"(d[10]), "+r"(d[11]), "+r"(d[12]), "+r"(d[13]), "+r"(d[14]), "+r"(d[15]),
+              "+r"(d[16]), "+r"(d[17]), "+r"(d[18]), "+r"(d[19]), "+r"(d[20]), "+r"(d[21]), "+r"(d[22]), "+r"(d[23]),
+              "+r"(d[24]), "+r"(d[25]), "+r"(d[26]), "+r"(d[27]), "+r"(d[28]), "+r"(d[29]), "+r"(d[30]), "+r"(d[31]),
+              "+r"(d[32]), "+r"(d[33]), "+r"(d[34]), "+r"(d[35]), "+r"(d[36]), "+r"(d[37]), "+r"(d[38]), "+r"(d[39]),
+              "+r"(d[40]), "+r"(d[41]), "+r"(d[42]), "+r"(d[43]), "+r"(d[44]), "+r"(d[45]), "+r"(d[46]), "+r"(d[47]),
+              "+r"(d[48]), "+r"(d[49]), "+r"(d[50]), "+r"(d[51]), "+r"(d[52]), "+r"(d[53]), "+r"(d[54]), "+r"(d[55]),
+              "+r"(d[56]), "+r"(d[57]), "+r"(d[58]), "+r"(d[59]), "+r"(d[60]), "+r"(d[61]), "+r"(d[62]), "+r"(d[63])
             : "l"(adesc), "l"(bdesc), "r"((uint32_t)accumulate)
             : "memory");
 }
diff --git a/dorado_b200/lib.py b/dorado_b200/lib.py
--- a/dorado_b200/lib.py
+++ b/dorado_b200/lib.py
@@ -85,7 +85,7 @@
     "b200_runner_set_decoder_options", "b200_runner_batch_size", "b200_runner_chunk_size", "b200_runner_out_len",
     "b200_runner_accept_chunk_f16", "b200_runner_accept_chunk_f32", "b200_runner_input", "b200_runner_call_chunks",
     "b200_runner_upload", "b200_runner_step_device", "b200_runners_step_device", "b200_runner_forward_scores", "b200_runner_profile", "b200_runner_plan_info", "b200_runner_debug_read_workspace", "b200_decode_scores",
-    "b200_test_gemm", "b200_test_gemm_fp8", "b200_test_gemm_s8", "b200_test_quantize_rows", "b200_test_to_e4m3", "b200_test_remove_bits", "b200_test_attention", "b200_generate_chunks", "b200_stitch_chunks", "b200_runner_accept_raw_chunk",
+    "b200_test_gemm", "b200_test_gemm_fp8", "b200_test_gemm_s8", "b200_test_gemm_store_map", "b200_test_gemm_strided", "b200_test_quantize_rows", "b200_test_to_e4m3", "b200_test_remove_bits", "b200_test_attention", "b200_generate_chunks", "b200_stitch_chunks", "b200_runner_accept_raw_chunk",
     "b200_runner_debug_read_input", "b200_engine_runner_bytes", "b200_engine_benchmark_batch_sizes",
     "b200_select_batch_size", "b200_generate_variable_chunks", "b200_engine_terminate", "b200_engine_restart",
     "b200_engine_set_low_latency", "b200_engine_is_low_latency", "b200_engine_batch_timeouts_ms",
@@ -172,6 +172,10 @@
     lib.b200_test_gemm_fp8.argtypes = [i32, vp, vp, i32, i32, i32, i32, vp, f32, vp]
     lib.b200_test_gemm_s8.argtypes = [i32, vp, vp, vp, vp, i32, i32, i32, i32, vp]
     lib.b200_test_quantize_rows.argtypes = [vp, i32, i32, vp, vp]
+    i64 = C.c_int64
+    lib.b200_test_gemm_store_map.argtypes = [i32, i32, i32, i32, i64, i64, i64, vp, vp]
+    lib.b200_test_gemm_strided.argtypes = [i32, vp, i64, i32, i32, i64, i64, vp, vp, i32, i32, i32, i32, i64, i64, i64, i64, i32,
+                                           vp, vp]
     lib.b200_test_to_e4m3.argtypes = [vp, C.c_int64, vp]
     lib.b200_test_remove_bits.argtypes = [vp, C.c_int64, i32, vp]
     u64 = C.c_uint64
@@ -313,6 +317,36 @@
     return c
 
 
+def gemm_store_map(batches: int, rows_per_batch: int, N: int, out_m1: int, out_s0: int, out_s1: int, q8_store: bool = False):
+    info = np.zeros(11, np.int64)
+    tiles = batches * ((rows_per_batch + 127) // 128)
+    slices = np.zeros((tiles, 2, 2), np.uint32)
+    check(load_library().b200_test_gemm_store_map(batches, rows_per_batch, N, int(q8_store), out_m1, out_s0, out_s1,
+                                                  info.ctypes.data, slices.ctypes.data))
+    keys = dict(staged=bool(info[0]), elem_bytes=int(info[1]), dims=tuple(int(x) for x in info[2:5]),
+                strides=tuple(int(x) for x in info[5:7]), box=tuple(int(x) for x in info[7:10]), bn=int(info[10]))
+    return keys, slices
+
+
+def test_gemm_strided(a: np.ndarray, batches: int, rows_per_batch: int, a_row_stride: int, a_batch_stride: int, w: np.ndarray,
+                      bias: np.ndarray | None, activation: int, out: np.ndarray, out_m1: int, out_s0: int, out_s1: int,
+                      q8_store: bool = False, max_ctas: int = 0, device: int = 0):
+    lib = load_library()
+    a = np.ascontiguousarray(a, np.float16).ravel()
+    w = np.ascontiguousarray(w, np.float16)
+    N, K = w.shape
+    res = np.ascontiguousarray(out).copy()
+    bias_p = None
+    if bias is not None:
+        bias = np.ascontiguousarray(bias, np.float32)
+        bias_p = bias.ctypes.data
+    staged = np.zeros(1, np.int32)
+    check(lib.b200_test_gemm_strided(device, a.ctypes.data, a.size, batches, rows_per_batch, a_row_stride, a_batch_stride,
+                                     w.ctypes.data, bias_p, N, K, activation, int(q8_store), out_m1, out_s0, out_s1, res.nbytes,
+                                     max_ctas, res.ctypes.data, staged.ctypes.data))
+    return res, bool(staged[0])
+
+
 def quantize_rows(w: np.ndarray):
     h = np.ascontiguousarray(w, np.float16)
     q = np.empty(h.shape, np.int8)
diff --git a/include/b200call.h b/include/b200call.h
--- a/include/b200call.h
+++ b/include/b200call.h
@@ -307,6 +307,13 @@
                                 int32_t activation, const uint16_t* residual, float alpha, void* c);
 B200_API int b200_test_gemm_s8(int32_t device, const int8_t* a, const int8_t* b, const float* col_scale, const float* bias,
                                int32_t M, int32_t N, int32_t K, int32_t activation, uint16_t* c);
+B200_API int b200_test_gemm_store_map(int32_t batches, int32_t rows_per_batch, int32_t N, int32_t q8_store, int64_t out_m1,
+                                      int64_t out_s0, int64_t out_s1, int64_t* info, uint32_t* slices);
+B200_API int b200_test_gemm_strided(int32_t device, const uint16_t* a, int64_t a_elems, int32_t batches, int32_t rows_per_batch,
+                                    int64_t a_row_stride, int64_t a_batch_stride, const uint16_t* w ,
+                                    const float* bias , int32_t N, int32_t K, int32_t activation, int32_t q8_store,
+                                    int64_t out_m1, int64_t out_s0, int64_t out_s1, int64_t out_bytes, int32_t max_ctas, void* out,
+                                    int32_t* staged);
 B200_API int b200_test_quantize_rows(const uint16_t* f16, int32_t rows, int32_t cols, int8_t* q, uint16_t* scale);
 B200_API int b200_test_to_e4m3(const uint16_t* f16, int64_t n, uint8_t* out);
 B200_API int b200_test_remove_bits(const uint16_t* f16, int64_t n, int32_t bits, uint16_t* out);
```
